# Geo3DSmart/PDANet

Measured on AMD Instinct MI355X. Metric: scenes/sec (16384-pt ONCE, PDA-SSD forward+backward), higher is better.
Workload: dtype f32; 1 GPU; once16k_b2_detector_fwd_bwd_adam; scenes_per_gpu=2, global_batch=2, parallelism=dp1, world_size_seen=1, cpu_affinity=GPU-local NUMA node of 0000:26:00.0: 128 CPUs, full=False, graph_tail=False, graph_head=True

## Files before the change

include/pda_pointnet2.h:

```cpp
#ifndef PDA_POINTNET2_H
#define PDA_POINTNET2_H

#include <stdint.h>

#ifdef __cplusplus
extern "C" {
#endif

#define PDA_OK 0
#define PDA_ERR_INVALID_ARGUMENT 1
#define PDA_ERR_LAUNCH 2
#define PDA_ERR_UNSUPPORTED 3

typedef void *pda_stream_t;

#define PDA_POINTNET2_ABI_VERSION 20
int pda_abi_version(void);
const char *pda_last_error(void);
int pda_fp_contract_mode(void);
int pda_opt_n_threads(int work_size);
int pda_fps_coop_timeouts(unsigned long long *total, int reset);
int pda_debug_fps_spin_limit(int polls);
long long pda_debug_fps_exchange_nonzero(void);

int pda_furthest_point_sampling(const float *xyz, float *temp, int32_t *idx, int b, int n, int m,
                                pda_stream_t stream);
int pda_furthest_point_sampling_with_dist(const float *dist, float *temp, int32_t *idx, int b,
                                          int n, int m, pda_stream_t stream);

int pda_gather_points(const float *points, const int32_t *idx, float *out, int b, int c, int n,
                      int m, pda_stream_t stream);
int pda_gather_points_grad(const float *grad_out, const int32_t *idx, float *grad_points, int b,
                           int c, int n, int m, pda_stream_t stream);

int pda_ball_query(const float *new_xyz, const float *xyz, int32_t *idx, int b, int n, int m,
                   float radius, int nsample, pda_stream_t stream);
int pda_ball_query_dilated(const float *new_xyz, const float *xyz, int32_t *idx, int b, int n,
                           int m, float max_radius, float min_radius, int nsample,
                           pda_stream_t stream);
int pda_ellipsoid_query(const float *new_xyz, const float *xyz, int32_t *idx, int b, int n, int m,
                        float e1, float e2, float e3, int nsample, pda_stream_t stream);
int64_t pda_ball_query_cells_scratch_bytes(int b, int n);
int pda_ball_query_cells(const float *new_xyz, const float *xyz, int32_t *const *idx, int b, int n, int m, int nr,
                         const float *radii, const int32_t *nsamples, void *scratch, int64_t scratch_bytes,
                         pda_stream_t stream);
int pda_ball_query_multi(const float *new_xyz, const float *xyz, int32_t *const *idx, int b, int n,
                         int m, int nr, const float *radii, const int32_t *nsamples,
                         pda_stream_t stream);

int pda_group_points(const float *points, const int32_t *idx, float *out, int b, int c, int n,
                     int npoints, int nsample, pda_stream_t stream);
int pda_group_points_grad(const float *grad_out, const int32_t *idx, float *grad_points, int b,
                          int c, int n, int npoints, int nsample, pda_stream_t stream);

int pda_group_rows(const float *rows, const int32_t *idx, float *out, int b, int n, int c,
                   int64_t num_idx, pda_stream_t stream);
int pda_group_rows_grad(const float *grad_out, const int32_t *idx, float *grad_rows, int b, int n,
                        int c, int64_t num_idx, pda_stream_t stream);

int pda_three_nn(const float *unknown, const float *known, float *dist2, int32_t *idx, int b,
                 int n, int m, pda_stream_t stream);
int pda_three_interpolate(const float *points, const int32_t *idx, const float *weight,
                          float *out, int b, int c, int m, int n, pda_stream_t stream);
int pda_three_interpolate_grad(const float *grad_out, const int32_t *idx, const float *weight,
                               float *grad_points, int b, int c, int n, int m,
                               pda_stream_t stream);

int pda_chamfer_forward(const float *xyz1, const float *xyz2, float *dist1, float *dist2,
                        int32_t *idx1, int32_t *idx2, int b, int n, int m, pda_stream_t stream);
int pda_chamfer_backward(const float *xyz1, const float *xyz2, float *gradxyz1, float *gradxyz2,
                         const float *graddist1, const float *graddist2, const int32_t *idx1,
                         const int32_t *idx2, int b, int n, int m, pda_stream_t stream);

int pda_group_attention_fwd(const float *qkv, float *out, float *lse, int64_t num_groups, int seq,
                            int heads, int head_dim, pda_stream_t stream);
int pda_group_attention_bwd(const float *qkv, const float *grad_out, const float *lse,
                            float *grad_qkv, int64_t num_groups, int seq, int heads, int head_dim,
                            pda_stream_t stream);
int pda_group_attention_fwd_bf16(const uint16_t *qkv, uint16_t *out, float *lse, int64_t num_groups, int seq,
                                 int heads, int head_dim, pda_stream_t stream);
int pda_group_attention_bwd_bf16(const uint16_t *qkv, const uint16_t *grad_out, const float *lse,
                                 uint16_t *grad_qkv, int64_t num_groups, int seq, int heads, int head_dim,
                                 pda_stream_t stream);

int pda_sa_mlp_maxpool(const float *xyz, const float *new_xyz, const float *features,
                       const int32_t *idx, float *out, int b, int n, int m, int c, int nsample,
                       const int32_t *dims, const float *const *wf, const float *const *scale,
                       const float *const *shift, pda_stream_t stream);
int pda_linear_cols_packed_size(int n_out, int k);
int pda_linear_cols_pack(const float *w, float *wf, int n_out, int k, int transposed_source, int gather_order,
                         pda_stream_t stream);
int pda_linear_cols(const float *x, const float *wf, float *y, int64_t tokens, int k, int n_out, pda_stream_t stream);
int pda_sa_gather_linear(const float *xyz, const float *new_xyz, const float *feats_pm, const int32_t *idx,
                         const float *wf, float *y, int b, int n, int m, int c, int nsample, int n_out,
                         pda_stream_t stream);
int64_t pda_linear_split_packed_bytes(int n_out, int k);
int pda_linear_split_pack(const float *w, void *wf, int n_out, int k, int transposed_source, pda_stream_t stream);
int pda_linear_split_pack_both(const float *w, void *wf, void *wft, int n_out, int k, pda_stream_t stream);
int pda_linear_split(const float *x, const void *wf, const float *bias, float *y, int64_t tokens, int k, int n_out,
                     int relu, pda_stream_t stream);
int pda_gemm_split(const float *x, const void *wf, const float *bias, float *y, int64_t tokens, int k, int n_out,
                   int relu, int accumulate, pda_stream_t stream);
int pda_sa_mlp_packed_size(int rows, int cols, int first_layer);
int pda_sa_mlp_pack_weights(const float *w, float *wf, int rows, int cols, int first_layer,
                            pda_stream_t stream);

#ifdef __cplusplus
}
#endif
#endif
```

include/pda_train.h:

```cpp
#ifndef PDA_TRAIN_H
#define PDA_TRAIN_H
#include "pda_pointnet2.h"

#ifdef __cplusplus
extern "C" {
#endif

int pda_grad_norm(const float *g, int64_t n, float *norm_out, float *scratch1024, pda_stream_t stream);
int pda_adam_onecycle_step(float *p, const float *g, float *m, float *v, int64_t n, float lr,
                           float beta1, float beta2, float eps, float wd, int step,
                           const float *total_norm, float max_norm, pda_stream_t stream);

int64_t pda_bn_relu_scratch_bytes(int c);
int pda_bn_relu_fwd(const float *x, const float *gamma, const float *beta, float *running_mean,
                    float *running_var, float *y, float *mean_invstd, void *scratch, int64_t rows, int c,
                    float eps, float momentum, pda_stream_t stream);
int pda_bn_relu_bwd(const float *x, const float *grad_y, const float *gamma, const float *beta,
                    const float *mean_invstd, float *grad_x, float *grad_gamma, float *grad_beta,
                    void *scratch, int64_t rows, int c, pda_stream_t stream);
int pda_bn_relu_fwd_counted(const float *x, const float *gamma, const float *beta, float *running_mean, float *running_var,
                            float *y, float *mean_invstd, void *scratch, int64_t rows, int c, float eps, float momentum,
                            const int32_t *count, int32_t *status, int relu, int training, pda_stream_t stream);
int pda_bn_relu_bwd_counted(const float *x, const float *grad_y, const float *gamma, const float *beta,
                            const float *mean_invstd, float *grad_x, float *grad_gamma, float *grad_beta, void *scratch,
// ... 112 lines not shown
int pda_assemble_tokens_ragged(const float *rppe, const float *dscale, const float *feats, const int32_t *idx,
                               const float *glob, const int32_t *rowmap, const int32_t *off, float *out,
                               int64_t max_tokens, int b, int n, int m, int nsample, int c, int rppe_compact,
                               pda_stream_t stream);
int pda_assemble_tokens_ragged_grad(const float *grad_out, const float *dscale, const float *feats,
                                    const int32_t *idx, const int32_t *cnt, const int32_t *off, const int32_t *rowmap,
                                    float *grad_rppe, float *grad_dscale, float *grad_feats, float *grad_glob,
                                    int64_t max_tokens, int b, int n, int m, int nsample, int c, int rppe_compact,
                                    pda_stream_t stream);
int pda_add_max_pool_ragged(const float *a, const float *b, const int32_t *cnt, const int32_t *off, float *out,
                            uint8_t *arg, int64_t groups, int d, pda_stream_t stream);
int pda_max_pool_scatter_ragged(const float *grad_out, const uint8_t *arg, const int32_t *rowmap,
                                const int32_t *off, float *grad_x, int64_t max_tokens, int64_t groups, int nsample,
                                int d, pda_stream_t stream);
int pda_group_attention_ragged_fwd(const float *qkv, const int32_t *cnt, const int32_t *off, float *out, float *lse,
                                   int64_t tokens, int64_t num_groups, int seq, int heads, int head_dim,
                                   pda_stream_t stream);
int pda_group_attention_ragged_bwd(const float *qkv, const float *grad_out, const float *lse, const int32_t *cnt,
                                   const int32_t *off, float *grad_qkv, int64_t tokens, int64_t num_groups, int seq,
                                   int heads, int head_dim, pda_stream_t stream);

int pda_densitynet_param_count(void);
int64_t pda_densitynet_scratch_bytes(void);
int pda_densitynet_fwd(const float *x, const float *params, float *y, float *stats, void *scratch,
                       float *running_mean1, float *running_var1, float *running_mean2, float *running_var2,
                       float *running_mean3, float *running_var3, int64_t n, float eps, float momentum,
                       pda_stream_t stream);
int pda_densitynet_bwd(const float *x, const float *grad_y, const float *params, const float *stats,
                       float *grad_params, void *scratch, int64_t n, float eps, pda_stream_t stream);
int pda_densitynet_fwd_unique(const float *x, const float *params, float *y, float *stats, void *scratch,
                              float *running_mean1, float *running_var1, float *running_mean2, float *running_var2,
                              float *running_mean3, float *running_var3, int64_t n, const int32_t *rowmap,
                              const float *row_weight, const int32_t *n_unique, int nsample, float eps, float momentum,
                              pda_stream_t stream);
int pda_densitynet_bwd_unique(const float *x, const float *grad_y, const float *params, const float *stats,
                              float *grad_params, void *scratch, int64_t n, const int32_t *rowmap,
                              const float *row_weight, const int32_t *n_unique, int nsample, float eps,
                              pda_stream_t stream);
#define PDA_DENSITYNET_MAX_SCALES 4
typedef struct pda_densitynet_scale {
    const float *x, *grad_y, *params;
    float *y, *stats;
    void *scratch;
    float *running[6];
    float *grad_params;
    int64_t n;
    const int32_t *rowmap;
    const float *row_weight;
    const int32_t *n_unique;
    int nsample;
    float eps, momentum;
} pda_densitynet_scale_t;
int pda_densitynet_fwd_multi(const pda_densitynet_scale_t *scales, int nscales, pda_stream_t stream);
int pda_densitynet_bwd_multi(const pda_densitynet_scale_t *scales, int nscales, pda_stream_t stream);

int pda_densitynet_eval_param_count(void);
int pda_densitynet_eval(const float *x, const float *folded, float *y, int64_t n, pda_stream_t stream);

int pda_pda_geometry(const float *xyz, const float *new_xyz, const int32_t *idx, float *rppe, float *dscale,
                     int b, int n, int m, int nsample, float radius, pda_stream_t stream);

int pda_points_in_boxes(const float *boxes, const float *pts, int32_t *box_idx_of_points, int b, int t,
                        int m, pda_stream_t stream);
int pda_roiaware_pool3d_fwd(const float *rois, const float *pts, const float *pts_feature, int32_t *argmax,
                            int32_t *pts_idx_of_voxels, float *pooled_features, int boxes_num, int pts_num,
                            int channels, int max_pts_each_voxel, int out_x, int out_y, int out_z, int pool_method,
                            pda_stream_t stream);
int pda_roiaware_pool3d_bwd(const int32_t *pts_idx_of_voxels, const int32_t *argmax, const float *grad_out,
                            float *grad_in, int boxes_num, int pts_num, int channels, int max_pts_each_voxel,
                            int out_x, int out_y, int out_z, int pool_method, pda_stream_t stream);
int pda_roipoint_pool3d_fwd(const float *xyz, const float *boxes3d, const float *pts_feature, float *pooled_features,
                            int32_t *pooled_empty_flag, int batch_size, int pts_num, int boxes_num, int channels,
                            int sampled_pts_num, pda_stream_t stream);
int pda_points_in_boxes_mask(const float *boxes, const float *pts, int32_t *mask, int boxes_num, int pts_num,
                             pda_stream_t stream);
int pda_points_in_boxes_count(const float *points, int stride, const float *boxes, int32_t *counts, int pts_num,
                              int batch_size, int boxes_num, pda_stream_t stream);
int pda_assign_point_targets(const float *gt_boxes, const int32_t *in_box, const int32_t *in_ext, int64_t *labels,
                             int64_t *box_idx, float *gt_of_points, int b, int n, int t, int mode, int single_class,
                             pda_stream_t stream);
int pda_head_assign_targets(const float *points, int point_stride, int point_offset, const float *gt_boxes, const float *extra_width,
                            int64_t *labels, int64_t *box_idx, float *gt_of_points, float *box_labels, const float *mean_size,
                            int bins, int b, int n, int t, int mode, int single_class, pda_stream_t stream);
int pda_sa_gaussian_mask(const float *coords, int stride, int offset, const float *gt_of_points, const int64_t *labels,
                         float *out, int64_t points, pda_stream_t stream);

int pda_boxes_overlap_bev(const float *boxes_a, const float *boxes_b, float *ans_overlap, int num_a,
                          int num_b, pda_stream_t stream);
int pda_boxes_iou_bev(const float *boxes_a, const float *boxes_b, float *ans_iou, int num_a, int num_b,
                      pda_stream_t stream);
int64_t pda_nms_mask_words(int n);
int pda_nms_bev(const float *boxes, const int32_t *num_valid, int64_t *keep, int32_t *num_keep,
                uint64_t *mask_scratch, int b, int n, float thresh, int normal, pda_stream_t stream);
int pda_multi_nms_compact(const float *boxes, const float *scores, const int64_t *keep, const int32_t *num_keep,
                          const int32_t *label_map, int b, int c, int k, int post_max, float *pred_boxes, float *pred_scores,
                          int64_t *pred_labels, int32_t *num_pred, pda_stream_t stream);
int pda_multi_nms_compact_wide(int box_cols, const float *boxes, const float *scores, const int64_t *keep,
                               const int32_t *num_keep, const int32_t *label_map, int b, int c, int k, int post_max,
                               float *pred_boxes, float *pred_scores, int64_t *pred_labels, int32_t *num_pred,
                               pda_stream_t stream);

int pda_head_cls_loss(const float *preds, int row_stride, int col0, int num_class, const int64_t *labels, const float *soft,
                      int64_t n, float scale, float *out2, float *grad, pda_stream_t stream);
int pda_head_centerness(const float *centers, const float *gt, const int64_t *labels, float *out, int64_t n, pda_stream_t stream);
int pda_head_box_loss(const float *preds, const float *labels, const int64_t *cls_labels, const float *code_weights, float beta,
                      int bins, float dir_weight, float box_weight, int64_t n, float *out4, float *grad, pda_stream_t stream);
int pda_head_vote_loss(int mode, const float *origin, const float *offsets, const int64_t *key, const float *gt, int b, int boxes,
                       int num_class, float weight, int64_t n, float *out1, float *grad, pda_stream_t stream);
int pda_head_corner_loss(const float *box_preds, const float *centers, const float *cls_preds, int num_class, const float *gt,
                         const int64_t *cls_labels, const float *mean_size, int bins, float weight, int64_t n, float *out1,
                         float *grad_box, float *grad_centers, pda_stream_t stream);

int64_t pda_sa_small_train_workspace_bytes(void);
int pda_sa_small_train_supported(int c, int nsample, int c1, int c2, int c3, int64_t tokens);
int pda_sa_small_train_fwd(const float *xyz, const float *new_xyz, const float *feat_pm, const int32_t *idx,
                           const float *w1, const float *w2, const float *w3, const float *const *gamma,
                           const float *const *beta, float *const *running_mean, float *const *running_var,
                           const float *eps, const float *momentum, void *workspace, float *out, float *zmax,
                           uint8_t *arg, int b, int n, int m, int c, int nsample, int c1, int c2, int c3,
                           pda_stream_t stream);
int pda_sa_small_train_bwd(const float *xyz, const float *new_xyz, const float *feat_pm, const int32_t *idx,
                           const float *grad_out, const float *zmax, const uint8_t *arg, void *workspace, float *dz2,
                           float *dz1, float *dw1, float *dw2, float *dw3, float *const *dgamma, float *const *dbeta,
                           int b, int n, int m, int c, int nsample, int c1, int c2, int c3, pda_stream_t stream);

int64_t pda_sa_xyz_grad_scratch_bytes(int c1);
int pda_sa_point_gather(const float *point_rows, const float *xyz, const float *new_xyz, const int32_t *idx, const float *w,
                        int ldw, const float *bias, int relu, float *z, int b, int n, int m, int nsample, int c1,
                        pda_stream_t stream);
int pda_sa_xyz_grad(const float *grad_z1, const float *xyz, const float *new_xyz, const int32_t *idx, const float *w, int ldw,
                    float *dw, int lddw, float *grad_new_xyz, void *scratch, int b, int n, int m, int nsample, int c1,
                    pda_stream_t stream);
int64_t pda_sa_point_gather_stats_blocks(int64_t tokens, int c1);
int pda_sa_point_gather_stats(const float *point_rows, const float *xyz, const float *new_xyz, const int32_t *idx,
                              const float *w, int ldw, float *z, double *partial, int b, int n, int m, int nsample, int c1,
                              pda_stream_t stream);
int pda_sa_point_grad_bn(const float *grad_a1, const float *z1, const float *mean_invstd, const float *gamma,
                         const float *beta, const float *bwd_sums, const float *xyz, const float *new_xyz, const int32_t *idx,
                         const float *w, int ldw, float *dw, int lddw, float *grad_new_xyz, float *grad_points, void *scratch,
                         int b, int n, int m, int nsample, int c1, pda_stream_t stream);

int64_t pda_input_stage_workspace_bytes(int batch, int64_t n_cap);
int pda_input_stage(const float *points, const int64_t *offsets, int64_t n_total, int batch, int c, int64_t n_cap,
                    const float *range6, int num_points, const int32_t *pick, const int32_t *perm1, const int32_t *perm2,
                    uint64_t seed, int shuffle, float *out_points, int32_t *info, void *workspace, pda_stream_t stream);
int pda_input_boxes(const float *boxes, const int64_t *box_offsets, int64_t m_total, int batch, int box_dim, int max_gt,
                    const float *range6, int min_num_corners, float *gt_boxes, int32_t *info, pda_stream_t stream);

int64_t pda_augment_workspace_bytes(int batch, int64_t n_cap, int k);
int pda_augment(const float *points, const int64_t *offsets, int64_t n_total, int batch, int c, int64_t n_cap,
                const float *boxes, const int64_t *box_offsets, int64_t m_total, const float *db_points,
                const int64_t *db_offsets, int64_t db_n_points, const float *db_boxes, const double *db_centre,
                const int32_t *db_class, int n_obj, const int32_t *cand, const int32_t *cand_group, const double *cand_dz,
                int k, const int32_t *flip, const double *angle, const float *scale, const float *remove_extra_width,
                int64_t paste_cap, float *out_points, int64_t out_cap, int64_t *out_offsets, float *out_boxes,
                int64_t out_box_cap, int64_t *out_box_offsets, int32_t *info, void *workspace, pda_stream_t stream);

int pda_augment_paste(const float *points, const int64_t *offsets, int64_t n_total, int batch, int c, int64_t n_cap,
                      const float *boxes, const int64_t *box_offsets, int64_t m_total, const float *db_points,
                      const int64_t *db_offsets, int64_t db_n_points, const float *db_boxes, const double *db_centre,
                      const int32_t *db_class, int n_obj, const int32_t *cand, const int32_t *cand_group,
                      const double *cand_dz, int k, const float *remove_extra_width, int64_t paste_cap, float *out_points,
                      int64_t out_cap, int64_t *out_offsets, float *out_boxes, int64_t out_box_cap,
                      int64_t *out_box_offsets, int32_t *info, void *workspace, pda_stream_t stream);

int64_t pda_augment_steps_workspace_bytes(int batch, int64_t n_cap, int box_slots, int n_ops);
int pda_augment_steps(const float *points, const int64_t *offsets, int64_t n_total, int batch, int c, int64_t n_cap,
                      const float *boxes, const int64_t *box_offsets, int64_t m_total, const int32_t *ops, int n_ops,
                      const double *scene_draws, const double *box_draws, int draw_cap, int box_slots,
                      const int32_t *info_in, float *out_points, int64_t out_cap, int64_t *out_offsets, float *out_boxes,
                      int64_t out_box_cap, int64_t *out_box_offsets, int32_t *info, void *workspace, pda_stream_t stream);

int64_t pda_pyramid_aug_workspace_bytes(int batch, int64_t n_cap, int box_slots);
int pda_pyramid_aug(const float *points, const int64_t *offsets, int64_t n_total, int batch, int c, int64_t n_cap,
                    const float *boxes, const int64_t *box_offsets, int64_t m_total, const double *draws_f64,
                    const int32_t *draws_i32, const uint64_t *sparsify_key, const int32_t *sparsify_keep,
                    const int32_t *n_draws, int draw_cap, const double *probs, int sparsify_max, int swap_max,
                    int box_slots, const int32_t *info_in, float *out_points, int64_t out_cap, int64_t *out_offsets,
                    float *out_boxes, int64_t out_box_cap, int64_t *out_box_offsets, int32_t *info, void *workspace,
                    pda_stream_t stream);

typedef struct pda_once_frames {
    const double *gt_boxes;
    const int32_t *gt_name;
    const int64_t *gt_offsets;
    const float *pred_boxes, *pred_score;
    const int32_t *pred_name;
    const int64_t *pred_start;
    const int32_t *pred_count;
    const int64_t *iou_start;
    int64_t n_gt_total, pred_cap, iou_cap;
    int n_frames, max_gt, max_pred;
} pda_once_frames_t;

// ... 265 lines not shown
```

pdanet_amd/_lib.py:

```python
import ctypes
import os

_HERE = os.path.dirname(os.path.abspath(__file__))
LIB_PATH = os.environ.get("PDA_LIB_PATH") or os.path.join(_HERE, "libpda_pointnet2.so")
ABI_VERSION = 20


class DensityNetScale(ctypes.Structure):
    _fields_ = [("x", ctypes.c_void_p), ("grad_y", ctypes.c_void_p), ("params", ctypes.c_void_p), ("y", ctypes.c_void_p),
                ("stats", ctypes.c_void_p), ("scratch", ctypes.c_void_p), ("running", ctypes.c_void_p * 6),
                ("grad_params", ctypes.c_void_p), ("n", ctypes.c_int64), ("rowmap", ctypes.c_void_p),
                ("row_weight", ctypes.c_void_p), ("n_unique", ctypes.c_void_p), ("nsample", ctypes.c_int),
                ("eps", ctypes.c_float), ("momentum", ctypes.c_float)]


class OnceFrames(ctypes.Structure):
    _fields_ = [("gt_boxes", ctypes.c_void_p), ("gt_name", ctypes.c_void_p), ("gt_offsets", ctypes.c_void_p),
                ("pred_boxes", ctypes.c_void_p), ("pred_score", ctypes.c_void_p), ("pred_name", ctypes.c_void_p),
                ("pred_start", ctypes.c_void_p), ("pred_count", ctypes.c_void_p), ("iou_start", ctypes.c_void_p),
                ("n_gt_total", ctypes.c_int64), ("pred_cap", ctypes.c_int64), ("iou_cap", ctypes.c_int64),
                ("n_frames", ctypes.c_int), ("max_gt", ctypes.c_int), ("max_pred", ctypes.c_int)]


class KittiFrames(ctypes.Structure):
    _fields_ = [(n, ctypes.c_void_p) for n in ("gt_bbox", "gt_loc", "gt_dims", "gt_ry", "gt_alpha", "gt_trunc", "gt_occ",
                                               "gt_name", "gt_offsets", "dt_bbox", "dt_box", "dt_alpha", "dt_score",
                                               "dt_name", "dt_start", "dt_count", "ov_start", "frame_mode")] + \
               [("n_gt_total", ctypes.c_int64), ("det_cap", ctypes.c_int64), ("ov_cap", ctypes.c_int64),
                ("n_frames", ctypes.c_int), ("max_gt", ctypes.c_int), ("max_det", ctypes.c_int)]


class ParamGradEntry(ctypes.Structure):
    _fields_ = [("kind", ctypes.c_int32), ("count", ctypes.c_int32), ("part", ctypes.c_void_p), ("part_bias", ctypes.c_void_p),
                ("dst", ctypes.c_void_p), ("dst_bias", ctypes.c_void_p), ("nm", ctypes.c_int64), ("n", ctypes.c_int32),
                ("cols", ctypes.c_int32), ("ld", ctypes.c_int64)]


PARAM_EPOCH = [0]
WEIGHT_EPOCH = [0]

_vp = ctypes.c_void_p
_i = ctypes.c_int
_f = ctypes.c_float

SIGNATURES = {
    "pda_furthest_point_sampling": [_vp, _vp, _vp, _i, _i, _i, _vp],
    "pda_furthest_point_sampling_with_dist": [_vp, _vp, _vp, _i, _i, _i, _vp],
    "pda_gather_points": [_vp, _vp, _vp, _i, _i, _i, _i, _vp],
    "pda_gather_points_grad": [_vp, _vp, _vp, _i, _i, _i, _i, _vp],
    "pda_ball_query": [_vp, _vp, _vp, _i, _i, _i, _f, _i, _vp],
    "pda_ball_query_dilated": [_vp, _vp, _vp, _i, _i, _i, _f, _f, _i, _vp],
    "pda_ellipsoid_query": [_vp, _vp, _vp, _i, _i, _i, _f, _f, _f, _i, _vp],
    "pda_ball_query_cells_scratch_bytes": [_i, _i],
    "pda_ball_query_cells": [_vp, _vp, ctypes.POINTER(_vp), _i, _i, _i, _i, ctypes.POINTER(_f), ctypes.POINTER(ctypes.c_int32),
                             _vp, ctypes.c_int64, _vp],
    "pda_ball_query_multi": [_vp, _vp, ctypes.POINTER(_vp), _i, _i, _i, _i,
                             ctypes.POINTER(_f), ctypes.POINTER(ctypes.c_int32), _vp],
    "pda_group_points": [_vp, _vp, _vp, _i, _i, _i, _i, _i, _vp],
    "pda_group_points_grad": [_vp, _vp, _vp, _i, _i, _i, _i, _i, _vp],
    "pda_group_rows": [_vp, _vp, _vp, _i, _i, _i, ctypes.c_int64, _vp],
    "pda_group_rows_grad": [_vp, _vp, _vp, _i, _i, _i, ctypes.c_int64, _vp],
    "pda_three_nn": [_vp, _vp, _vp, _vp, _i, _i, _i, _vp],
    "pda_three_interpolate": [_vp, _vp, _vp, _vp, _i, _i, _i, _i, _vp],
    "pda_three_interpolate_grad": [_vp, _vp, _vp, _vp, _i, _i, _i, _i, _vp],
    "pda_chamfer_forward": [_vp, _vp, _vp, _vp, _vp, _vp, _i, _i, _i, _vp],
    "pda_chamfer_backward": [_vp, _vp, _vp, _vp, _vp, _vp, _vp, _vp, _i, _i, _i, _vp],
    "pda_group_attention_fwd": [_vp, _vp, _vp, ctypes.c_int64, _i, _i, _i, _vp],
    "pda_group_attention_bwd": [_vp, _vp, _vp, _vp, ctypes.c_int64, _i, _i, _i, _vp],
    "pda_group_attention_fwd_bf16": [_vp, _vp, _vp, ctypes.c_int64, _i, _i, _i, _vp],
    "pda_group_attention_bwd_bf16": [_vp, _vp, _vp, _vp, ctypes.c_int64, _i, _i, _i, _vp],
    "pda_sa_mlp_maxpool": [_vp, _vp, _vp, _vp, _vp, _i, _i, _i, _i, _i, ctypes.POINTER(ctypes.c_int32),
                           ctypes.POINTER(_vp), ctypes.POINTER(_vp), ctypes.POINTER(_vp), _vp],
    "pda_linear_cols_packed_size": [_i, _i],
    "pda_linear_cols_pack": [_vp, _vp, _i, _i, _i, _i, _vp],
    "pda_linear_cols": [_vp, _vp, _vp, ctypes.c_int64, _i, _i, _vp],
    "pda_sa_gather_linear": [_vp, _vp, _vp, _vp, _vp, _vp, _i, _i, _i, _i, _i, _i, _vp],
    "pda_linear_split_packed_bytes": [_i, _i],
    "pda_linear_split_pack": [_vp, _vp, _i, _i, _i, _vp],
    "pda_linear_split_pack_both": [_vp, _vp, _vp, _i, _i, _vp],
    "pda_linear_split": [_vp, _vp, _vp, _vp, ctypes.c_int64, _i, _i, _i, _vp],
    "pda_gemm_split": [_vp, _vp, _vp, _vp, ctypes.c_int64, _i, _i, _i, _i, _vp],
    "pda_sa_mlp_packed_size": [_i, _i, _i],
    "pda_sa_mlp_pack_weights": [_vp, _vp, _i, _i, _i, _vp],
    "pda_grad_norm": [_vp, ctypes.c_int64, _vp, _vp, _vp],
    "pda_bn_relu_scratch_bytes": [_i],
    "pda_bn_relu_fwd": [_vp, _vp, _vp, _vp, _vp, _vp, _vp, _vp, ctypes.c_int64, _i, _f, _f, _vp],
    "pda_bn_relu_bwd": [_vp, _vp, _vp, _vp, _vp, _vp, _vp, _vp, _vp, ctypes.c_int64, _i, _vp],    "pda_bn_relu_fwd_mixed": [_vp, _i, _vp, _vp, _vp, _vp, _vp, _i, _vp, _vp, ctypes.c_int64, _i, _f, _f, _vp],
    "pda_bn_relu_bwd_mixed": [_vp, _i, _vp, _i, _vp, _vp, _vp, _vp, _vp, _vp, _vp, ctypes.c_int64, _i, _vp],
    "pda_bn_relu_max_pool_fwd": [_vp, _i, _vp, _vp, _vp, _vp, _vp, _vp, _vp, _vp, ctypes.c_int64, _i, _i, _f, _f, _vp],
    "pda_bn_relu_max_pool_bwd": [_vp, _i, _vp, _vp, _vp, _vp, _vp, _vp, _vp, _vp, _vp, ctypes.c_int64, _i, _i, _vp],

    "pda_layer_norm_scratch_bytes": [_i],
    "pda_layer_norm_fwd": [_vp, _vp, _vp, _vp, _vp, _vp, _vp, ctypes.c_int64, _i, _f, _vp],
    "pda_layer_norm_bwd": [_vp, _vp, _vp, _vp, _vp, _vp, _vp, _vp, _vp, ctypes.c_int64, _i, _vp],
    "pda_layer_norm_fwd_mixed": [_vp, _i, _vp, _vp, _vp, _vp, _vp, _vp, _vp, ctypes.c_int64, _i, _f, _vp],
    "pda_layer_norm_bwd_mixed": [_vp, _vp, _vp, _i, _vp, _vp, _vp, _vp, _vp, _vp, _vp, ctypes.c_int64, _i, _vp],
    "pda_linear_wgrad_scratch_bytes": [ctypes.c_int64, _i, _i],
    "pda_linear_wgrad_form": [ctypes.c_int64, _i, _i],
    "pda_linear_wgrad": [_vp, _vp, _vp, _vp, _vp, ctypes.c_int64, _i, _i, _vp],
    "pda_linear_wgrad_bn": [_vp, _vp, _vp, _vp, _vp, ctypes.c_int64, _i, _i, _vp, _vp, _vp, _vp],
    "pda_linear_wgrad_partials": [_vp, _vp, _vp, _i, ctypes.c_int64, _i, _i, ctypes.POINTER(_i), _vp],
    "pda_linear_wgrad_bn_partials": [_vp, _vp, _vp, ctypes.c_int64, _i, _i, _vp, _vp, _vp, ctypes.POINTER(_i), _vp],
    "pda_layer_norm_bwd_partials": [_vp, _vp, _vp, _i, _vp, _vp, _vp, _vp, _vp, ctypes.c_int64, _i, ctypes.POINTER(_i), _vp],
    "pda_param_grad_reduce_grouped": [ctypes.POINTER(ParamGradEntry), _i, _vp],
    "pda_gemm_split_bn_tiles": [ctypes.c_int64],
    "pda_gemm_split_bn": [_vp, _vp, _vp, ctypes.c_int64, _i, _i, _vp, _vp, _vp, _i, _vp, _vp],
    "pda_gemm_split_maxpool": [_vp, _vp, _vp, _vp, ctypes.c_int64, _i, _i, _i, _i, _vp],
    "pda_gemm_split_gather": [_vp, _vp, _vp, _vp, _vp, _i, _vp, _vp, _vp, _vp, _i, _i, _i, _i, _i, _i, _i, _vp],
    "pda_bn_stats_fwd": [_vp, _vp, _vp, _vp, _vp, ctypes.c_int64, _i, _f, _f, _vp],
    "pda_bn_finalize_fwd": [_vp, _i, _i, ctypes.c_int64, _f, _f, _vp, _vp, _vp, _vp],
    "pda_bn_relu_max_pool_apply": [_vp, _vp, _vp, _vp, _vp, _vp, ctypes.c_int64, _i, _i, _vp],
    "pda_bn_relu_bwd_reduce": [_vp, _vp, _vp, _vp, _vp, _vp, _vp, _vp, _vp, ctypes.c_int64, _i, _vp],
    "pda_colsum_scratch_bytes": [_i],
    "pda_colsum_bf16": [_vp, _vp, _vp, ctypes.c_int64, _i, _vp],
    "pda_assemble_tokens": [_vp, _vp, _vp, _vp, _vp, _vp, _i, _i, _i, _i, _i, _vp],
    "pda_assemble_tokens_grad": [_vp, _vp, _vp, _vp, _vp, _vp, _vp, _vp, _i, _i, _i, _i, _i, _vp],
    "pda_add_max_pool": [_vp, _vp, _vp, _vp, ctypes.c_int64, _i, _i, _vp],
    "pda_max_pool_scatter": [_vp, _vp, _vp, ctypes.c_int64, _i, _i, _vp],
    "pda_add_max_pool_bf16": [_vp, _vp, _vp, _vp, ctypes.c_int64, _i, _i, _vp],
    "pda_max_pool_scatter_bf16": [_vp, _vp, _vp, _vp, ctypes.c_int64, _i, _i, _vp],
    "pda_ragged_plan": [_vp, _vp, _vp, _vp, _vp, ctypes.c_int64, _i, _vp],
    "pda_assemble_tokens_ragged": [_vp, _vp, _vp, _vp, _vp, _vp, _vp, _vp, ctypes.c_int64, _i, _i, _i, _i, _i, _i, _vp],
    "pda_assemble_tokens_ragged_grad": [_vp, _vp, _vp, _vp, _vp, _vp, _vp, _vp, _vp, _vp, _vp, ctypes.c_int64, _i, _i, _i, _i, _i, _i, _vp],
    "pda_bn_relu_fwd_weighted": [_vp, _vp, _vp, _vp, _vp, _vp, _vp, _vp, ctypes.c_int64, _i, _f, _f, _vp, ctypes.c_int64, _vp],
    "pda_bn_relu_bwd_weighted": [_vp, _vp, _vp, _vp, _vp, _vp, _vp, _vp, _vp, ctypes.c_int64, _i, _vp, ctypes.c_int64, _vp],
    "pda_add_max_pool_ragged": [_vp, _vp, _vp, _vp, _vp, _vp, ctypes.c_int64, _i, _vp],
    "pda_max_pool_scatter_ragged": [_vp, _vp, _vp, _vp, _vp, ctypes.c_int64, ctypes.c_int64, _i, _i, _vp],
    "pda_group_attention_ragged_fwd": [_vp, _vp, _vp, _vp, _vp, ctypes.c_int64, ctypes.c_int64, _i, _i, _i, _vp],
    "pda_group_attention_ragged_bwd": [_vp, _vp, _vp, _vp, _vp, _vp, ctypes.c_int64, ctypes.c_int64, _i, _i, _i, _vp],
    "pda_densitynet_param_count": [],
    "pda_densitynet_eval_param_count": [],
    "pda_densitynet_scratch_bytes": [],
    "pda_densitynet_fwd": [_vp, _vp, _vp, _vp, _vp, _vp, _vp, _vp, _vp, _vp, _vp, ctypes.c_int64, _f, _f, _vp],
    "pda_densitynet_bwd": [_vp, _vp, _vp, _vp, _vp, _vp, ctypes.c_int64, _f, _vp],
    "pda_densitynet_eval": [_vp, _vp, _vp, ctypes.c_int64, _vp],
    "pda_densitynet_fwd_multi": [_vp, _i, _vp],
    "pda_densitynet_bwd_multi": [_vp, _i, _vp],
    "pda_densitynet_fwd_unique": [_vp, _vp, _vp, _vp, _vp, _vp, _vp, _vp, _vp, _vp, _vp, ctypes.c_int64, _vp, _vp, _vp, _i, _f, _f, _vp],
    "pda_densitynet_bwd_unique": [_vp, _vp, _vp, _vp, _vp, _vp, ctypes.c_int64, _vp, _vp, _vp, _i, _f, _vp],
    "pda_pda_geometry": [_vp, _vp, _vp, _vp, _vp, _i, _i, _i, _i, _f, _vp],
    "pda_points_in_boxes": [_vp, _vp, _vp, _i, _i, _i, _vp],
    "pda_roiaware_pool3d_fwd": [_vp, _vp, _vp, _vp, _vp, _vp, _i, _i, _i, _i, _i, _i, _i, _i, _vp],
    "pda_roiaware_pool3d_bwd": [_vp, _vp, _vp, _vp, _i, _i, _i, _i, _i, _i, _i, _i, _vp],
    "pda_roipoint_pool3d_fwd": [_vp, _vp, _vp, _vp, _vp, _i, _i, _i, _i, _i, _vp],
    "pda_points_in_boxes_mask": [_vp, _vp, _vp, _i, _i, _vp],
    "pda_points_in_boxes_count": [_vp, _i, _vp, _vp, _i, _i, _i, _vp],
    "pda_assign_point_targets": [_vp, _vp, _vp, _vp, _vp, _vp, _i, _i, _i, _i, _i, _vp],
    "pda_sa_gaussian_mask": [_vp, _i, _i, _vp, _vp, _vp, ctypes.c_int64, _vp],
    "pda_head_assign_targets": [_vp, _i, _i, _vp, ctypes.POINTER(ctypes.c_float), _vp, _vp, _vp, _vp, _vp, _i, _i, _i, _i, _i, _i, _vp],
    "pda_head_cls_loss": [_vp, _i, _i, _i, _vp, _vp, ctypes.c_int64, _f, _vp, _vp, _vp],
    "pda_head_centerness": [_vp, _vp, _vp, _vp, ctypes.c_int64, _vp],
    "pda_head_box_loss": [_vp, _vp, _vp, _vp, _f, _i, _f, _f, ctypes.c_int64, _vp, _vp, _vp],
    "pda_head_vote_loss": [_i, _vp, _vp, _vp, _vp, _i, _i, _i, _f, ctypes.c_int64, _vp, _vp, _vp],
    "pda_head_corner_loss": [_vp, _vp, _vp, _i, _vp, _vp, _vp, _i, _f, ctypes.c_int64, _vp, _vp, _vp, _vp],
    "pda_boxes_overlap_bev": [_vp, _vp, _vp, _i, _i, _vp],
    "pda_boxes_iou_bev": [_vp, _vp, _vp, _i, _i, _vp],
    "pda_nms_mask_words": [_i],
    "pda_nms_bev": [_vp, _vp, _vp, _vp, _vp, _i, _i, _f, _i, _vp],
    "pda_sa_small_train_workspace_bytes": [],
    "pda_sa_small_train_supported": [_i, _i, _i, _i, _i, ctypes.c_int64],
    "pda_sa_small_train_fwd": [_vp] * 7 + [ctypes.POINTER(_vp)] * 4 + [ctypes.POINTER(_f)] * 2 + [_vp] * 4 + [_i] * 8 + [_vp],
    "pda_sa_small_train_bwd": [_vp] * 13 + [ctypes.POINTER(_vp)] * 2 + [_i] * 8 + [_vp],
    "pda_sa_xyz_grad_scratch_bytes": [_i],
    "pda_sa_point_gather": [_vp, _vp, _vp, _vp, _vp, _i, _vp, _i, _vp, _i, _i, _i, _i, _i, _vp],
    "pda_sa_xyz_grad": [_vp, _vp, _vp, _vp, _vp, _i, _vp, _i, _vp, _vp, _i, _i, _i, _i, _i, _vp],
    "pda_sa_point_gather_stats_blocks": [ctypes.c_int64, _i],
    "pda_sa_point_gather_stats": [_vp, _vp, _vp, _vp, _vp, _i, _vp, _vp, _i, _i, _i, _i, _i, _vp],
    "pda_sa_point_grad_bn": [_vp] * 10 + [_i, _vp, _i, _vp, _vp, _vp, _i, _i, _i, _i, _i, _vp],
    "pda_adam_onecycle_step": [_vp, _vp, _vp, _vp, ctypes.c_int64, _f, _f, _f, _f, _f, _i, _vp, _f, _vp],
    "pda_input_stage_workspace_bytes": [_i, ctypes.c_int64],
    "pda_input_stage": [_vp, _vp, ctypes.c_int64, _i, _i, ctypes.c_int64, ctypes.POINTER(_f), _i, _vp, _vp, _vp,
                        ctypes.c_uint64, _i, _vp, _vp, _vp, _vp],
    "pda_input_boxes": [_vp, _vp, ctypes.c_int64, _i, _i, _i, ctypes.POINTER(_f), _i, _vp, _vp, _vp],
    "pda_augment_workspace_bytes": [_i, ctypes.c_int64, _i],
    "pda_augment": [_vp, _vp, ctypes.c_int64, _i, _i, ctypes.c_int64, _vp, _vp, ctypes.c_int64, _vp, _vp, ctypes.c_int64, _vp,
                    _vp, _vp, _i, _vp, _vp, _vp, _i, _vp, _vp, _vp, ctypes.POINTER(_f), ctypes.c_int64, _vp, ctypes.c_int64,
                    _vp, _vp, ctypes.c_int64, _vp, _vp, _vp, _vp],
    "pda_augment_paste": [_vp, _vp, ctypes.c_int64, _i, _i, ctypes.c_int64, _vp, _vp, ctypes.c_int64, _vp, _vp, ctypes.c_int64, _vp,
                          _vp, _vp, _i, _vp, _vp, _vp, _i, ctypes.POINTER(_f), ctypes.c_int64, _vp, ctypes.c_int64, _vp, _vp,
                          ctypes.c_int64, _vp, _vp, _vp, _vp],
    "pda_augment_steps_workspace_bytes": [_i, ctypes.c_int64, _i, _i],
    "pda_augment_steps": [_vp, _vp, ctypes.c_int64, _i, _i, ctypes.c_int64, _vp, _vp, ctypes.c_int64,
                          ctypes.POINTER(ctypes.c_int32), _i, _vp, _vp, _i, _i, _vp, _vp, ctypes.c_int64, _vp, _vp,
                          ctypes.c_int64, _vp, _vp, _vp, _vp],
    "pda_pyramid_aug_workspace_bytes": [_i, ctypes.c_int64, _i],
    "pda_pyramid_aug": [_vp, _vp, ctypes.c_int64, _i, _i, ctypes.c_int64, _vp, _vp, ctypes.c_int64, _vp, _vp, _vp, _vp, _vp, _i,
                        ctypes.POINTER(ctypes.c_double), _i, _i, _i, _vp, _vp, ctypes.c_int64, _vp, _vp, ctypes.c_int64, _vp,
                        _vp, _vp, _vp],
    "pda_once_eval_workspace_bytes": [_i, ctypes.c_int64, _i],
    "pda_once_eval_iou": [ctypes.POINTER(OnceFrames), _i, _vp, _vp, _vp],
    "pda_once_eval_accumulate": [ctypes.POINTER(OnceFrames), _vp, _vp, _i, _i, ctypes.POINTER(ctypes.c_double), _i, _vp, _vp,
                                 _vp, _vp],
    "pda_once_eval_match": [ctypes.POINTER(OnceFrames), _vp, _vp, _i, _i, ctypes.POINTER(ctypes.c_double), _i, _i, _vp, _vp,
                            _vp, _vp, _vp, _vp, _vp, _vp],
    "pda_kitti_eval_workspace_bytes": [_i, ctypes.c_int64, ctypes.c_int64, _i],
    "pda_kitti_eval_overlaps": [ctypes.POINTER(KittiFrames), _vp, _vp, _vp],
    "pda_kitti_eval_first_pass": [ctypes.POINTER(KittiFrames), _vp, _i, _i, _vp, _vp, _vp, ctypes.POINTER(ctypes.c_double),
                                  _vp, _vp, _vp, _vp, _vp, _vp],
    "pda_kitti_eval_match": [ctypes.POINTER(KittiFrames), _vp, _i, _i, _vp, _vp, _vp, ctypes.POINTER(ctypes.c_double), _i,
                             _vp, _vp, _vp, _vp, _vp, _vp, _vp, _vp, _vp, _vp, _vp],
    "pda_kitti_eval_predictions": [_vp, ctypes.c_int64, _i, _i, _vp, _vp, _vp, _i, _vp, _vp, _vp, _vp, _vp],
    "pda_recall_record": [_vp, _vp, _vp, _i, ctypes.POINTER(_f), _i, _vp, _vp, _i, _i, _i, _vp],
    "pda_roi_max_iou": [_vp, _vp, _vp, _i, _i, _vp, _vp, _i, _i, _i, _vp],
    "pda_roi_sample_targets": [_vp, _vp, _vp, _vp, _i, _vp, _vp, _i, _i] + [ctypes.c_double] * 5 + [_i, _vp, _vp, _vp, _vp,
                               ctypes.c_uint64] + [_vp] * 10 + [_i, _i, _i, _vp],
    "pda_kitti_fov_filter_workspace_bytes": [_i, ctypes.c_int64],
    "pda_kitti_fov_filter": [_vp, _vp, ctypes.c_int64, _i, _i, ctypes.c_int64, _vp, _vp, _vp, ctypes.c_int64, _vp, _vp, _vp, _vp],
    "pda_gt_extract_workspace_bytes": [_i, ctypes.c_int64, ctypes.c_int64],
    "pda_gt_extract_count": [_vp, _vp, ctypes.c_int64, _i, _i, ctypes.c_int64, _vp, _vp, ctypes.c_int64, _vp, _vp, _vp, _vp],
    "pda_gt_extract_write": [_vp, _vp, ctypes.c_int64, _i, _i, ctypes.c_int64, _vp, _vp, ctypes.c_int64, _vp, _vp, _vp,
                             ctypes.c_int64, _vp, _vp, _vp],
    "pda_voxel_workspace_bytes": [_i, ctypes.c_int64, _i, _i],
    "pda_voxelize": [_vp, _vp, ctypes.c_int64, _i, _i, ctypes.c_int64, ctypes.POINTER(_f), ctypes.POINTER(_f),
                     ctypes.POINTER(ctypes.c_int32), _i, _i, _vp, _vp, _vp, _vp, _vp, _vp],
    "pda_voxel_sample": [_vp, _vp, ctypes.c_int64, _i, _i, ctypes.c_int64, ctypes.POINTER(_f), ctypes.POINTER(_f),
                         ctypes.POINTER(ctypes.c_int32), _i, _i, _i, _i, _i, _vp, _vp, ctypes.c_int64, ctypes.c_uint64, _vp,
                         ctypes.c_int64, _vp, _vp, _vp, _vp],
    "pda_dyn_voxel_workspace_bytes": [ctypes.c_int64, _i],
    "pda_dyn_voxel_index": [_vp, ctypes.c_int64, _i, ctypes.POINTER(_f), ctypes.POINTER(_f), ctypes.POINTER(ctypes.c_int32),
                            _i, _i, _vp, _vp, _vp, _vp, _vp, _vp, _vp, _vp, _vp],
    "pda_dyn_scatter_mean": [_vp, _i, _vp, _vp, _vp, ctypes.c_int64, _vp, _vp],
    "pda_dyn_scatter_max_fwd": [_vp, _i, _vp, _vp, _vp, ctypes.c_int64, _vp, _vp, _vp],
    "pda_dyn_scatter_max_bwd": [_vp, _vp, _vp, _vp, ctypes.c_int64, ctypes.c_int64, _i, _vp, _vp],
    "pda_dyn_pillar_features": [_vp, ctypes.c_int64, _i, _vp, _vp, _vp, _vp, _vp, ctypes.POINTER(_f), ctypes.POINTER(_f), _i,
                                _i, _vp, _vp],
    "pda_pillar_scatter_fwd": [_vp, _vp, _vp, ctypes.c_int64, _i, _i, _i, _i, _vp, _vp],
    "pda_pillar_scatter_bwd": [_vp, _vp, _vp, ctypes.c_int64, _i, _i, _i, _i, _vp, _vp],
    "pda_center_assign_targets": [_vp, _i, _i, _i, _i, _i] + [ctypes.POINTER(ctypes.c_int32)] * 3 + [_i, _i, _i]
                                 + [ctypes.c_double] * 6 + [_i] + [ctypes.POINTER(_vp)] * 4 + [_vp],
    "pda_center_focal_blocks": [ctypes.c_int64],
    "pda_center_focal_loss": [_vp, _vp, ctypes.c_int64, _vp, _vp, _vp, _vp],
    "pda_center_scale": [_vp, _vp, _vp, _f, ctypes.c_int64, _vp, _vp],
# ... 139 lines not shown
```

pdanet_amd/csrc/gemm_split.hip:

```cpp
#include "pda_common.h"
#include "split_bf16.h"

#include <stdlib.h>

namespace pda {

constexpr int GS_MAX_N = 2048;
constexpr int GS_KSTEP = 12 * 64;

__device__ __forceinline__ void split_pack_one(const float* __restrict__ w, uint32_t* __restrict__ wf, int64_t o, int rows, int cols,
                                               int KS, int trans) {
    const int pr = (int)(o & 3), lane = (int)((o >> 2) & 63);
    int64_t rest = o >> 8;
    const int rb = (int)(rest & 3); rest >>= 2;
    const int s = (int)(rest % KS), c = (int)(rest / KS);
    const int row = c * 128 + rb * 32 + (lane & 31);
    const int k = 16 * s + 8 * (lane >> 5) + 2 * pr;
    float v[2];
    for (int e = 0; e < 2; ++e)
        v[e] = (row < rows && k + e < cols) ? (trans ? w[(size_t)(k + e) * rows + row] : w[(size_t)row * cols + k + e]) : 0.f;
    uint32_t h, m, l;
    split2(v[0], v[1], h, m, l);
    const size_t base = ((((size_t)c * KS + s) * 4 + rb) * 3) * 256 + (size_t)lane * 4 + pr;
    wf[base] = h; wf[base + 256] = m; wf[base + 512] = l;
}

__global__ void split_pack_kernel(const float* __restrict__ w, uint32_t* __restrict__ wf, int rows, int cols, int KS,
                                  int chunks, int trans) {
    const int64_t total = (int64_t)chunks * KS * 4 * 64 * 4;
    for (int64_t o = blockIdx.x * (int64_t)blockDim.x + threadIdx.x; o < total; o += (int64_t)gridDim.x * blockDim.x)
        split_pack_one(w, wf, o, rows, cols, KS, trans);
}

__global__ void split_pack_both_kernel(const float* __restrict__ w, uint32_t* __restrict__ wf, uint32_t* __restrict__ wft, int n_out,
                                       int k, int KS, int chunks, int KSt, int chunks_t) {
    const int64_t total = (int64_t)chunks * KS * 4 * 64 * 4, total_t = (int64_t)chunks_t * KSt * 4 * 64 * 4;
    for (int64_t o = blockIdx.x * (int64_t)blockDim.x + threadIdx.x; o < total + total_t; o += (int64_t)gridDim.x * blockDim.x) {
        if (o < total) split_pack_one(w, wf, o, n_out, k, KS, 0);
        else split_pack_one(w, wft, o - total, k, n_out, KSt, 1);
    }
}

struct LinSplitParams {
    const float* x;
    const uint4* wf;
    const float* bias;
    float* y;
    int64_t tokens;
    int k, n_out, chunks, relu;
    int cpb;
    unsigned long long* dbg;
};
#ifdef GS_PROFILE
#define GS_MARK(i) do { if (tid == 0) p.dbg[(size_t)blockIdx.x * 16 + (i)] = __builtin_readcyclecounter(); } while (0)
#else
#define GS_MARK(i) do {} while (0)
#endif

template <int KS>
__global__ __launch_bounds__(256) __attribute__((amdgpu_waves_per_eu(1, 1)))
void lin_split_kernel(const LinSplitParams p) {
    constexpr int G = KS % 4 == 0 ? 4 : 2;
    constexpr int TILE = G * GS_KSTEP;
    constexpr int NG = KS / G;
    constexpr int NLD = TILE / 256;
    __shared__ uint4 ring[3 * TILE];
    __shared__ float bias_s[GS_MAX_N];
    const int tid = threadIdx.x, lane = tid & 63, w = __builtin_amdgcn_readfirstlane(tid >> 6);
    const int h = lane >> 5, j = lane & 31;
    const int64_t tok0 = ((int64_t)blockIdx.x * 4 + w) * 32;
    const int64_t tk = tok0 + j < p.tokens ? tok0 + j : p.tokens - 1;
    const uint4* src = p.wf + tid;
    const int ntiles = p.chunks * NG;
    const int c0 = (int)blockIdx.y * p.cpb, c1 = min(p.chunks, c0 + p.cpb);
    const uint32_t ring_base = (uint32_t)(uintptr_t)(__attribute__((address_space(3))) void*)ring + w * 1024;
    auto issue = [&](int t, int slot) {
        const uint4* g = src + (size_t)(t < ntiles ? t : ntiles - 1) * TILE;
        const uint32_t l = ring_base + slot * (TILE * 16);
#pragma unroll
        for (int i = 0; i < NLD; ++i) glds16(g + 256 * i, l + 4096 * i);
    };
    static_assert(NLD <= G * 4, "one DMA instruction per MFMA group at most");
    GS_MARK(0);
    float x[KS * 8];
    {
        const float* row = p.x + tk * p.k + 8 * h;
#pragma unroll
        for (int s = 0; s < KS; ++s) {
            const float4 a = *reinterpret_cast<const float4*>(row + 16 * s), b = *reinterpret_cast<const float4*>(row + 16 * s + 4);
            x[8 * s] = a.x; x[8 * s + 1] = a.y; x[8 * s + 2] = a.z; x[8 * s + 3] = a.w;
            x[8 * s + 4] = b.x; x[8 * s + 5] = b.y; x[8 * s + 6] = b.z; x[8 * s + 7] = b.w;
        }
    }
    for (int i = tid; i < p.n_out; i += 256) bias_s[i] = p.bias ? p.bias[i] : 0.f;
    asm volatile("s_waitcnt vmcnt(0)" ::: "memory");
    GS_MARK(1);
    issue(c0 * NG, 0);
    issue(c0 * NG + 1, 1);
    asm volatile("s_waitcnt vmcnt(%0)" ::"n"(NLD) : "memory");
    __builtin_amdgcn_s_barrier();
    GS_MARK(2);
    const uint32_t lane_off = (uint32_t)(4 * h * p.n_out + j);
    const int64_t left = p.tokens - tok0 - 4 * h;
    const bool whole = tok0 + 32 <= p.tokens;
    auto store_one = [&](const gs_f32x16 (&res)[4], int chunk, int n) {
        const int r = n >> 4, i = n & 15, t = (i & 3) + 8 * (i >> 2);
        float v = res[r][i] + bias_s[chunk * 128 + r * 32 + j];
        if (p.relu) v = fmaxf(v, 0.f);
        float* row = p.y + (tok0 + t) * p.n_out + chunk * 128 + r * 32;
        if (whole) row[lane_off] = v;
        else if (t < left) row[lane_off] = v;
    };
    int ti = c0 * NG, slot = 0;
    gs_f32x16 done[4];
    for (int c = c0; c < c1; ++c) {
        gs_f32x16 acc[4];
#pragma unroll
        for (int r = 0; r < 4; ++r)
#pragma unroll
            for (int i = 0; i < 16; ++i) acc[r][i] = 0.f;
#pragma unroll
        for (int g = 0; g < NG; ++g, ++ti, slot = slot == 2 ? 0 : slot + 1) {
            if (c == 1 && g == 0) GS_MARK(4);
// ... 411 lines not shown
        }
        return;
    }
    double cs1[4], cs2[4];
#pragma unroll
    for (int ot = 0; ot < 4; ++ot) {
        cs1[ot] = 0; cs2[ot] = 0;
        const int col = (2 * ncb + wo) * 128 + ot * 32 + r;
        if (col >= p.n_out) continue;
        const float bias = p.bias ? p.bias[col] : 0.f;
#pragma unroll
        for (int tt = 0; tt < 2; ++tt) {
            const int64_t trow = tok0 + wt * 64 + tt * 32 + 4 * h;
#pragma unroll
            for (int i = 0; i < 16; ++i) {
                const int64_t tok = trow + (i & 3) + 8 * (i >> 2);
                if (tok < p.tokens) {
                    float* dst = p.y + tok * p.n_out + col;
                    float v = acc[tt][ot][i] + bias;
                    if (p.accum) v += *dst;
                    if (p.relu) v = fmaxf(v, 0.f);
#ifdef GS_NOSTORE
                    if (v == 12345.678f)
#endif
                    *dst = v;
                    if constexpr (EPI == 1) { cs1[ot] += v; cs2[ot] += (double)v * v; }
                }
            }
        }
    }
    if constexpr (EPI == 1) {
        double* red = reinterpret_cast<double*>(gp_planes);
        __syncthreads();
#pragma unroll
        for (int ot = 0; ot < 4; ++ot) {
            const double a = cs1[ot] + __shfl_xor(cs1[ot], 32), b = cs2[ot] + __shfl_xor(cs2[ot], 32);
            if (h == 0) {
                const int cl = wo * 128 + ot * 32 + r;
                red[(wt * 256 + cl) * 2] = a; red[(wt * 256 + cl) * 2 + 1] = b;
            }
        }
        __syncthreads();
        if (tid < 256) {
            const int col = 2 * ncb * 128 + tid;
            if (col < p.n_out) {
                double a = 0, b = 0;
#pragma unroll
                for (int q = 0; q < TW; ++q) { a += red[(q * 256 + tid) * 2]; b += red[(q * 256 + tid) * 2 + 1]; }
                double* pp = p.partial + (size_t)(blockIdx.x / (unsigned)wide_chunks) * 2 * p.n_out;
                pp[col] = a; pp[p.n_out + col] = b;
            }
        }
    }
}

}

PDA_API int64_t pda_linear_split_packed_bytes(int n_out, int k) {
    if (n_out <= 0 || k <= 0) return 0;
    return (int64_t)pda::divup(n_out, 128) * pda::divup(k, 32) * 2 * 12 * 64 * 16;
}

PDA_API int pda_linear_split_pack(const float* w, void* wf, int n_out, int k, int transposed_source, pda_stream_t stream) {
    PDA_REQUIRE(w && wf && n_out > 0 && k > 0, "pda_linear_split_pack: bad argument");
    const int chunks = pda::divup(n_out, 128), KS = pda::divup(k, 32) * 2;
    const int64_t total = (int64_t)chunks * KS * 4 * 64 * 4;
    const int blocks = (int)(pda::divup64(total, 256) < 2048 ? pda::divup64(total, 256) : 2048);
    hipLaunchKernelGGL(pda::split_pack_kernel, dim3(blocks), dim3(256), 0, (hipStream_t)stream, w, (uint32_t*)wf, n_out, k, KS,
                       chunks, transposed_source);
    return pda::check_launch("pda_linear_split_pack");
}

PDA_API int pda_linear_split_pack_both(const float* w, void* wf, void* wft, int n_out, int k, pda_stream_t stream) {
    PDA_REQUIRE(w && wf && wft && n_out > 0 && k > 0, "pda_linear_split_pack_both: bad argument");
    const int chunks = pda::divup(n_out, 128), KS = pda::divup(k, 32) * 2;
    const int chunks_t = pda::divup(k, 128), KSt = pda::divup(n_out, 32) * 2;
    const int64_t total = ((int64_t)chunks * KS + (int64_t)chunks_t * KSt) * 4 * 64 * 4;
    const int blocks = (int)(pda::divup64(total, 256) < 2048 ? pda::divup64(total, 256) : 2048);
    hipLaunchKernelGGL(pda::split_pack_both_kernel, dim3(blocks), dim3(256), 0, (hipStream_t)stream, w, (uint32_t*)wf, (uint32_t*)wft,
                       n_out, k, KS, chunks, KSt, chunks_t);
    return pda::check_launch("pda_linear_split_pack_both");
}

PDA_API int pda_linear_split(const float* x, const void* wf, const float* bias, float* y, int64_t tokens, int k, int n_out,
                             int relu, pda_stream_t stream) {
    PDA_REQUIRE(tokens >= 0 && k > 0 && n_out > 0, "pda_linear_split: bad size");
    if (tokens == 0) return PDA_OK;
    PDA_REQUIRE(x && wf && y && (((uintptr_t)x | (uintptr_t)wf | (uintptr_t)y | (uintptr_t)bias) & 15) == 0,
                "pda_linear_split: null or misaligned pointer");
    if (k % 32 != 0 || k > 512 || n_out % 128 != 0 || n_out > pda::GS_MAX_N) {
        pda::set_error("pda_linear_split: no kernel built for K=%d, N=%d (K a multiple of 32 <= 512, N a multiple of 128 <= 2048)", k, n_out);
        return PDA_ERR_UNSUPPORTED;
    }
    pda::LinSplitParams p{};
    p.x = x; p.wf = (const uint4*)wf; p.bias = bias; p.y = y; p.tokens = tokens; p.k = k; p.n_out = n_out; p.chunks = n_out / 128;
    p.relu = relu;
#ifdef GS_PROFILE
    p.dbg = (unsigned long long*)bias; p.bias = nullptr;
#endif
    const int64_t tiles = pda::divup64(tokens, 128);
    const int want = tiles >= 192 ? 1 : (int)pda::divup64(256, tiles);
    p.cpb = pda::divup(p.chunks, want < p.chunks ? want : p.chunks);
    const dim3 grid((unsigned)tiles, (unsigned)pda::divup(p.chunks, p.cpb)), block(256);
    const hipStream_t s = (hipStream_t)stream;
    switch (k / 16) {
#define PDA_GS_CASE(KS) case KS: hipLaunchKernelGGL((pda::lin_split_kernel<KS>), grid, block, 0, s, p); break
        PDA_GS_CASE(2); PDA_GS_CASE(4); PDA_GS_CASE(6); PDA_GS_CASE(8); PDA_GS_CASE(12); PDA_GS_CASE(16); PDA_GS_CASE(24); PDA_GS_CASE(32);
#undef PDA_GS_CASE
        default:
            pda::set_error("pda_linear_split: no kernel built for K=%d", k);
            return PDA_ERR_UNSUPPORTED;
    }
    return pda::check_launch("pda_linear_split");
}

PDA_API int pda_gemm_split(const float* x, const void* wf, const float* bias, float* y, int64_t tokens, int k, int n_out,
                           int relu, int accumulate, pda_stream_t stream) {
    PDA_REQUIRE(tokens >= 0 && k > 0 && n_out > 0, "pda_gemm_split: bad size");
    if (tokens == 0) return PDA_OK;
    PDA_REQUIRE(x && wf && y && (((uintptr_t)x | (uintptr_t)wf) & 15) == 0, "pda_gemm_split: null or misaligned pointer");
    if (k % 16 != 0) {
        pda::set_error("pda_gemm_split: K=%d must be a multiple of 16", k);
        return PDA_ERR_UNSUPPORTED;
    }
    pda::GemmSplitParams p{};
    p.x = x; p.wf = (const uint4*)wf; p.bias = bias; p.y = y; p.tokens = tokens; p.k = k; p.n_out = n_out;
    p.chunks = pda::divup(n_out, 128); p.ksteps = pda::divup(k, 32) * 2; p.relu = relu; p.accum = accumulate;
    const int64_t blocks = pda::divup64(tokens, 128) * p.chunks;
    PDA_REQUIRE(blocks < (1ll << 31), "pda_gemm_split: too many tiles");
    const int packed_steps = p.ksteps;
    p.ksteps = k / 16;
    if (packed_steps != p.ksteps) {
        pda::set_error("pda_gemm_split: K=%d must be a multiple of 32 (packed planes come in pairs of K steps)", k);
        return PDA_ERR_UNSUPPORTED;
    }
    static const int force = getenv("PDA_GEMM_SPLIT_TILE") ? atoi(getenv("PDA_GEMM_SPLIT_TILE")) : 0;
    const int64_t wide_blocks = pda::divup64(tokens, 256) * ((p.chunks + 1) / 2);
    if (force == 256 || (force != 128 && wide_blocks >= 200 && (p.chunks % 2 == 0 || p.chunks >= 5))) {
        static pda::PerDevice<bool> lds_ok;
        const bool ok = lds_ok.get([] { return hipFuncSetAttribute((const void*)pda::gemm_split_wide_kernel<0, 0>, hipFuncAttributeMaxDynamicSharedMemorySize,
                                                                   2 * pda::GW_TILE_U4 * 16) == hipSuccess; });
        if (ok) {
            hipLaunchKernelGGL((pda::gemm_split_wide_kernel<0, 0>), dim3((unsigned)wide_blocks), dim3(512), 2 * pda::GW_TILE_U4 * 16,
                               (hipStream_t)stream, p);
            return pda::check_launch("pda_gemm_split");
        }
    }
    hipLaunchKernelGGL(pda::gemm_split_kernel, dim3((unsigned)blocks), dim3(256), 0, (hipStream_t)stream, p);
    return pda::check_launch("pda_gemm_split");
}

PDA_API int64_t pda_gemm_split_bn_tiles(int64_t tokens) { return tokens > 0 ? pda::divup64(tokens, 256) : 0; }

PDA_API int pda_gemm_split_bn(const float* x, const void* wf, float* y, int64_t tokens, int k, int n_out, const float* in_mean_invstd,
                              const float* in_gamma, const float* in_beta, int stats_mode, double* partial, pda_stream_t stream) {
    PDA_REQUIRE(tokens >= 1 && k > 0 && n_out > 0, "pda_gemm_split_bn: bad size");
    PDA_REQUIRE(x && wf && y && (((uintptr_t)x | (uintptr_t)wf) & 15) == 0, "pda_gemm_split_bn: null or misaligned pointer");
    const bool pro = in_mean_invstd != nullptr;
    PDA_REQUIRE(pro == (in_gamma != nullptr) && pro == (in_beta != nullptr), "pda_gemm_split_bn: the input BatchNorm needs mean_invstd, gamma and beta");
    PDA_REQUIRE(stats_mode >= 0 && stats_mode <= 1 && (stats_mode == 0 || partial), "pda_gemm_split_bn: stats_mode=%d (0 or 1; 1 needs `partial`)", stats_mode);
    if (k % 32 != 0 || k > 1024) {
        pda::set_error("pda_gemm_split_bn: no kernel built for K=%d (a multiple of 32, <= 1024)", k);
        return PDA_ERR_UNSUPPORTED;
    }
    pda::GemmSplitParams p{};
    p.x = x; p.wf = (const uint4*)wf; p.y = y; p.tokens = tokens; p.k = k; p.n_out = n_out;
// ... 69 lines not shown
```

pdanet_amd/csrc/head_loss.hip:

```cpp
#include "pda_common.h"

namespace pda {

constexpr int HL_THREADS = 1024;

__device__ __forceinline__ double hl_block_sum(double v, double* red) {
    const int lane = threadIdx.x & 63, w = threadIdx.x >> 6;
#pragma unroll
    for (int o = 32; o > 0; o >>= 1) v += __shfl_down(v, o);
    __syncthreads();
    if (lane == 0) red[w] = v;
    __syncthreads();
    if (threadIdx.x == 0) {
        double s = 0;
        for (int i = 0; i < HL_THREADS / 64; ++i) s += red[i];
        red[16] = s;
    }
    __syncthreads();
    return red[16];
}

__device__ __forceinline__ float hl_smooth_l1(float d, float beta, float& dd) {
    const float n = fabsf(d);
    if (beta < 1e-5f) { dd = d > 0.f ? 1.f : (d < 0.f ? -1.f : 0.f); return n; }
    if (n < beta) { dd = d / beta; return 0.5f * n * n / beta; }
    dd = d > 0.f ? 1.f : -1.f;
    return n - 0.5f * beta;
}

__global__ __launch_bounds__(HL_THREADS) void head_cls_loss_kernel(const float* __restrict__ preds, int row_stride, int col0, int C,
                                                                   const int64_t* __restrict__ labels, const float* __restrict__ soft,
                                                                   int64_t n, float scale, float* __restrict__ out,
                                                                   float* __restrict__ grad) {
    __shared__ double red[17];
    double cnt = 0;
    for (int64_t r = threadIdx.x; r < n; r += HL_THREADS) cnt += labels[r] > 0 ? 1.0 : 0.0;
    const double npos = hl_block_sum(cnt, red);
    const float wnorm = 1.f / (float)(npos > 1.0 ? npos : 1.0);
    double acc = 0;
    for (int64_t r = threadIdx.x; r < n; r += HL_THREADS) {
        const int64_t lab = labels[r];
        const float w = lab >= 0 ? wnorm : 0.f;
        const float s = soft ? soft[r] : 1.f;
        const float* x = preds + r * row_stride;
        float* g = grad + r * row_stride;
        for (int c = 0; c < col0; ++c) g[c] = 0.f;
        for (int c = col0 + C; c < row_stride; ++c) g[c] = 0.f;
        float rowloss = 0.f;
        for (int c = 0; c < C; ++c) {
            const float v = x[col0 + c];
            const float t = lab == c + 1 ? s : 0.f;
            const float e = expf(-fabsf(v));
            rowloss += fmaxf(v, 0.f) - v * t + log1pf(e);
            const float sig = v >= 0.f ? 1.f / (1.f + e) : e / (1.f + e);
            g[col0 + c] = scale * w * (sig - t) / (float)C;
        }
        acc += (double)(w * rowloss) / C;
    }
    const double total = hl_block_sum(acc, red);
    if (threadIdx.x == 0) { out[0] = scale * (float)total; out[1] = (float)npos; }
}

__global__ __launch_bounds__(256) void head_centerness_kernel(const float* __restrict__ centers, const float* __restrict__ gt,
                                                              const int64_t* __restrict__ labels, float* __restrict__ out, int64_t n) {
    const int64_t p = (int64_t)blockIdx.x * 256 + threadIdx.x;
    if (p >= n) return;
    const float* c = centers + p * 4 + 1;
    const float* g = gt + p * 8;
    const float dx = c[0] - g[0], dy = c[1] - g[1], dz = c[2] - g[2];
    const float a = -g[6], ca = cosf(a), sa = sinf(a);
    const float o[3] = {dx * ca + dy * (-sa), dx * sa + dy * ca, dz};
    float prod = 1.f;
#pragma unroll
    for (int k = 0; k < 3; ++k) {
        const float m = g[3 + k] * 0.5f;
        const float d0 = m - o[k], d1 = m + o[k];
        prod *= fminf(d0, d1) / fmaxf(d0, d1);
    }
    out[p] = labels[p] > 0 ? powf(fmaxf(prod, 1e-6f), 1.f / 3.f) : 0.f;
}

__global__ __launch_bounds__(HL_THREADS) void head_box_loss_kernel(const float* __restrict__ preds, const float* __restrict__ labels,
                                                                   const int64_t* __restrict__ cls_labels, const float* __restrict__ code_w,
                                                                   float beta, int nb, float dir_w, float box_w, int64_t n,
                                                                   float* __restrict__ out, float* __restrict__ grad) {
    __shared__ double red[17];
    const int W = 6 + 2 * nb;
    double cnt = 0, sres = 0;
    for (int64_t r = threadIdx.x; r < n; r += HL_THREADS) {
        cnt += cls_labels[r] > 0 ? 1.0 : 0.0;
        const int id = (int)labels[r * 8 + 6];
        float dd;
        sres += hl_smooth_l1(preds[r * W + 6 + nb + id] - labels[r * 8 + 7], 1.f, dd);
    }
    const double npos = hl_block_sum(cnt, red);
    const double res_mean = hl_block_sum(sres, red) / (double)(n > 0 ? n : 1);
    const float wpos = 1.f / (float)(npos > 1.0 ? npos : 1.0);
    const float sumw = npos > 0.0 ? 1.f : 0.f;
    double a_xyz = 0, a_cls = 0;
    for (int64_t r = threadIdx.x; r < n; r += HL_THREADS) {
        const float w = cls_labels[r] > 0 ? wpos : 0.f;
        const float* x = preds + r * W;
        const float* l = labels + r * 8;
        float* g = grad + r * W;
        float rl = 0.f;
#pragma unroll
        for (int k = 0; k < 6; ++k) {
            const float cw = code_w ? code_w[k] : 1.f;
            const float t = (__float_as_uint(l[k]) & 0x7fffffffu) > 0x7f800000u ? x[k] : l[k];
            float dd;
            rl += hl_smooth_l1((x[k] - t) * cw, beta, dd);
            g[k] = box_w * w * dd * cw;
        }
        a_xyz += (double)(w * rl);
        const int id = (int)l[6];
        float mx = x[6];
        for (int k = 1; k < nb; ++k) mx = fmaxf(mx, x[6 + k]);
        float se = 0.f;
        for (int k = 0; k < nb; ++k) se += expf(x[6 + k] - mx);
        const float lse = mx + logf(se);
        a_cls += (double)(w * (lse - x[6 + id]));
        for (int k = 0; k < nb; ++k) g[6 + k] = box_w * dir_w * w * (expf(x[6 + k] - lse) - (k == id ? 1.f : 0.f));
        float dd;
        hl_smooth_l1(x[6 + nb + id] - l[7], 1.f, dd);
        for (int k = 0; k < nb; ++k) g[6 + nb + k] = k == id ? box_w * sumw * dd / (float)n : 0.f;
    }
    const double xyz = hl_block_sum(a_xyz, red);
    const double cls = hl_block_sum(a_cls, red) * dir_w;
    if (threadIdx.x == 0) {
        const double res = res_mean * sumw;
        out[0] = (float)((xyz + res + cls) * box_w); out[1] = (float)xyz; out[2] = (float)cls; out[3] = (float)res;
    }
}

constexpr int HL_MAX_SEG = 2048;
__global__ __launch_bounds__(HL_THREADS) void head_vote_loss_kernel(int mode, const float* __restrict__ origin, const float* __restrict__ offsets,
                                                                    const int64_t* __restrict__ key, const float* __restrict__ gt, int B,
                                                                    int S, int num_class, float weight, int64_t n, float* __restrict__ out,
                                                                    float* __restrict__ grad) {
    __shared__ double red[17];
    __shared__ float cnt[HL_MAX_SEG], m3[HL_MAX_SEG][3], a3[HL_MAX_SEG][3], lsum[HL_MAX_SEG];
    const int nseg = mode == 0 ? num_class + 1 : B * S;
    for (int s = threadIdx.x; s < nseg; s += HL_THREADS) {
        cnt[s] = 0.f; lsum[s] = 0.f;
        for (int k = 0; k < 3; ++k) { m3[s][k] = 0.f; a3[s][k] = 0.f; }
    }
    __syncthreads();
    const int64_t per_scene = n / (B > 0 ? B : 1);
    auto seg_of = [&](int64_t r) -> int {
        const int64_t k = key[r];
        if (mode == 0) return (k >= 1 && k <= num_class) ? (int)k : -1;
        return k >= 0 ? (int)(r / per_scene) * S + (int)k : -1;
    };
    for (int64_t r = threadIdx.x; r < n; r += HL_THREADS) {
        const int s = seg_of(r);
        if (s < 0) continue;
        atomicAdd(&cnt[s], 1.f);
        if (mode == 1)
            for (int k = 0; k < 3; ++k) atomicAdd(&m3[s][k], origin[r * 4 + 1 + k] + offsets[r * 4 + 1 + k]);
    }
    __syncthreads();
    if (mode == 1)
        for (int s = threadIdx.x; s < nseg; s += HL_THREADS)
            for (int k = 0; k < 3; ++k) m3[s][k] = m3[s][k] / fmaxf(cnt[s], 1.f);
    __syncthreads();
    double present = 0;
    for (int s = threadIdx.x; s < nseg; s += HL_THREADS) present += cnt[s] > 0.f ? 1.0 : 0.0;
    const double npresent = hl_block_sum(present, red);
    const float inv_present = 1.f / (float)(npresent > 1.0 ? npresent : 1.0);
    for (int64_t r = threadIdx.x; r < n; r += HL_THREADS) {
        const int s = seg_of(r);
        if (s < 0) continue;
        float l = 0.f;
        for (int k = 0; k < 3; ++k) {
            const float p = origin[r * 4 + 1 + k] + offsets[r * 4 + 1 + k];
            float dd;
            l += hl_smooth_l1(p - gt[r * 8 + k], 1.f, dd);
            if (mode == 1) {
                float dm;
                l += 0.5f * hl_smooth_l1(p - m3[s][k], 1.f, dm);
                atomicAdd(&a3[s][k], dm);
            }
        }
        atomicAdd(&lsum[s], l);
    }
    __syncthreads();
    double acc = 0;
    for (int s = threadIdx.x; s < nseg; s += HL_THREADS)
        if (cnt[s] > 0.f) acc += (double)lsum[s] / (double)(cnt[s] * (mode == 0 ? 3.f : 1.f));
    const double total = hl_block_sum(acc, red);
    if (threadIdx.x == 0) out[0] = mode == 0 ? (float)(total / npresent * weight) : (float)(total * inv_present * weight);
    for (int64_t r = threadIdx.x; r < n; r += HL_THREADS) {
        const int s = seg_of(r);
        float* g = grad + r * 4;
        g[0] = 0.f;
        if (s < 0) { g[1] = g[2] = g[3] = 0.f; continue; }
        const float base = weight / (mode == 0 ? (float)npresent * 3.f * cnt[s] : cnt[s]) * (mode == 0 ? 1.f : inv_present);
        for (int k = 0; k < 3; ++k) {
            const float p = origin[r * 4 + 1 + k] + offsets[r * 4 + 1 + k];
            float dd, dm = 0.f;
            hl_smooth_l1(p - gt[r * 8 + k], 1.f, dd);
            float d = dd;
            if (mode == 1) {
                hl_smooth_l1(p - m3[s][k], 1.f, dm);
                d += 0.5f * (dm - a3[s][k] / cnt[s]);
            }
            g[1 + k] = base * d;
        }
    }
}

__global__ __launch_bounds__(HL_THREADS) void head_corner_loss_kernel(const float* __restrict__ box_preds, const float* __restrict__ centers,
                                                                      const float* __restrict__ cls_preds, int C, const float* __restrict__ gt,
                                                                      const int64_t* __restrict__ cls_labels, const float* __restrict__ mean_size,
                                                                      int nb, float weight, int64_t n, float* __restrict__ out,
                                                                      float* __restrict__ grad_box, float* __restrict__ grad_ctr) {
    __shared__ double red[17];
    const int W = 6 + 2 * nb;
    const float PI = 3.14159265358979323846f;
    const float inter = 2.f * PI / (float)nb;
    double cnt = 0;
    for (int64_t r = threadIdx.x; r < n; r += HL_THREADS) cnt += cls_labels[r] > 0 ? 1.0 : 0.0;
    const double npos = hl_block_sum(cnt, red);
    const float wpos = weight / (float)npos;
    double acc = 0;
    const float tmpl[8][3] = {{1, 1, -1}, {1, -1, -1}, {-1, -1, -1}, {-1, 1, -1}, {1, 1, 1}, {1, -1, 1}, {-1, -1, 1}, {-1, 1, 1}};
    for (int64_t r = threadIdx.x; r < n; r += HL_THREADS) {
        float* gb = grad_box + r * W;
        float* gc = grad_ctr + r * 4;
        for (int k = 0; k < W; ++k) gb[k] = 0.f;
        gc[0] = gc[1] = gc[2] = gc[3] = 0.f;
        if (!(cls_labels[r] > 0)) continue;
        const float* e = box_preds + r * W;
        int pc = 0;
        for (int c = 1; c < C; ++c) pc = cls_preds[r * C + c] > cls_preds[r * C + pc] ? c : pc;
        float dxa = 1.f, dya = 1.f, dza = 1.f, diag = 1.f;
        if (mean_size) { dxa = mean_size[pc * 3]; dya = mean_size[pc * 3 + 1]; dza = mean_size[pc * 3 + 2]; diag = sqrtf(dxa * dxa + dya * dya); }
        const float xa = centers[r * 4 + 1], ya = centers[r * 4 + 2], za = centers[r * 4 + 3];
        const float xg = mean_size ? e[0] * diag + xa : e[0] + xa, yg = mean_size ? e[1] * diag + ya : e[1] + ya,
                    zg = mean_size ? e[2] * dza + za : e[2] + za;
        const float dxg = expf(e[3]) * dxa, dyg = expf(e[4]) * dya, dzg = expf(e[5]) * dza;
        int bin = 0;
        for (int k = 1; k < nb; ++k) bin = e[6 + k] > e[6 + bin] ? k : bin;
        const float ry = ((float)bin * inter - PI + inter * 0.5f) + e[6 + nb + bin] * (inter * 0.5f);
        const float* g = gt + r * 8;
        const float cp = cosf(ry), sp = sinf(ry), cg = cosf(g[6]), sg = sinf(g[6]), cf = cosf(g[6] + PI), sf = sinf(g[6] + PI);
        float d_x = 0.f, d_y = 0.f, d_z = 0.f, d_dx = 0.f, d_dy = 0.f, d_dz = 0.f, d_ry = 0.f, lsum = 0.f;
#pragma unroll
        for (int k = 0; k < 8; ++k) {
            const float tx = tmpl[k][0] * 0.5f, ty = tmpl[k][1] * 0.5f, tz = tmpl[k][2] * 0.5f;
            const float px = tx * dxg, py = ty * dyg;
            const float rx = px * cp - py * sp, rry = px * sp + py * cp;
            const float pcx = rx + xg, pcy = rry + yg, pcz = tz * dzg + zg;
            const float qx = tx * g[3], qy = ty * g[4];
            const float gx = qx * cg - qy * sg + g[0], gy = qx * sg + qy * cg + g[1], gz = tz * g[5] + g[2];
            const float fx = qx * cf - qy * sf + g[0], fy = qx * sf + qy * cf + g[1];
            const float ax = pcx - gx, ay = pcy - gy, az = pcz - gz;
            const float bx = pcx - fx, by = pcy - fy;
            const float d0 = sqrtf(ax * ax + ay * ay + az * az), d1 = sqrtf(bx * bx + by * by + az * az);
            const bool first = d0 <= d1;
            const float d = first ? d0 : d1;
            float dd;
            lsum += hl_smooth_l1(d, 1.f, dd);
            const float inv = d > 0.f ? dd / d : 0.f;
            const float ux = (first ? ax : bx) * inv, uy = (first ? ay : by) * inv, uz = az * inv;
            d_x += ux; d_y += uy; d_z += uz;
            d_dx += ux * tx * cp + uy * tx * sp;
            d_dy += -ux * ty * sp + uy * ty * cp;
            d_dz += uz * tz;
            d_ry += -ux * rry + uy * rx;
        }
        acc += (double)(lsum * 0.125f);
        const float s = wpos * 0.125f;
        gc[1] = s * d_x; gc[2] = s * d_y; gc[3] = s * d_z;
        gb[0] = s * d_x * (mean_size ? diag : 1.f); gb[1] = s * d_y * (mean_size ? diag : 1.f); gb[2] = s * d_z * (mean_size ? dza : 1.f);
        gb[3] = s * d_dx * dxg; gb[4] = s * d_dy * dyg; gb[5] = s * d_dz * dzg;
        gb[6 + nb + bin] = s * d_ry * (inter * 0.5f);
    }
    const double total = hl_block_sum(acc, red);
    if (threadIdx.x == 0) out[0] = (float)(total / npos) * weight;
}

}

PDA_API int pda_head_cls_loss(const float* preds, int row_stride, int col0, int num_class, const int64_t* labels, const float* soft,
                              int64_t n, float scale, float* out2, float* grad, pda_stream_t stream) {
    PDA_REQUIRE(n >= 0 && num_class >= 1 && col0 >= 0 && col0 + num_class <= row_stride, "pda_head_cls_loss: bad shape");
    PDA_REQUIRE(preds && labels && out2 && grad, "pda_head_cls_loss: null pointer");
    hipLaunchKernelGGL(pda::head_cls_loss_kernel, dim3(1), dim3(pda::HL_THREADS), 0, (hipStream_t)stream, preds, row_stride, col0, num_class,
                       labels, soft, n, scale, out2, grad);
    return pda::check_launch("pda_head_cls_loss");
}

PDA_API int pda_head_centerness(const float* centers, const float* gt, const int64_t* labels, float* out, int64_t n, pda_stream_t stream) {
    PDA_REQUIRE(n >= 0, "pda_head_centerness: n=%lld", (long long)n);
    if (n == 0) return PDA_OK;
    PDA_REQUIRE(centers && gt && labels && out, "pda_head_centerness: null pointer");
    hipLaunchKernelGGL(pda::head_centerness_kernel, dim3((unsigned)pda::divup64(n, 256)), dim3(256), 0, (hipStream_t)stream, centers, gt, labels,
                       out, n);
    return pda::check_launch("pda_head_centerness");
}

PDA_API int pda_head_box_loss(const float* preds, const float* labels, const int64_t* cls_labels, const float* code_weights, float beta,
                              int bins, float dir_weight, float box_weight, int64_t n, float* out4, float* grad, pda_stream_t stream) {
    PDA_REQUIRE(n >= 1 && bins >= 1 && bins <= 64, "pda_head_box_loss: n=%lld bins=%d", (long long)n, bins);
    PDA_REQUIRE(preds && labels && cls_labels && out4 && grad, "pda_head_box_loss: null pointer");
    hipLaunchKernelGGL(pda::head_box_loss_kernel, dim3(1), dim3(pda::HL_THREADS), 0, (hipStream_t)stream, preds, labels, cls_labels,
                       code_weights, beta, bins, dir_weight, box_weight, n, out4, grad);
    return pda::check_launch("pda_head_box_loss");
}

PDA_API int pda_head_vote_loss(int mode, const float* origin, const float* offsets, const int64_t* key, const float* gt, int b, int boxes,
                               int num_class, float weight, int64_t n, float* out1, float* grad, pda_stream_t stream) {
    PDA_REQUIRE(n >= 1 && b >= 1 && n % b == 0 && (mode == 0 || mode == 1), "pda_head_vote_loss: n=%lld b=%d mode=%d", (long long)n, b, mode);
    if ((mode == 0 ? num_class + 1 : b * boxes) > pda::HL_MAX_SEG) {
        pda::set_error("pda_head_vote_loss: %d segments exceed %d", mode == 0 ? num_class + 1 : b * boxes, pda::HL_MAX_SEG);
        return PDA_ERR_UNSUPPORTED;
    }
    PDA_REQUIRE(origin && offsets && key && gt && out1 && grad, "pda_head_vote_loss: null pointer");
    hipLaunchKernelGGL(pda::head_vote_loss_kernel, dim3(1), dim3(pda::HL_THREADS), 0, (hipStream_t)stream, mode, origin, offsets, key, gt, b,
                       boxes, num_class, weight, n, out1, grad);
    return pda::check_launch("pda_head_vote_loss");
}

PDA_API int pda_head_corner_loss(const float* box_preds, const float* centers, const float* cls_preds, int num_class, const float* gt,
                                 const int64_t* cls_labels, const float* mean_size, int bins, float weight, int64_t n, float* out1,
                                 float* grad_box, float* grad_centers, pda_stream_t stream) {
    PDA_REQUIRE(n >= 1 && bins >= 1 && bins <= 64 && num_class >= 1, "pda_head_corner_loss: n=%lld bins=%d", (long long)n, bins);
    PDA_REQUIRE(box_preds && centers && cls_preds && gt && cls_labels && out1 && grad_box && grad_centers, "pda_head_corner_loss: null pointer");
    hipLaunchKernelGGL(pda::head_corner_loss_kernel, dim3(1), dim3(pda::HL_THREADS), 0, (hipStream_t)stream, box_preds, centers, cls_preds,
                       num_class, gt, cls_labels, mean_size, bins, weight, n, out1, grad_box, grad_centers);
    return pda::check_launch("pda_head_corner_loss");
}
```

pdanet_amd/csrc/head_targets.hip:

```cpp
#include "pda_common.h"

namespace pda {

__global__ __launch_bounds__(256) void assign_point_targets_kernel(const float* __restrict__ gt_boxes, const int* __restrict__ in_box,
                                                                   const int* __restrict__ in_ext, int64_t* __restrict__ labels,
                                                                   int64_t* __restrict__ box_idx, float* __restrict__ gt_of_points,
                                                                   int n, int t, int mode, int single_class, int64_t total) {
    const int64_t p = (int64_t)blockIdx.x * 256 + threadIdx.x;
    if (p >= total) return;
    const int64_t b = p / n;
    const int ib = in_box[p], ie = in_ext[p];
    const bool box_fg = ib >= 0, ext_fg = ie >= 0;
    bool fg;
    int idx;
    int64_t lab = 0;
    if (mode == 0) {
        fg = box_fg; idx = ib;
        if (fg != ext_fg) lab = -1;
    } else {
        idx = box_fg ? ib : ie;
        if (mode == 2) { fg = ext_fg != box_fg; if (ib != -1) idx = -1; }
        else fg = ext_fg;
    }
    const float4* row = reinterpret_cast<const float4*>(gt_boxes + ((size_t)b * t + (idx < 0 ? idx + t : idx)) * 8);
    const float4 r0 = row[0], r1 = row[1];
    const int64_t cls = single_class ? 1 : (int64_t)r1.w;
    if (fg) lab = cls;
    labels[p] = lab;
    box_idx[p] = idx;
    float4* out = reinterpret_cast<float4*>(gt_of_points + (size_t)p * 8);
    out[0] = r0; out[1] = r1;
}

__global__ __launch_bounds__(256) void sa_gaussian_mask_kernel(const float* __restrict__ coords, int stride, int offset,
                                                               const float* __restrict__ gt, const int64_t* __restrict__ labels,
                                                               float* __restrict__ out, int64_t total) {
    const int64_t p = (int64_t)blockIdx.x * 256 + threadIdx.x;
    if (p >= total) return;
    const float* c = coords + (size_t)p * stride + offset;
    const float4 g0 = reinterpret_cast<const float4*>(gt + (size_t)p * 8)[0], g1 = reinterpret_cast<const float4*>(gt + (size_t)p * 8)[1];
    const float dx = c[0] - g0.x, dy = c[1] - g0.y, dz = c[2] - g0.z;
    const float w = g0.w, l = g1.x, h = g1.y, a = -g1.z, cls = g1.w;
    const float ca = cosf(a), sa = sinf(a);
    const float ox = dx * ca + dy * (-sa), oy = dx * sa + dy * ca, oz = dz;
    const float k = cls == 1.f ? 4.f : (cls == 2.f ? 6.f : (cls == 3.f ? 5.f : 1.f));
    const float vx = ox * (4.f / (w * w + l * l) * k), vy = oy * (4.f / (w * w + h * h) * k), vz = oz * (4.f / (h * h + l * l) * k);
    const float hm = expf(-0.5f * (vx * vx + vy * vy + vz * vz));
    out[p] = labels[p] > 0 ? hm : 0.f;
}

struct HtBoxRec {
    float cx, cy, cz, cosa, sina, hz, hz_e;
    double lim_x, lim_y, lim_xe, lim_ye;
};

__global__ __launch_bounds__(256) void head_assign_targets_kernel(const float* __restrict__ pts, int pstride, int poff,
                                                                  const float* __restrict__ gt_boxes, float ex, float ey, float ez,
                                                                  int64_t* __restrict__ labels, int64_t* __restrict__ box_idx,
                                                                  float* __restrict__ gt_of_points, float* __restrict__ box_labels,
                                                                  const float* __restrict__ mean_size, int bins, int n, int t, int mode,
                                                                  int single_class) {
    __shared__ HtBoxRec rec[256];
    const int bs = blockIdx.y;
    const int pt = blockIdx.x * 256 + threadIdx.x;
    const bool live = pt < n;
    float x = 0.f, y = 0.f, z = 0.f;
    if (live) {
        const float* p = pts + ((size_t)bs * n + pt) * pstride + poff;
        x = p[0]; y = p[1]; z = p[2];
    }
    int ib = -1, ie = -1;
    for (int k0 = 0; k0 < t; k0 += 256) {
        const int nk = min(256, t - k0);
        __syncthreads();
        if ((int)threadIdx.x < nk) {
            const float* b = gt_boxes + ((size_t)bs * t + k0 + threadIdx.x) * 8;
            HtBoxRec r;
            r.cx = b[0]; r.cy = b[1]; r.cz = b[2];
            const double a = (double)(-b[6]);
            r.cosa = (float)cos(a);
            r.sina = (float)sin(a);
            r.hz = b[5] * 0.5f;
            r.lim_x = (double)b[3] / 2.0 + (double)1e-5f;
            r.lim_y = (double)b[4] / 2.0 + (double)1e-5f;
            const float dxe = b[3] + ex, dye = b[4] + ey, dze = b[5] + ez;
            r.hz_e = dze * 0.5f;
            r.lim_xe = (double)dxe / 2.0 + (double)1e-5f;
            r.lim_ye = (double)dye / 2.0 + (double)1e-5f;
            rec[threadIdx.x] = r;
        }
        __syncthreads();
        if (live && (ib < 0 || ie < 0)) {
            for (int k = 0; k < nk; ++k) {
                const HtBoxRec& r = rec[k];
                const float az = fabsf(z - r.cz);
                if (az > r.hz_e && az > r.hz) continue;
                const float sx = x - r.cx, sy = y - r.cy;
#if PDA_FP_CONTRACT
                const float lx = __builtin_fmaf(sx, r.cosa, sy * (-r.sina));
                const float ly = __builtin_fmaf(sx, r.sina, sy * r.cosa);
#else
                const float lx = sx * r.cosa + sy * (-r.sina);
                const float ly = sx * r.sina + sy * r.cosa;
#endif
                const double alx = (double)fabsf(lx), aly = (double)fabsf(ly);
                if (ib < 0 && !(az > r.hz) && alx < r.lim_x && aly < r.lim_y) ib = k0 + k;
                if (ie < 0 && !(az > r.hz_e) && alx < r.lim_xe && aly < r.lim_ye) ie = k0 + k;
                if (ib >= 0 && ie >= 0) break;
            }
        }
    }
    if (!live) return;
    const size_t p = (size_t)bs * n + pt;
    const bool box_fg = ib >= 0, ext_fg = ie >= 0;
    bool fg;
    int idx;
    int64_t lab = 0;
    if (mode == 0) {
        fg = box_fg; idx = ib;
        if (fg != ext_fg) lab = -1;
    } else {
        idx = box_fg ? ib : ie;
        if (mode == 2) { fg = ext_fg != box_fg; if (ib != -1) idx = -1; }
        else fg = ext_fg;
    }
    const float4* row = reinterpret_cast<const float4*>(gt_boxes + ((size_t)bs * t + (idx < 0 ? idx + t : idx)) * 8);
    const float4 r0 = row[0], r1 = row[1];
    const int64_t cls = single_class ? 1 : (int64_t)r1.w;
    if (fg) lab = cls;
    labels[p] = lab;
    box_idx[p] = idx;
    float4* out = reinterpret_cast<float4*>(gt_of_points + p * 8);
    out[0] = r0; out[1] = r1;
    if (box_labels) {
        float4 e0 = make_float4(0.f, 0.f, 0.f, 0.f), e1 = e0;
        if (lab > 0) {
            const float PI = 3.14159265358979323846f;
            const float dxg = fmaxf(r0.w, 1e-5f), dyg = fmaxf(r1.x, 1e-5f), dzg = fmaxf(r1.y, 1e-5f);
            if (mean_size) {
                int gc = (int)r1.w; gc = gc < 1 ? 1 : gc;
                const float dxa = mean_size[(gc - 1) * 3], dya = mean_size[(gc - 1) * 3 + 1], dza = mean_size[(gc - 1) * 3 + 2];
                const float diag = sqrtf(dxa * dxa + dya * dya);
                e0 = make_float4((r0.x - x) / diag, (r0.y - y) / diag, (r0.z - z) / dza, logf(dxg / dxa));
                e1.x = logf(dyg / dya); e1.y = logf(dzg / dza);
            } else {
                e0 = make_float4(r0.x - x, r0.y - y, r0.z - z, logf(dxg));
                e1.x = logf(dyg); e1.y = logf(dzg);
            }
            const float inter = (float)(2.0 * 3.14159265358979323846 / (double)bins), half = (float)(3.14159265358979323846 / (double)bins);
            const float rg = fminf(fmaxf(r1.z, -PI + 1e-5f), PI - 1e-5f);
            const float sh = rg + PI;
            const float bin = floorf(sh / inter);
            e1.z = bin;
            e1.w = (sh - (bin * inter + half)) / half;
        }
        float4* bl = reinterpret_cast<float4*>(box_labels + p * 8);
        bl[0] = e0; bl[1] = e1;
    }
}

}

PDA_API int pda_assign_point_targets(const float* gt_boxes, const int32_t* in_box, const int32_t* in_ext, int64_t* labels,
                                     int64_t* box_idx, float* gt_of_points, int b, int n, int t, int mode, int single_class,
                                     pda_stream_t stream) {
    PDA_REQUIRE(b >= 0 && n >= 0 && t >= 1 && mode >= 0 && mode <= 2, "pda_assign_point_targets: b=%d n=%d boxes=%d mode=%d", b, n, t, mode);
    const int64_t total = (int64_t)b * n;
    if (total == 0) return PDA_OK;
    PDA_REQUIRE(gt_boxes && in_box && in_ext && labels && box_idx && gt_of_points, "pda_assign_point_targets: null pointer");
    PDA_REQUIRE((((uintptr_t)gt_boxes | (uintptr_t)gt_of_points) & 15) == 0, "pda_assign_point_targets: gt_boxes / gt_of_points must be 16-byte aligned");
    hipLaunchKernelGGL(pda::assign_point_targets_kernel, dim3((unsigned)pda::divup64(total, 256)), dim3(256), 0, (hipStream_t)stream, gt_boxes,
                       in_box, in_ext, labels, box_idx, gt_of_points, n, t, mode, single_class, total);
    return pda::check_launch("pda_assign_point_targets");
}

PDA_API int pda_sa_gaussian_mask(const float* coords, int stride, int offset, const float* gt_of_points, const int64_t* labels,
                                 float* out, int64_t points, pda_stream_t stream) {
    PDA_REQUIRE(points >= 0 && stride >= 3 && offset >= 0 && offset + 3 <= stride, "pda_sa_gaussian_mask: points=%lld stride=%d offset=%d",
                (long long)points, stride, offset);
    if (points == 0) return PDA_OK;
    PDA_REQUIRE(coords && gt_of_points && labels && out, "pda_sa_gaussian_mask: null pointer");
    PDA_REQUIRE(((uintptr_t)gt_of_points & 15) == 0, "pda_sa_gaussian_mask: gt_of_points must be 16-byte aligned");
    hipLaunchKernelGGL(pda::sa_gaussian_mask_kernel, dim3((unsigned)pda::divup64(points, 256)), dim3(256), 0, (hipStream_t)stream, coords,
                       stride, offset, gt_of_points, labels, out, points);
    return pda::check_launch("pda_sa_gaussian_mask");
}

PDA_API int pda_head_assign_targets(const float* points, int point_stride, int point_offset, const float* gt_boxes, const float* extra_width,
                                    int64_t* labels, int64_t* box_idx, float* gt_of_points, float* box_labels, const float* mean_size,
                                    int bins, int b, int n, int t, int mode, int single_class, pda_stream_t stream) {
    PDA_REQUIRE(b >= 0 && n >= 0 && t >= 1 && mode >= 0 && mode <= 2 && point_stride >= 3 && point_offset >= 0 && point_offset + 3 <= point_stride,
                "pda_head_assign_targets: b=%d n=%d boxes=%d mode=%d stride=%d", b, n, t, mode, point_stride);
    if (b == 0 || n == 0) return PDA_OK;
    PDA_REQUIRE(points && gt_boxes && extra_width && labels && box_idx && gt_of_points, "pda_head_assign_targets: null pointer");
    PDA_REQUIRE((((uintptr_t)gt_boxes | (uintptr_t)gt_of_points | (uintptr_t)box_labels) & 15) == 0 && b <= 65535,
                "pda_head_assign_targets: gt_boxes / gt_of_points / box_labels must be 16-byte aligned, b <= 65535");
    PDA_REQUIRE(!box_labels || (bins >= 1 && bins <= 64), "pda_head_assign_targets: bins=%d", bins);
    hipLaunchKernelGGL(pda::head_assign_targets_kernel, dim3(pda::divup(n, 256), b), dim3(256), 0, (hipStream_t)stream, points, point_stride,
                       point_offset, gt_boxes, extra_width[0], extra_width[1], extra_width[2], labels, box_idx, gt_of_points, box_labels,
                       mean_size, bins, n, t, mode, single_class);
    return pda::check_launch("pda_head_assign_targets");
}
```

pdanet_amd/iassd_head.py:

```python
import numpy as np
import os

import torch
import torch.nn as nn
import torch.nn.functional as F

from . import box_coder_utils, box_utils, loss_utils, roiaware_pool3d_utils


def _get(cfg, key, default=None):
    return cfg.get(key, default) if hasattr(cfg, "get") else getattr(cfg, key, default)


FUSED_HEAD_TARGETS = True

FUSED_HEAD_LOSS = os.environ.get("PDA_FUSED_HEAD_LOSS", "1") != "0"


class IASSD_Head(nn.Module):
    def __init__(self, num_class, input_channels, model_cfg, predict_boxes_when_training=False, **kwargs):
        super().__init__()
        self.model_cfg, self.num_class = model_cfg, num_class
        self.predict_boxes_when_training = predict_boxes_when_training
        target_cfg = model_cfg["TARGET_CONFIG"]
        if target_cfg["BOX_CODER"] != "PointResidual_BinOri_Coder":
            raise NotImplementedError(target_cfg["BOX_CODER"])
        self.box_coder = box_coder_utils.PointResidual_BinOri_Coder(**target_cfg["BOX_CODER_CONFIG"])
        detector_dim = _get(model_cfg, "INPUT_DIM", input_channels)
        self.cls_center_layers = self.make_fc_layers(model_cfg["CLS_FC"], detector_dim, num_class)
        self.box_center_layers = self.make_fc_layers(model_cfg["REG_FC"], detector_dim, self.box_coder.code_size)
        if _get(model_cfg, "IOU_FC") is not None:
            raise NotImplementedError("IOU_FC head (not used by PDA-SSD.yaml)")
        self.build_losses(model_cfg["LOSS_CONFIG"])
        self.forward_ret_dict = None

    @staticmethod
    def make_fc_layers(fc_cfg, input_channels, output_channels):
        layers, c_in = [], input_channels
        for c in fc_cfg:
            layers.extend([nn.Linear(c_in, c, bias=False), nn.BatchNorm1d(c), nn.ReLU()])
            c_in = c
        layers.append(nn.Linear(c_in, output_channels, bias=True))
        return nn.Sequential(*layers)

    def build_losses(self, losses_cfg):
        for key in ("LOSS_CLS", "LOSS_INS"):
            if not str(_get(losses_cfg, key, "WeightedCrossEntropy")).startswith("WeightedCrossEntropy"):
                raise NotImplementedError("%s = %s" % (key, losses_cfg[key]))
        if losses_cfg["LOSS_REG"] != "WeightedSmoothL1Loss":
            raise NotImplementedError(losses_cfg["LOSS_REG"])
        self.decode_in_training = True
        self.cls_loss_func = loss_utils.WeightedClassificationLoss()
        self.ins_loss_func = loss_utils.WeightedClassificationLoss()
        self.reg_loss_func = loss_utils.WeightedSmoothL1Loss(
            code_weights=_get(losses_cfg["LOSS_WEIGHTS"], "code_weights"), **_get(losses_cfg, "LOSS_REG_CONFIG", {}))

    def assign_stack_targets_IASSD(self, points, gt_boxes, extend_gt_boxes=None, ret_box_labels=False,
                                   set_ignore_flag=True, use_ex_gt_assign=False, fg_pc_ignore=False,
                                   binary_label=False, extra_width=None):
        assert points.dim() == 2 and points.shape[1] == 4 and gt_boxes.dim() == 3 and gt_boxes.shape[2] == 8
        B, T = gt_boxes.shape[0], gt_boxes.shape[1]
        assert points.shape[0] % B == 0, "scenes must contribute equally many points"
        if FUSED_HEAD_TARGETS and points.is_cuda and extra_width is not None and (use_ex_gt_assign or set_ignore_flag):
            mode = (2 if fg_pc_ignore else 1) if use_ex_gt_assign else 0
            coder = self.box_coder
            mean = coder._mean(gt_boxes).contiguous() if (ret_box_labels and coder.use_mean_size) else None
            labels, idx, gt_of_pts, box_labels = roiaware_pool3d_utils.head_assign_targets(
                points.contiguous(), gt_boxes.contiguous(), extra_width, mode, self.num_class == 1 or binary_label, mean_size=mean,
                bins=coder.bin_size, ret_box_labels=ret_box_labels)
            return {'point_cls_labels': labels, 'point_box_labels': box_labels, 'box_idxs_labels': idx,
                    'gt_box_of_points': gt_of_pts}
        xyz = points[:, 1:4].reshape(B, -1, 3).contiguous()
        N = xyz.shape[1]
        if FUSED_HEAD_TARGETS and xyz.is_cuda and (use_ex_gt_assign or set_ignore_flag):
            in_box = roiaware_pool3d_utils.points_in_boxes_gpu(xyz, gt_boxes[:, :, 0:7].contiguous())
            in_ext = roiaware_pool3d_utils.points_in_boxes_gpu(xyz, extend_gt_boxes[:, :, 0:7].contiguous())
            mode = (2 if fg_pc_ignore else 1) if use_ex_gt_assign else 0
            labels, idx, gt_of_pts = roiaware_pool3d_utils.assign_point_targets(
                gt_boxes.contiguous(), in_box, in_ext, mode, self.num_class == 1 or binary_label)
            box_labels = None
            if ret_box_labels:
                enc = self.box_coder.encode_torch(gt_of_pts[:, :-1], xyz.reshape(B * N, 3),
                                                  gt_classes=gt_of_pts[:, -1].long().clamp(min=1))
                box_labels = torch.where((labels > 0).reshape(-1, 1), enc, torch.zeros_like(enc))
            return {'point_cls_labels': labels, 'point_box_labels': box_labels, 'box_idxs_labels': idx,
                    'gt_box_of_points': gt_of_pts}
        in_box = roiaware_pool3d_utils.points_in_boxes_gpu(xyz, gt_boxes[:, :, 0:7].contiguous()).long()
        box_fg = in_box >= 0
        labels = torch.zeros_like(in_box)
        if use_ex_gt_assign:
            in_ext = roiaware_pool3d_utils.points_in_boxes_gpu(xyz, extend_gt_boxes[:, :, 0:7].contiguous()).long()
            ext_fg = in_ext >= 0
            idx = torch.where(box_fg, in_box, in_ext)
            if fg_pc_ignore:
                fg = ext_fg ^ box_fg
                idx = torch.where(in_box != -1, torch.full_like(idx, -1), idx)
            else:
                fg = ext_fg
        elif set_ignore_flag:
            in_ext = roiaware_pool3d_utils.points_in_boxes_gpu(xyz, extend_gt_boxes[:, :, 0:7].contiguous()).long()
            fg, idx = box_fg, in_box
            labels = torch.where(fg ^ (in_ext >= 0), torch.full_like(labels, -1), labels)
        else:
            raise NotImplementedError
        gt_of_pts = torch.gather(gt_boxes, 1, torch.where(idx < 0, idx + T, idx).unsqueeze(-1).expand(B, N, 8))
        cls_of_box = torch.ones_like(labels) if (self.num_class == 1 or binary_label) else gt_of_pts[..., -1].long()
        labels = torch.where(fg, cls_of_box, labels)
        fg = fg & (labels != 0)
        box_labels = None
        if ret_box_labels:
            enc = self.box_coder.encode_torch(gt_of_pts.reshape(B * N, 8)[:, :-1], xyz.reshape(B * N, 3),
                                              gt_classes=gt_of_pts.reshape(B * N, 8)[:, -1].long().clamp(min=1))
            box_labels = torch.where(fg.reshape(-1, 1), enc, torch.zeros_like(enc))
        return {'point_cls_labels': labels.reshape(-1), 'point_box_labels': box_labels,
                'box_idxs_labels': idx.reshape(-1), 'gt_box_of_points': gt_of_pts.reshape(B * N, 8)}

    def assign_targets(self, input_dict):
        target_cfg = self.model_cfg["TARGET_CONFIG"]
        gt_boxes = input_dict['gt_boxes']
        if gt_boxes.shape[-1] == 10:
            gt_boxes = torch.cat((gt_boxes[..., 0:7], gt_boxes[..., -1:]), dim=-1)
        B = input_dict['batch_size']
        self._bs, self._num_boxes = B, gt_boxes.shape[1]
        if _get(target_cfg, 'EXTRA_WIDTH', False):
            raise NotImplementedError("TARGET_CONFIG.EXTRA_WIDTH (enlarge_box3d_for_class)")

        fused = FUSED_HEAD_TARGETS and gt_boxes.is_cuda

        def enlarge(width):
            if fused:
                return None
            return box_utils.enlarge_box3d(gt_boxes.view(-1, gt_boxes.shape[-1]), extra_width=width).view(B, -1, gt_boxes.shape[-1])

        out = {}
        t = self.assign_stack_targets_IASSD(input_dict['centers'].detach(), gt_boxes, enlarge(target_cfg["GT_EXTRA_WIDTH"]),
                                            set_ignore_flag=True, ret_box_labels=True, extra_width=target_cfg["GT_EXTRA_WIDTH"])
        out['center_cls_labels'], out['center_box_labels'] = t['point_cls_labels'], t['point_box_labels']
        out['center_gt_box_of_points'] = t['gt_box_of_points']
        if _get(target_cfg, 'INS_AWARE_ASSIGN', False):
            preds = input_dict['sa_ins_preds']
            ext = enlarge([0.5, 0.5, 0.5])
            first = self.assign_stack_targets_IASSD(input_dict['encoder_coords'][0].reshape(-1, 4).detach(), gt_boxes, ext,
                                                    set_ignore_flag=True, extra_width=[0.5, 0.5, 0.5])
            out['get_origin_class_label'] = [first['point_cls_labels']]
            labels, boxes, coords, idxs = [], [], [], []
            for i in range(1, len(preds)):
                sa_xyz = input_dict['encoder_coords'][i]
                t = self.assign_stack_targets_IASSD(sa_xyz.reshape(-1, sa_xyz.shape[-1]).detach(), gt_boxes, ext,
                                                    set_ignore_flag=(i == 1), use_ex_gt_assign=(i >= 2), extra_width=[0.5, 0.5, 0.5])
                coords.append(sa_xyz); labels.append(t['point_cls_labels'])
                boxes.append(t['gt_box_of_points']); idxs.append(t['box_idxs_labels'])
            out.update(sa_ins_labels=labels, sa_xyz_coords=coords, sa_gt_box_of_points=boxes, sa_box_idxs_labels=idxs)
        extra = _get(target_cfg, 'ASSIGN_METHOD')
        if extra is not None:
            if extra["NAME"] != 'extend_gt':
                raise NotImplementedError(extra["NAME"])
            pts = input_dict['centers_origin' if _get(extra, 'ASSIGN_TYPE', 'centers') == 'centers_origin' else 'centers'].detach()
            t = self.assign_stack_targets_IASSD(pts, gt_boxes, enlarge(extra["EXTRA_WIDTH"]), set_ignore_flag=True,
                                                ret_box_labels=True, use_ex_gt_assign=True, extra_width=extra["EXTRA_WIDTH"],
                                                fg_pc_ignore=extra["FG_PC_IGNORE"])
            out['center_origin_cls_labels'] = t['point_cls_labels']
            out['center_origin_box_idxs_of_pts'] = t['box_idxs_labels']
            out['gt_box_of_center_origin'] = t['gt_box_of_points']
        return out

    def generate_predicted_boxes(self, points, point_cls_preds, point_box_preds):
        _, pred_classes = point_cls_preds.max(dim=-1)
        return point_cls_preds, self.box_coder.decode_torch(point_box_preds, points, pred_classes + 1)

    def forward(self, batch_dict):
        feats, centers = batch_dict['centers_features'], batch_dict['centers']
        cls_preds = self.cls_center_layers(feats)
        box_preds = self.box_center_layers(feats)
        ret = {'center_cls_preds': cls_preds, 'center_box_preds': box_preds, 'ctr_offsets': batch_dict['ctr_offsets'],
               'centers': centers, 'centers_origin': batch_dict['centers_origin'],
               'sa_ins_preds': batch_dict['sa_ins_preds'], 'sample_list_id': batch_dict.get('sample_list_id'),
               'box_iou3d_preds': None}
        if self.training:
            ret.update(self.assign_targets(batch_dict))
        loss_cfg = self.model_cfg["LOSS_CONFIG"]
        regularised = (_get(loss_cfg, "CORNER_LOSS_REGULARIZATION", False) or _get(loss_cfg, "CENTERNESS_REGULARIZATION", False)
                       or _get(loss_cfg, "IOU3D_REGULARIZATION", False))
        skip = (self.training and not self.predict_boxes_when_training and not self.decode_in_training and FUSED_HEAD_LOSS
                and feats.is_cuda and not _get(loss_cfg, "IOU3D_REGULARIZATION", False))
        if (not self.training or self.predict_boxes_when_training or regularised) and not skip:
            point_cls_preds, point_box_preds = self.generate_predicted_boxes(centers[:, 1:4], cls_preds, box_preds)
            batch_dict['batch_cls_preds'], batch_dict['batch_box_preds'] = point_cls_preds, point_box_preds
            batch_dict['box_iou3d_preds'] = None
            batch_dict['batch_index'] = centers[:, 0]
            batch_dict['cls_preds_normalized'] = False
            ret['point_box_preds'] = point_box_preds
        self.forward_ret_dict = ret
        return batch_dict

    def get_loss(self, tb_dict=None):
        tb_dict = {} if tb_dict is None else tb_dict
        cfg, tcfg = self.model_cfg["LOSS_CONFIG"], self.model_cfg["TARGET_CONFIG"]
        am = _get(tcfg, 'ASSIGN_METHOD')
        if am is not None and _get(am, 'ASSIGN_TYPE') == 'centers_origin':
            kind = _get(cfg, 'LOSS_VOTE_TYPE', 'none')
            if kind == 'ver2':
                vote = self.get_contextual_vote_loss_ver2(tb_dict)
            elif kind == 'none':
                vote = self.get_contextual_vote_loss(tb_dict)
            else:
                raise NotImplementedError("LOSS_VOTE_TYPE %s" % kind)
        else:
            raise NotImplementedError("vote loss on 'centers' assignment (get_vote_loss_loss)")
        sa = self.get_sa_ins_layer_loss(tb_dict) if _get(cfg, 'LOSS_INS') is not None else 0
        cls = self.get_center_cls_layer_loss(tb_dict)
        box = self.get_center_box_binori_layer_loss(tb_dict)
        corner = self.get_corner_layer_loss(tb_dict) if _get(cfg, 'CORNER_LOSS_REGULARIZATION', False) else 0
        return vote + cls + box + corner + sa, tb_dict

    def _weights(self):
        return self.model_cfg["LOSS_CONFIG"]["LOSS_WEIGHTS"]

    def get_contextual_vote_loss_ver2(self, tb_dict):
        r = self.forward_ret_dict
        idx, gt = r['center_origin_box_idxs_of_pts'], r['gt_box_of_center_origin']
        if FUSED_HEAD_LOSS and gt.is_cuda and self._bs * self._num_boxes <= 2048:
            loss = roiaware_pool3d_utils.head_vote_loss(1, r['centers_origin'].detach().contiguous(), r['ctr_offsets'], idx.contiguous(),
                                                        gt.contiguous(), self._bs, self._num_boxes, self.num_class,
                                                        self._weights()['vote_weight'])
            tb_dict['vote_loss_ver2'] = loss.detach()
            return loss
        pred = r['centers_origin'][:, 1:4] + r['ctr_offsets'][:, 1:4]
        B, S = self._bs, self._num_boxes
        scene = torch.arange(B, device=idx.device).repeat_interleave(idx.shape[0] // B)
        valid = idx >= 0
        seg = torch.where(valid, scene * S + idx, torch.full_like(idx, B * S))
        ones = valid.to(pred.dtype)
        cnt = torch.zeros(B * S + 1, device=pred.device, dtype=pred.dtype).index_add_(0, seg, ones)
        mean = torch.zeros(B * S + 1, 3, device=pred.device, dtype=pred.dtype).index_add_(0, seg, pred * ones[:, None])
        mean = mean / cnt.clamp(min=1.0)[:, None]
        l_gt = F.smooth_l1_loss(pred, gt[:, 0:3], reduction='none').sum(-1)
        l_mean = F.smooth_l1_loss(pred, mean.index_select(0, seg), reduction='none').sum(-1)
        per_pt = torch.where(valid, l_gt + 0.5 * l_mean, torch.zeros_like(l_gt))
        per_ins = torch.zeros(B * S + 1, device=pred.device, dtype=pred.dtype).index_add_(0, seg, per_pt) / cnt.clamp(min=1.0)
        present = (cnt[:-1] > 0).to(pred.dtype)
        loss = (per_ins[:-1] * present).sum() / present.sum().clamp(min=1.0)
        loss = loss * self._weights()['vote_weight']
        tb_dict['vote_loss_ver2'] = loss.detach()
        return loss

    def get_contextual_vote_loss(self, tb_dict):
        r = self.forward_ret_dict
        labels, gt = r['center_origin_cls_labels'], r['gt_box_of_center_origin']
        if FUSED_HEAD_LOSS and gt.is_cuda:
            loss = roiaware_pool3d_utils.head_vote_loss(0, r['centers_origin'].detach().contiguous(), r['ctr_offsets'], labels.contiguous(),
                                                        gt.contiguous(), self._bs, self._num_boxes, self.num_class,
                                                        self._weights()['vote_weight'])
            tb_dict['center_origin_loss_reg'] = loss.detach()
            return loss
        pred = r['centers_origin'][:, 1:4] + r['ctr_offsets'][:, 1:4]
        l = F.smooth_l1_loss(pred, gt[:, 0:3], reduction='none').sum(-1)
        total, present = 0, 0
        for c in range(1, self.num_class + 1):
            m = labels == c
            n = m.sum()
            total = total + torch.where(m, l, torch.zeros_like(l)).sum() / (3.0 * n.clamp(min=1))
            present = present + (n > 0).to(l.dtype)
        loss = total / present * self._weights()['vote_weight']
        tb_dict['center_origin_loss_reg'] = loss.detach()
        return loss

    @staticmethod
    def _one_hot_targets(preds, labels, num_class):
        one_hot = preds.new_zeros(*labels.shape, num_class + 1)
        one_hot.scatter_(-1, (labels * (labels >= 0).long()).unsqueeze(-1).long(), 1.0)
        return one_hot[..., 1:]

    @staticmethod
    def _cls_weights(labels):
        positives = labels > 0
        w = ((labels == 0) * 1.0 + 1.0 * positives).float()
        n = positives.sum(dim=0).float()
        return w / torch.clamp(n, min=1.0), n

    def get_center_cls_layer_loss(self, tb_dict):
        r = self.forward_ret_dict
        labels = r['center_cls_labels'].view(-1)
        preds = r['center_cls_preds'].view(-1, self.num_class)
        if FUSED_HEAD_LOSS and preds.is_cuda:
            soft = None
            if self.model_cfg["LOSS_CONFIG"]["CENTERNESS_REGULARIZATION"]:
                soft = roiaware_pool3d_utils.head_centerness(r['centers'].detach().contiguous(), r['center_gt_box_of_points'].contiguous(), labels)
            loss, n = roiaware_pool3d_utils.head_cls_loss(preds, 0, self.num_class, labels, soft, self._weights()['point_cls_weight'])
            tb_dict.update(center_loss_cls=loss.detach(), center_pos_num=n)
            return loss
        w, n = self._cls_weights(labels)
        targets = self._one_hot_targets(preds, labels, self.num_class)
        if self.model_cfg["LOSS_CONFIG"]["CENTERNESS_REGULARIZATION"]:
            targets = targets * self.generate_center_ness_mask().unsqueeze(-1)
        loss = self.cls_loss_func(preds, targets, weights=w).mean(dim=-1).sum() * self._weights()['point_cls_weight']
        tb_dict.update(center_loss_cls=loss.detach(), center_pos_num=n)
        return loss

    def generate_center_ness_mask(self):
        r = self.forward_ret_dict
        pos = r['center_cls_labels'] > 0
        gt = r['center_gt_box_of_points']
        off = r['centers'][:, 1:4].detach() - gt[:, 0:3]
        off = box_utils.rotate_points_along_z(off.unsqueeze(1), -gt[:, 6]).squeeze(1)
        template = box_utils.const_tensor(gt, 'centerness', ([1, 1, 1], [-1, -1, -1])) / 2
        margin = gt[:, None, 3:6].repeat(1, 2, 1) * template[None, :, :]
        dist = margin - off[:, None, :].repeat(1, 2, 1)
        d0, d1 = dist[:, 0, :], -dist[:, 1, :]
        c = torch.min(d0, d1) / torch.max(d0, d1)
        c = torch.pow(torch.clamp(c[:, 0] * c[:, 1] * c[:, 2], min=1e-6), 1 / 3)
        return torch.where(pos, c, torch.zeros_like(c))

    def sa_gaussian_masks(self):
        r = self.forward_ret_dict
        masks = []
        for labels, gt, coords in zip(r['sa_ins_labels'], r['sa_gt_box_of_points'], r['sa_xyz_coords']):
            if FUSED_HEAD_TARGETS and gt.is_cuda and gt.shape[-1] == 8:
                c2 = coords.detach().reshape(-1, coords.shape[-1]).contiguous()
                masks.append(roiaware_pool3d_utils.sa_gaussian_mask(c2, gt.contiguous(), labels.reshape(-1).contiguous()))
                continue
            pos = labels > 0
            xyz = coords.reshape(-1, coords.shape[-1])[:, 1:4].detach()
            off = box_utils.rotate_points_along_z((xyz - gt[:, 0:3]).unsqueeze(1), -gt[:, 6]).squeeze(1)
            w, l, h, cls = gt[:, 3], gt[:, 4], gt[:, 5], gt[:, -1]
            covs = []
            for c in (4 / (w ** 2 + l ** 2), 4 / (w ** 2 + h ** 2), 4 / (h ** 2 + l ** 2)):
                c = torch.where(cls == 1, c * 4, c)
                c = torch.where(cls == 2, c * 6, c)
                c = torch.where(cls == 3, c * 5, c)
                covs.append(c)
            v = off * torch.stack(covs, dim=-1)
            hm = torch.exp(-0.5 * (v * v).sum(-1))
            masks.append(torch.where(pos, hm, torch.zeros_like(hm)))
        return masks

    def get_sa_ins_layer_loss(self, tb_dict):
        r = self.forward_ret_dict
        labels_l, preds_l = r['sa_ins_labels'], r['sa_ins_preds']
        masks = self.sa_gaussian_masks()
        methods = self.model_cfg["LOSS_CONFIG"]["SAMPLE_METHOD_LIST"]
        ws = _get(self._weights(), 'ins_aware_weight', [1] * len(labels_l))
        total, ignore = 0, 0
        for i in range(len(labels_l)):
            if len(preds_l[i]) == 0:
                ignore += 1
                continue
            labels = labels_l[i].view(-1)
            if FUSED_HEAD_LOSS and preds_l[i].is_cuda:
                soft = masks[i] if 'ctr' in methods[i + 1][0] else None
                li, n = roiaware_pool3d_utils.head_cls_loss(preds_l[i], 1, self.num_class, labels, soft, ws[i])
                total = total + li
                tb_dict['sa%d_loss_ins' % i], tb_dict['sa%d_pos_num' % i] = li.detach(), n
                continue
            preds = preds_l[i][..., 1:].reshape(-1, self.num_class)
            w, n = self._cls_weights(labels)
            targets = self._one_hot_targets(preds, labels, self.num_class)
            if 'ctr' in methods[i + 1][0]:
                targets = targets * masks[i].unsqueeze(-1)
            li = self.ins_loss_func(preds, targets, weights=w).mean(dim=-1).sum() * ws[i]
            total = total + li
            tb_dict['sa%d_loss_ins' % i], tb_dict['sa%d_pos_num' % i] = li.detach(), n
        total = total / (len(labels_l) - ignore)
        tb_dict['sa_loss_ins'] = tb_dict['sa_loss_ins_all'] = total.detach()
        return total

    def get_center_box_binori_layer_loss(self, tb_dict):
        r = self.forward_ret_dict
        pos = r['center_cls_labels'] > 0
        labels, preds = r['center_box_labels'], r['center_box_preds']
        if FUSED_HEAD_LOSS and preds.is_cuda:
            lw = self._weights()
            loss, l_xyz, l_bin, l_res = roiaware_pool3d_utils.head_box_loss(
                preds, labels.contiguous(), r['center_cls_labels'].view(-1), self.reg_loss_func.code_weights, self.reg_loss_func.beta,
                self.box_coder.bin_size, _get(lw, 'dir_weight', 1.0), lw['point_box_weight'])
            tb_dict.update(center_loss_box=loss.detach(), center_loss_box_xyzwhl=l_xyz, center_loss_box_ori_bin=l_bin, center_loss_box_ori_res=l_res)
            return loss
        w = pos.float()
        w = w / torch.clamp(pos.sum().float(), min=1.0)
        loss_xyzwhl = self.reg_loss_func(preds[None, :, :6], labels[None, :, :6], weights=w[None]).sum()
        nb = self.box_coder.bin_size
        bin_id, bin_res = preds[:, 6:6 + nb], preds[:, 6 + nb:]
        lab_id, lab_res = labels[:, 6].long(), labels[:, 7]
        loss_cls = (F.cross_entropy(bin_id.contiguous(), lab_id.contiguous(), reduction='none') * w).sum()
        res = torch.sum(bin_res * F.one_hot(lab_id, nb).float(), dim=-1)
        loss_res = torch.sum(F.smooth_l1_loss(res, lab_res) * w)
        lw = self._weights()
        loss_cls = loss_cls * _get(lw, 'dir_weight', 1.0)
        loss = (loss_xyzwhl + loss_res + loss_cls) * lw['point_box_weight']
        tb_dict.update(center_loss_box=loss.detach(), center_loss_box_xyzwhl=loss_xyzwhl.detach(),
                       center_loss_box_ori_bin=loss_cls.detach(), center_loss_box_ori_res=loss_res.detach())
        return loss

    def get_corner_layer_loss(self, tb_dict):
        r = self.forward_ret_dict
        pos = r['center_cls_labels'] > 0
        if FUSED_HEAD_LOSS and r['center_box_preds'].is_cuda and isinstance(self.box_coder, box_coder_utils.PointResidual_BinOri_Coder):
            mean = self.box_coder._mean(r['center_box_preds']) if self.box_coder.use_mean_size else None
            loss = roiaware_pool3d_utils.head_corner_loss(r['center_box_preds'], r['centers'], r['center_cls_preds'],
                                                          r['center_gt_box_of_points'].contiguous(), r['center_cls_labels'].view(-1),
                                                          None if mean is None else mean.contiguous(), self.box_coder.bin_size,
                                                          self._weights()['corner_weight'])
            tb_dict['corner_loss_reg'] = loss.detach()
            return loss
        per_pt = loss_utils.get_corner_loss_lidar(r['point_box_preds'][:, 0:7], r['center_gt_box_of_points'][:, 0:7])
        loss = torch.where(pos, per_pt, torch.zeros_like(per_pt)).sum() / pos.sum()
        loss = loss * self._weights()['corner_weight']
        tb_dict['corner_loss_reg'] = loss.detach()
        return loss

    def compact_targets(self):
        r = self.forward_ret_dict
        out = {'center_gt_box_of_fg_points': r['center_gt_box_of_points'][r['center_cls_labels'] > 0]}
        if 'sa_ins_labels' in r:
            out['sa_gt_box_of_fg_points'] = [g[l > 0] for g, l in zip(r['sa_gt_box_of_points'], r['sa_ins_labels'])]
        if 'center_origin_cls_labels' in r:
            out['center_origin_gt_box_of_fg_points'] = r['gt_box_of_center_origin'][r['center_origin_cls_labels'] > 0]
        return out
```

pdanet_amd/param_cache.py:

```python
import weakref

import torch
import torch.nn as nn

from . import _lib


def parameters_written():
    _lib.PARAM_EPOCH[0] += 1
    _lib.WEIGHT_EPOCH[0] += 1


def buffers_written():
    _lib.PARAM_EPOCH[0] += 1


def stamp(tensors, weights_only=False):
    key = [_lib.WEIGHT_EPOCH[0] if weights_only else _lib.PARAM_EPOCH[0]]
    for t in tensors:
        key.append(None if t is None else (t.data_ptr(), t._version))
    return tuple(key)


def owning_parameter(t):
    if isinstance(t, nn.Parameter):
        return t
    base = t._base
    return base if isinstance(base, nn.Parameter) else None


class Store:

    def __init__(self, under_capture, weights_only=False):
        self.under_capture, self.weights_only = under_capture, weights_only
        self._entries = {}

    def __len__(self):
        return len(self._entries)

    def _collected(self, key, ref):
        ent = self._entries.get(key)
        if ent is not None and ent[1] is ref:
            del self._entries[key]

    def _fill(self, key, st, owner, offset, make):
        value = make()
        self._entries[key] = (st, weakref.ref(owner, lambda r: self._collected(key, r)), offset, value)
        return value

    def get(self, owner, sources, make):
        if not self.under_capture and sources[0].is_cuda and torch.cuda.is_current_stream_capturing():
            return None
        st, key = stamp(sources, self.weights_only), id(owner)
        ent = self._entries.get(key)
        if ent is not None and ent[0] == st and ent[1]() is owner:
            return ent[3]
        return self._fill(key, st, owner, 0, make)

    def get_at(self, t, make, extra=()):
        if not self.under_capture and t.is_cuda and torch.cuda.is_current_stream_capturing():
            return None
        st = stamp((t,), self.weights_only) + extra
        key = st[1][0]
        ent = self._entries.get(key)
        if ent is not None:
            held = ent[1]()
            if held is None or held.data_ptr() + ent[2] != key:
                del self._entries[key]
            elif ent[0] == st:
                return ent[3]
        owner = owning_parameter(t)
        return None if owner is None else self._fill(key, st, owner, key - owner.data_ptr(), make)
```

pdanet_amd/pointnet2_batch_cuda.py:

```python
import ctypes

import functools
import os
import threading

import torch

from . import _lib
from . import param_cache


def _chk(t, name, dtype):
    if not isinstance(t, torch.Tensor):
        raise TypeError("%s must be a torch.Tensor" % name)
    if not t.is_cuda:
        raise RuntimeError("%s must be a CUDA(HIP) tensor -- there is no CPU path" % name)
    if not t.is_contiguous():
        raise RuntimeError("%s must be contiguous" % name)
    if t.dtype != dtype:
        raise RuntimeError("%s must be %s, got %s" % (name, dtype, t.dtype))
    return t.data_ptr()


def _numel_ok(t, n, name):
# ... 726 lines not shown
          _chk(idx, "idx", I32), _chk(glob, "glob", F32), _chk(rowmap, "rowmap", I32), _chk(off, "off", I32), _chk(out, "out", F32),
          tokens, b, n, m, nsample, c, 1 if rppe_compact else 0)
    return 1


def assemble_tokens_ragged_grad(grad_out, dscale, feats, idx, cnt, off, grad_rppe, grad_dscale, grad_feats, grad_glob, tokens, b, n, m, nsample, c,
                                rppe_compact=False, rowmap=None):
    t = b * m * nsample
    if rowmap is not None:
        _numel_ok(rowmap, tokens, "rowmap")
    _numel_ok(grad_out, tokens * 4 * c, "grad_out"); _numel_ok(grad_rppe, (tokens if rppe_compact else t) * c, "grad_rppe"); _numel_ok(grad_dscale, t, "grad_dscale")
    _numel_ok(grad_feats, b * n * c, "grad_feats"); _numel_ok(grad_glob, b * m * c, "grad_glob"); _numel_ok(cnt, b * m, "cnt"); _numel_ok(off, b * m + 1, "off")
    _call("pda_assemble_tokens_ragged_grad", grad_out, _chk(grad_out, "grad_out", F32), _chk(dscale, "dscale", F32), _chk(feats, "feats", F32),
          _chk(idx, "idx", I32), _chk(cnt, "cnt", I32), _chk(off, "off", I32), None if rowmap is None else _chk(rowmap, "rowmap", I32),
          _chk(grad_rppe, "grad_rppe", F32), _chk(grad_dscale, "grad_dscale", F32), _chk(grad_feats, "grad_feats", F32),
          _chk(grad_glob, "grad_glob", F32), tokens, b, n, m, nsample, c, 1 if rppe_compact else 0)
    return 1


def add_max_pool_ragged(a, b, cnt, off, out, arg, tokens, groups, d):
    _numel_ok(a, tokens * d, "a"); _numel_ok(b, tokens * d, "b"); _numel_ok(out, groups * d, "out"); _numel_ok(arg, groups * d, "arg")
    _numel_ok(cnt, groups, "cnt"); _numel_ok(off, groups + 1, "off")
    _call("pda_add_max_pool_ragged", a, _chk(a, "a", F32), _chk(b, "b", F32), _chk(cnt, "cnt", I32), _chk(off, "off", I32),
          _chk(out, "out", F32), _chk(arg, "arg", torch.uint8), groups, d)
    return 1


def max_pool_scatter_ragged(grad_out, arg, rowmap, off, grad_x, tokens, groups, nsample, d):
    _numel_ok(grad_out, groups * d, "grad_out"); _numel_ok(arg, groups * d, "arg"); _numel_ok(grad_x, tokens * d, "grad_x")
    _numel_ok(rowmap, tokens, "rowmap"); _numel_ok(off, groups + 1, "off")
    _call("pda_max_pool_scatter_ragged", grad_out, _chk(grad_out, "grad_out", F32), _chk(arg, "arg", torch.uint8),
          _chk(rowmap, "rowmap", I32), _chk(off, "off", I32), _chk(grad_x, "grad_x", F32), tokens, groups, nsample, d)
    return 1


def group_attention_ragged_fwd(qkv, cnt, off, out, lse, tokens, num_groups, seq, heads, head_dim):
    _numel_ok(qkv, tokens * 3 * heads * head_dim, "qkv"); _numel_ok(out, tokens * heads * head_dim, "out")
    _numel_ok(lse, num_groups * heads * seq, "lse"); _numel_ok(cnt, num_groups, "cnt"); _numel_ok(off, num_groups + 1, "off")
    _call("pda_group_attention_ragged_fwd", qkv, _chk(qkv, "qkv", F32), _chk(cnt, "cnt", I32), _chk(off, "off", I32),
          _chk(out, "out", F32), _chk(lse, "lse", F32), tokens, num_groups, seq, heads, head_dim)
    return 1


def group_attention_ragged_bwd(qkv, grad_out, lse, cnt, off, grad_qkv, tokens, num_groups, seq, heads, head_dim):
    _numel_ok(qkv, tokens * 3 * heads * head_dim, "qkv"); _numel_ok(grad_qkv, tokens * 3 * heads * head_dim, "grad_qkv")
    _numel_ok(grad_out, tokens * heads * head_dim, "grad_out"); _numel_ok(lse, num_groups * heads * seq, "lse")
    _call("pda_group_attention_ragged_bwd", qkv, _chk(qkv, "qkv", F32), _chk(grad_out, "grad_out", F32), _chk(lse, "lse", F32),
          _chk(cnt, "cnt", I32), _chk(off, "off", I32), _chk(grad_qkv, "grad_qkv", F32), tokens, num_groups, seq, heads, head_dim)
    return 1


def linear_cols_pack(w, n_out, k, transposed_source=False, gather_order=False):
    lib = _lib.load()
    wf = torch.empty((_cols_packed_size(int(n_out), int(k)),), dtype=F32, device=w.device)
    _numel_ok(w, n_out * k, "w")
    _call("pda_linear_cols_pack", w, _chk(w, "w", F32), _chk(wf, "wf", F32), n_out, k, 1 if transposed_source else 0,
          1 if gather_order else 0)
    return wf


def linear_cols(x, wf, y, tokens, k, n_out):
    _numel_ok(x, tokens * k, "x"); _numel_ok(y, tokens * n_out, "y")
    _numel_ok(wf, _cols_packed_size(int(n_out), int(k)), "wf")
    _call("pda_linear_cols", x, _chk(x, "x", F32), _chk(wf, "wf", F32), _chk(y, "y", F32), tokens, k, n_out)
    return 1


def linear_split_pack(w, n_out, k, transposed_source=False):
    lib = _lib.load()
    wf = torch.empty((_split_packed_bytes(int(n_out), int(k)),), dtype=torch.uint8, device=w.device)
    _numel_ok(w, n_out * k, "w")
    _call("pda_linear_split_pack", w, _chk(w, "w", F32), _chk(wf, "wf", torch.uint8), n_out, k, 1 if transposed_source else 0)
    return wf


def linear_split_pack_both(w, n_out, k):
    wf = torch.empty((_split_packed_bytes(int(n_out), int(k)),), dtype=torch.uint8, device=w.device)
    wft = torch.empty((_split_packed_bytes(int(k), int(n_out)),), dtype=torch.uint8, device=w.device)
    _numel_ok(w, n_out * k, "w")
    _call("pda_linear_split_pack_both", w, _chk(w, "w", F32), _chk(wf, "wf", torch.uint8), _chk(wft, "wft", torch.uint8), n_out, k)
    return wf, wft


def linear_split(x, wf, bias, y, tokens, k, n_out, relu=False):
    _numel_ok(x, tokens * k, "x"); _numel_ok(y, tokens * n_out, "y")
    _numel_ok(wf, _split_packed_bytes(int(n_out), int(k)), "wf")
    if bias is not None:
        _numel_ok(bias, n_out, "bias")
    _call("pda_linear_split", x, _chk(x, "x", F32), _chk(wf, "wf", torch.uint8), None if bias is None else _chk(bias, "bias", F32),
          _chk(y, "y", F32), tokens, k, n_out, 1 if relu else 0)
    return 1


def gemm_split(x, wf, bias, y, tokens, k, n_out, relu=False, accumulate=False):
    _numel_ok(x, tokens * k, "x"); _numel_ok(y, tokens * n_out, "y")
    _numel_ok(wf, _split_packed_bytes(int(n_out), int(k)), "wf")
    if bias is not None:
        _numel_ok(bias, n_out, "bias")
    _call("pda_gemm_split", x, _chk(x, "x", F32), _chk(wf, "wf", torch.uint8), None if bias is None else _chk(bias, "bias", F32),
          _chk(y, "y", F32), tokens, k, n_out, 1 if relu else 0, 1 if accumulate else 0)
    return 1


def sa_gather_linear(xyz, new_xyz, feats_pm, idx, wf, y, b, n, m, c, nsample, n_out):
    _numel_ok(xyz, b * n * 3, "xyz"); _numel_ok(new_xyz, b * m * 3, "new_xyz"); _numel_ok(feats_pm, b * n * c, "feats_pm")
    _numel_ok(idx, b * m * nsample, "idx"); _numel_ok(y, b * m * nsample * n_out, "y")
    _numel_ok(wf, _cols_packed_size(int(n_out), 3 + int(c)), "wf")
    _call("pda_sa_gather_linear", xyz, _chk(xyz, "xyz", F32), _chk(new_xyz, "new_xyz", F32), _chk(feats_pm, "feats_pm", F32),
          _chk(idx, "idx", I32), _chk(wf, "wf", F32), _chk(y, "y", F32), b, n, m, c, nsample, n_out)
    return 1


@functools.lru_cache(maxsize=None)
def sa_small_train_workspace_bytes():
    return int(_lib.load().pda_sa_small_train_workspace_bytes())


@functools.lru_cache(maxsize=None)
def sa_small_train_supported(c, ns, c1, c2, c3, tokens):
    return bool(_lib.load().pda_sa_small_train_supported(int(c), int(ns), int(c1), int(c2), int(c3), int(tokens)))


def sa_small_train_fwd(xyz, new_xyz, feat_pm, idx, weights, gammas, betas, running_means, running_vars, eps, momentum,
                       workspace, out, zmax, arg, b, n, m, c, ns):
    c1, c2, c3 = (int(w.shape[0]) for w in weights)
    tokens = b * m * ns
    _numel_ok(xyz, b * n * 3, "xyz"); _numel_ok(new_xyz, b * m * 3, "new_xyz"); _numel_ok(idx, tokens, "idx")
    _numel_ok(out, b * m * c3, "out"); _numel_ok(zmax, b * m * c3, "zmax"); _numel_ok(arg, b * m * c3, "arg")
    _numel_ok(workspace, sa_small_train_workspace_bytes(), "workspace")
    assert weights[0].shape[1] == 3 + c and weights[1].shape[1] == c1 and weights[2].shape[1] == c2
    if feat_pm is not None:
        _numel_ok(feat_pm, b * n * c, "feat_pm")
    rm = [None if t is None else _chk(t, "running_mean", F32) for t in running_means]
    rv = [None if t is None else _chk(t, "running_var", F32) for t in running_vars]
    _buffers_written(rm[0] or rm[1] or rm[2])
    _call("pda_sa_small_train_fwd", xyz, _chk(xyz, "xyz", F32), _chk(new_xyz, "new_xyz", F32),
          None if feat_pm is None else _chk(feat_pm, "feat_pm", F32), _chk(idx, "idx", I32),
          _chk(weights[0], "w1", F32), _chk(weights[1], "w2", F32), _chk(weights[2], "w3", F32),
          _ptr_array([_chk(t, "gamma", F32) for t in gammas]), _ptr_array([_chk(t, "beta", F32) for t in betas]),
          _ptr_array(rm), _ptr_array(rv), (ctypes.c_float * 3)(*[float(e) for e in eps]),
          (ctypes.c_float * 3)(*[float(x) for x in momentum]), _chk(workspace, "workspace", torch.uint8),
          _chk(out, "out", F32), _chk(zmax, "zmax", F32), _chk(arg, "arg", torch.uint8), b, n, m, c, ns, c1, c2, c3)
    return 1


def sa_small_train_bwd(xyz, new_xyz, feat_pm, idx, grad_out, zmax, arg, workspace, dz2, dz1, dws, dgammas, dbetas, b, n, m, c, ns):
    c1, c2, c3 = (int(w.shape[0]) for w in dws)
    tokens = b * m * ns
    _numel_ok(grad_out, b * m * c3, "grad_out"); _numel_ok(dz2, tokens * c2, "dz2"); _numel_ok(dz1, tokens * c1, "dz1")
    _numel_ok(workspace, sa_small_train_workspace_bytes(), "workspace")
    _call("pda_sa_small_train_bwd", xyz, _chk(xyz, "xyz", F32), _chk(new_xyz, "new_xyz", F32),
          None if feat_pm is None else _chk(feat_pm, "feat_pm", F32), _chk(idx, "idx", I32), _chk(grad_out, "grad_out", F32),
          _chk(zmax, "zmax", F32), _chk(arg, "arg", torch.uint8), _chk(workspace, "workspace", torch.uint8),
          _chk(dz2, "dz2", F32), _chk(dz1, "dz1", F32), _chk(dws[0], "dw1", F32), _chk(dws[1], "dw2", F32), _chk(dws[2], "dw3", F32),
          _ptr_array([_chk(t, "dgamma", F32) for t in dgammas]), _ptr_array([_chk(t, "dbeta", F32) for t in dbetas]),
          b, n, m, c, ns, c1, c2, c3)
    return 1


@functools.lru_cache(maxsize=None)
def sa_xyz_grad_scratch_bytes(c1):
    return int(_lib.load().pda_sa_xyz_grad_scratch_bytes(int(c1)))


def sa_xyz_grad(grad_z1, xyz, new_xyz, idx, w, dw, grad_new_xyz, b, n, m, ns, c1):
    _numel_ok(grad_z1, b * m * ns * c1, "grad_z1"); _numel_ok(idx, b * m * ns, "idx")
# ... 52 lines not shown
```

pdanet_amd/pointnet2_utils.py:

```python
from typing import List, Tuple

import functools
import os

import torch
import torch.nn as nn
from torch.autograd import Function

from . import _lib
from . import param_cache
from . import pointnet2_batch_cuda as pointnet2

_fwd = torch.amp.custom_fwd(device_type="cuda", cast_inputs=torch.float32)
_bwd = torch.amp.custom_bwd(device_type="cuda")


class FarthestPointSampling(Function):

    @staticmethod
    @_fwd
    def forward(ctx, xyz: torch.Tensor, npoint: int) -> torch.Tensor:
        assert xyz.is_contiguous()
        B, N, _ = xyz.size()
        output = torch.empty((B, npoint), dtype=torch.int32, device=xyz.device)
# ... 489 lines not shown
        if n_out % 4 or n_in % 4:
            return False
        if max(n_out, n_in) <= 64:
            return tokens >= 4096
        return min(n_out, n_in) >= 64 and tokens >= LinearLongTokens.MIN_TOKENS

    @staticmethod
    def forward(ctx, x, weight, bias):
        ctx.save_for_backward(x, weight)
        ctx.has_bias = bias is not None
        if x.numel() // x.shape[-1] < LinearLongTokens.SPLIT_MIN_TOKENS or min(weight.shape) < 128:
            return torch.nn.functional.linear(x, weight, bias)
        return _gemm_nt(x.reshape(-1, x.shape[-1]), weight, bias).view(*x.shape[:-1], weight.shape[0])

    @staticmethod
    def backward(ctx, grad_out):
        x, weight = ctx.saved_tensors
        grad_out = grad_out.contiguous()
        gx = gw = gb = None
        if ctx.needs_input_grad[0]:
            if grad_out.numel() // grad_out.shape[-1] < LinearLongTokens.SPLIT_MIN_TOKENS or min(weight.shape) < 128:
                gx = grad_out.matmul(weight)
            else:
                gx = _gemm_nn(grad_out.reshape(-1, grad_out.shape[-1]), weight).view(*grad_out.shape[:-1], weight.shape[1])
        if ctx.needs_input_grad[1] or (ctx.has_bias and ctx.needs_input_grad[2]):
            n_out, n_in = weight.shape
            xc = x.contiguous()
            tokens = xc.numel() // n_in
            gw = torch.empty_like(weight)
            gb = torch.empty((n_out,), dtype=torch.float32, device=x.device) if ctx.has_bias else None
            pointnet2.linear_wgrad(xc, grad_out, gw, gb, tokens, n_in, n_out)
        return gx, gw, gb


DENSE_BF16 = False
BF16_MIN_TOKENS = 32768
BF16_MIN_FEATURES = 128


def _dense_bf16(x, weight=None):
    if not (DENSE_BF16 and x.is_cuda and x.dtype in (torch.float32, torch.bfloat16) and not torch.is_autocast_enabled()):
        return False
    if x.numel() // max(1, x.shape[-1]) < BF16_MIN_TOKENS:
        return False
    return weight is None or min(weight.shape[0], weight.shape[1]) >= BF16_MIN_FEATURES


def _b16(t):
    return t if t.dtype == torch.bfloat16 else t.to(torch.bfloat16)


_B16_COPIES = param_cache.Store(under_capture=False)


def _b16p(p):
    if p.dtype == torch.bfloat16:
        return p

    def cast():
        return p.detach().to(torch.bfloat16)
    pb = _B16_COPIES.get(p, (p,), cast)
    return cast() if pb is None else pb


SPLIT_GEMM = os.environ.get("PDA_SPLIT_GEMM", "1") != "0"

SPLIT_GEMM_MIN_TOKENS = 4096


def _split_gemm_ok(x2d, k):
    return (SPLIT_GEMM and x2d.is_cuda and x2d.dtype == torch.float32 and k % 32 == 0 and x2d.shape[0] >= SPLIT_GEMM_MIN_TOKENS
            and not DENSE_BF16 and not torch.is_autocast_enabled())


ROWS_IN_REGISTERS_MAX_TOKENS = int(os.environ.get("PDA_ROWS_MAX_TOKENS", "98304"))


def _rows_in_registers(tokens, k, n_out):
    return k <= 256 and n_out % 128 == 0 and n_out <= 2048 and tokens < ROWS_IN_REGISTERS_MAX_TOKENS


_PLANES = param_cache.Store(under_capture=False, weights_only=True)


def _split_planes(w, transposed=False):
    n_out, k = w.shape
    wd = w.detach()

    def pack(t):
        src = wd if wd.is_contiguous() else wd.contiguous()
        return pointnet2.linear_split_pack(src, k, n_out, transposed_source=True) if t else pointnet2.linear_split_pack(src, n_out, k)
    pair = _PLANES.get_at(w, lambda: [None, None], extra=(n_out, k)) if wd.is_contiguous() else None
    slot = 1 if transposed else 0
    if pair is not None and pair[slot] is not None:
        return pair[slot]
    if pair is None or param_cache.owning_parameter(w) is None:
        return pack(transposed)
    if w.requires_grad and n_out % 32 == 0 and k >= 128:
        pair[:] = pointnet2.linear_split_pack_both(wd, n_out, k)
    else:
        pair[slot] = pack(transposed)
    return pair[slot]


def _gemm_nt(x2d, w, bias=None, relu=False):
    n_out, k = w.shape
    if _split_gemm_ok(x2d, k) and w.dtype == torch.float32 and n_out >= 128:
        x2d = x2d.contiguous()
        T = x2d.shape[0]
        y = torch.empty((T, n_out), dtype=torch.float32, device=x2d.device)
        wf = _split_planes(w)
        bias = None if bias is None else bias.detach().contiguous()
        if _rows_in_registers(T, k, n_out):
            pointnet2.linear_split(x2d, wf, bias, y, T, k, n_out, relu=relu)
        else:
            pointnet2.gemm_split(x2d, wf, bias, y, T, k, n_out, relu=relu)
        return y
    if relu and bias is not None:
        return torch._addmm_activation(bias, x2d, w.t())
    y = torch.nn.functional.linear(x2d, w, bias)
    return torch.relu_(y) if relu else y


def _gemm_nn(g2d, w, acc=None):
    n, k_out = w.shape
    if _split_gemm_ok(g2d, n) and w.dtype == torch.float32 and k_out >= 128:
        g2d = g2d.contiguous()
        T = g2d.shape[0]
        y = acc if acc is not None else torch.empty((T, k_out), dtype=torch.float32, device=g2d.device)
        wf = _split_planes(w, transposed=True)
        if acc is None and _rows_in_registers(T, n, k_out):
            pointnet2.linear_split(g2d, wf, None, y, T, n, k_out)
        else:
            pointnet2.gemm_split(g2d, wf, None, y, T, n, k_out, accumulate=acc is not None)
        return y
    if acc is not None:
        return acc.addmm_(g2d, w)
    return g2d.mm(w)


def _mm_nt(x2d, w, bf16):
    if bf16:
        return torch.mm(_b16(x2d), _b16p(w).t(), out_dtype=torch.float32)
    return x2d.mm(w.t())


def _mm_nn(g2d, w, bf16, acc=None):
    if bf16:
        gb, wb = _b16(g2d), _b16p(w)
        if acc is not None:
            return torch.addmm(acc, gb, wb, out_dtype=torch.float32)
        return torch.mm(gb, wb, out_dtype=torch.float32)
    if acc is not None:
        return acc.addmm_(g2d, w)
    return g2d.mm(w)


def _lin(x, w, b, bf16, keep=False):
    if not bf16:
        y = torch.nn.functional.linear(x, w, b)
        return (y, x.reshape(-1, x.shape[-1])) if keep else y
    xb = _b16(x.reshape(-1, x.shape[-1]))
    y = _mm_nt(xb, w, True)
    if b is not None:
        y.add_(b)
    y = y.view(*x.shape[:-1], w.shape[0])
    return (y, xb) if keep else y


class LinearBF16(Function):
# ... 1050 lines not shown
```

pdanet_amd/roiaware_pool3d_utils.py:

```python
import torch

from .pointnet2_batch_cuda import F32, I32, _call, _chk, _numel_ok


class roiaware_pool3d_cuda:
    @staticmethod
    def points_in_boxes_gpu(boxes, pts, box_idx_of_points):
        b, t, m = boxes.shape[0], boxes.shape[1], pts.shape[1]
        _numel_ok(boxes, b * t * 7, "boxes"); _numel_ok(pts, b * m * 3, "pts")
        _numel_ok(box_idx_of_points, b * m, "box_idx_of_points")
        _call("pda_points_in_boxes", pts, _chk(boxes, "boxes", F32), _chk(pts, "pts", F32),
              _chk(box_idx_of_points, "box_idx_of_points", I32), b, t, m)
        return 1

    @staticmethod
    def forward(rois, pts, pts_feature, argmax, pts_idx_of_voxels, pooled_features, pool_method):
        n, p, c = rois.shape[0], pts.shape[0], pts_feature.shape[1]
        ox, oy, oz, k = (int(v) for v in pts_idx_of_voxels.shape[1:5])
        _numel_ok(rois, n * 7, "rois"); _numel_ok(pts, p * 3, "pts"); _numel_ok(pts_feature, p * c, "pts_feature")
        _numel_ok(argmax, n * ox * oy * oz * c, "argmax"); _numel_ok(pooled_features, n * ox * oy * oz * c, "pooled_features")
        _numel_ok(pts_idx_of_voxels, n * ox * oy * oz * k, "pts_idx_of_voxels")
        _call("pda_roiaware_pool3d_fwd", pts_feature, _chk(rois, "rois", F32), _chk(pts, "pts", F32),
              _chk(pts_feature, "pts_feature", F32), _chk(argmax, "argmax", I32), _chk(pts_idx_of_voxels, "pts_idx_of_voxels", I32),
              _chk(pooled_features, "pooled_features", F32), n, p, c, k, ox, oy, oz, int(pool_method))
        if p == 0 and int(pool_method) == 0:
            argmax.fill_(-1)
        return 1

    @staticmethod
    def backward(pts_idx_of_voxels, argmax, grad_out, grad_in, pool_method):
        n, ox, oy, oz, k = (int(v) for v in pts_idx_of_voxels.shape)
        c, p = int(grad_out.shape[4]), int(grad_in.shape[0])
        _numel_ok(argmax, n * ox * oy * oz * c, "argmax"); _numel_ok(grad_out, n * ox * oy * oz * c, "grad_out")
        _numel_ok(pts_idx_of_voxels, n * ox * oy * oz * k, "pts_idx_of_voxels"); _numel_ok(grad_in, p * c, "grad_in")
        _call("pda_roiaware_pool3d_bwd", grad_out, _chk(pts_idx_of_voxels, "pts_idx_of_voxels", I32), _chk(argmax, "argmax", I32),
              _chk(grad_out, "grad_out", F32), _chk(grad_in, "grad_in", F32), n, p, c, k, ox, oy, oz, int(pool_method))
        return 1

    @staticmethod
    def points_in_boxes_cpu(boxes, pts, pts_indices):
        n, p = boxes.shape[0], pts.shape[0]
        _numel_ok(boxes, n * 7, "boxes"); _numel_ok(pts, p * 3, "pts"); _numel_ok(pts_indices, n * p, "pts_indices")
        _call("pda_points_in_boxes_mask", pts, _chk(boxes, "boxes", F32), _chk(pts, "pts", F32),
              _chk(pts_indices, "pts_indices", I32), n, p)
        return 1


def points_in_boxes_count(points, boxes):
    if points.dim() != 2 or points.shape[1] < 4 or boxes.dim() != 3 or boxes.shape[2] < 7:
        raise ValueError("points must be (N, >= 4) and boxes (B, M, >= 7), got %s and %s" % (tuple(points.shape), tuple(boxes.shape)))
    points = points.detach().contiguous()
    boxes = boxes.detach()[..., :7].contiguous()
    B, M = boxes.shape[0], boxes.shape[1]
    counts = torch.zeros((B, M), dtype=I32, device=boxes.device)
    _call("pda_points_in_boxes_count", boxes, _chk(points, "points", F32), int(points.shape[1]), _chk(boxes, "boxes", F32),
          _chk(counts, "counts", I32), int(points.shape[0]), B, M)
    return counts


def points_in_boxes_gpu(points, boxes):
    assert boxes.shape[0] == points.shape[0]
    assert boxes.shape[2] == 7 and points.shape[2] == 3
    batch_size, num_points, _ = points.shape
    box_idxs_of_pts = points.new_zeros((batch_size, num_points), dtype=torch.int).fill_(-1)
    roiaware_pool3d_cuda.points_in_boxes_gpu(boxes.contiguous(), points.contiguous(), box_idxs_of_pts)
    return box_idxs_of_pts


def assign_point_targets(gt_boxes, in_box, in_ext, mode, single_class):
    B, T = gt_boxes.shape[0], gt_boxes.shape[1]
    N = in_box.shape[1]
    _numel_ok(gt_boxes, B * T * 8, "gt_boxes"); _numel_ok(in_ext, B * N, "in_ext")
    labels = torch.empty((B * N,), dtype=torch.int64, device=gt_boxes.device)
    idx = torch.empty((B * N,), dtype=torch.int64, device=gt_boxes.device)
    gt_of = torch.empty((B * N, 8), dtype=torch.float32, device=gt_boxes.device)
    _call("pda_assign_point_targets", gt_boxes, _chk(gt_boxes, "gt_boxes", F32), _chk(in_box, "in_box", I32), _chk(in_ext, "in_ext", I32),
          _chk(labels, "labels", torch.int64), _chk(idx, "box_idx", torch.int64), _chk(gt_of, "gt_of_points", F32), B, N, T, int(mode),
          int(bool(single_class)))
    return labels, idx, gt_of


def head_assign_targets(points, gt_boxes, extra_width, mode, single_class, mean_size=None, bins=0, ret_box_labels=False):
    import ctypes
    B, T = gt_boxes.shape[0], gt_boxes.shape[1]
    P = points.shape[0]
    N = P // B
    dev = gt_boxes.device
    labels = torch.empty((P,), dtype=torch.int64, device=dev)
    idx = torch.empty((P,), dtype=torch.int64, device=dev)
    gt_of = torch.empty((P, 8), dtype=torch.float32, device=dev)
    box_labels = torch.empty((P, 8), dtype=torch.float32, device=dev) if ret_box_labels else None
    ew = (ctypes.c_float * 3)(*[float(w) for w in extra_width])
    _call("pda_head_assign_targets", gt_boxes, _chk(points, "points", F32), int(points.shape[1]), 1, _chk(gt_boxes, "gt_boxes", F32), ew,
          _chk(labels, "labels", torch.int64), _chk(idx, "box_idx", torch.int64), _chk(gt_of, "gt_of_points", F32),
          None if box_labels is None else _chk(box_labels, "box_labels", F32), None if mean_size is None else _chk(mean_size, "mean_size", F32),
          int(bins), B, N, T, int(mode), int(bool(single_class)))
    return labels, idx, gt_of, box_labels


def sa_gaussian_mask(coords, gt_of_points, labels):
    P = gt_of_points.shape[0]
    _numel_ok(coords, P * coords.shape[-1], "coords"); _numel_ok(labels, P, "labels")
    out = torch.empty((P,), dtype=torch.float32, device=gt_of_points.device)
    _call("pda_sa_gaussian_mask", gt_of_points, _chk(coords, "coords", F32), int(coords.shape[-1]), 1, _chk(gt_of_points, "gt_of_points", F32),
          _chk(labels, "labels", torch.int64), _chk(out, "out", F32), P)
    return out


I64 = torch.int64


def head_centerness(centers, gt_of_points, labels):
    n = gt_of_points.shape[0]
    out = torch.empty((n,), dtype=torch.float32, device=gt_of_points.device)
    _call("pda_head_centerness", gt_of_points, _chk(centers, "centers", F32), _chk(gt_of_points, "gt_of_points", F32),
          _chk(labels, "labels", I64), _chk(out, "out", F32), n)
    return out


class _ScaledGrad(torch.autograd.Function):

    @staticmethod
    def forward(ctx, run, *preds):
        outs, grads = run()
        ctx.save_for_backward(*grads)
        ctx.mark_non_differentiable(*outs[1:])
        return tuple(outs)

    @staticmethod
    def backward(ctx, g0, *unused):
        return (None,) + tuple(g * g0 for g in ctx.saved_tensors)


def head_cls_loss(preds, col0, num_class, labels, soft, scale):
    p2 = preds.reshape(-1, preds.shape[-1])
    p2 = p2 if p2.is_contiguous() else p2.contiguous()
    n, cols = p2.shape

    def run():
        out = torch.empty((2,), dtype=torch.float32, device=p2.device)
        grad = torch.empty_like(p2)
        _call("pda_head_cls_loss", p2, _chk(p2.detach(), "preds", F32), cols, int(col0), int(num_class), _chk(labels, "labels", I64),
              None if soft is None else _chk(soft, "soft", F32), n, float(scale), _chk(out, "out", F32), _chk(grad, "grad", F32))
        return (out[0], out[1]), (grad.view(preds.shape),)
    return _ScaledGrad.apply(run, preds)


def head_box_loss(preds, labels, cls_labels, code_weights, beta, bins, dir_weight, box_weight):
    p2 = preds if preds.is_contiguous() else preds.contiguous()
    n = p2.shape[0]

    def run():
        out = torch.empty((4,), dtype=torch.float32, device=p2.device)
        grad = torch.empty_like(p2)
        _call("pda_head_box_loss", p2, _chk(p2.detach(), "preds", F32), _chk(labels, "labels", F32), _chk(cls_labels, "cls_labels", I64),
              None if code_weights is None else _chk(code_weights, "code_weights", F32), float(beta), int(bins), float(dir_weight),
              float(box_weight), n, _chk(out, "out", F32), _chk(grad, "grad", F32))
        return (out[0], out[1], out[2], out[3]), (grad,)
    return _ScaledGrad.apply(run, preds)


def head_vote_loss(mode, origin, offsets, key, gt, batch_size, boxes, num_class, weight):
    o2 = offsets if offsets.is_contiguous() else offsets.contiguous()
    n = o2.shape[0]

    def run():
        out = torch.empty((1,), dtype=torch.float32, device=o2.device)
        grad = torch.empty_like(o2)
        _call("pda_head_vote_loss", o2, int(mode), _chk(origin, "origin", F32), _chk(o2.detach(), "offsets", F32), _chk(key, "key", I64),
              _chk(gt, "gt", F32), int(batch_size), int(boxes), int(num_class), float(weight), n, _chk(out, "out", F32), _chk(grad, "grad", F32))
        return (out[0],), (grad,)
    return _ScaledGrad.apply(run, offsets)[0]


def head_corner_loss(box_preds, centers, cls_preds, gt, cls_labels, mean_size, bins, weight):
    b2 = box_preds if box_preds.is_contiguous() else box_preds.contiguous()
    c2 = centers if centers.is_contiguous() else centers.contiguous()
    k2 = cls_preds.detach().reshape(b2.shape[0], -1).contiguous()
    n = b2.shape[0]

    def run():
        out = torch.empty((1,), dtype=torch.float32, device=b2.device)
        gb, gc = torch.empty_like(b2), torch.empty_like(c2)
        _call("pda_head_corner_loss", b2, _chk(b2.detach(), "box_preds", F32), _chk(c2.detach(), "centers", F32), _chk(k2, "cls_preds", F32),
              int(k2.shape[1]), _chk(gt, "gt", F32), _chk(cls_labels, "cls_labels", I64),
              None if mean_size is None else _chk(mean_size, "mean_size", F32), int(bins), float(weight), n, _chk(out, "out", F32),
              _chk(gb, "grad_box", F32), _chk(gc, "grad_centers", F32))
        return (out[0],), (gb, gc)
    return _ScaledGrad.apply(run, box_preds, centers)[0]


def points_in_boxes_cpu(points, boxes):
    import numpy as np
    assert boxes.shape[1] == 7
    assert points.shape[1] == 3
    is_numpy = isinstance(points, np.ndarray)
    points = torch.from_numpy(points).float() if is_numpy else points
    boxes = torch.from_numpy(boxes).float() if isinstance(boxes, np.ndarray) else boxes
    home = points.device
    dev = home if home.type == "cuda" else (boxes.device if boxes.is_cuda else torch.device("cuda", torch.cuda.current_device()))
    point_indices = torch.zeros((boxes.shape[0], points.shape[0]), dtype=torch.int, device=dev)
    roiaware_pool3d_cuda.points_in_boxes_cpu(boxes.to(dev).float().contiguous(), points.to(dev).float().contiguous(), point_indices)
    return point_indices.cpu().numpy() if is_numpy else point_indices.to(home)


class RoIAwarePool3d(torch.nn.Module):
    def __init__(self, out_size, max_pts_each_voxel=128):
        super().__init__()
        self.out_size = out_size
        self.max_pts_each_voxel = max_pts_each_voxel

    def forward(self, rois, pts, pts_feature, pool_method='max'):
        assert pool_method in ['max', 'avg']
        return RoIAwarePool3dFunction.apply(rois, pts, pts_feature, self.out_size, self.max_pts_each_voxel, pool_method)


class RoIAwarePool3dFunction(torch.autograd.Function):
    @staticmethod
    def forward(ctx, rois, pts, pts_feature, out_size, max_pts_each_voxel, pool_method):
        assert rois.shape[1] == 7 and pts.shape[1] == 3
        if isinstance(out_size, int):
            out_x = out_y = out_z = out_size
        else:
            assert len(out_size) == 3
            for k in range(3):
                assert isinstance(out_size[k], int)
            out_x, out_y, out_z = out_size
        num_rois, num_channels, num_pts = rois.shape[0], pts_feature.shape[-1], pts.shape[0]
        pooled_features = pts_feature.new_zeros((num_rois, out_x, out_y, out_z, num_channels))
        argmax = pts_feature.new_zeros((num_rois, out_x, out_y, out_z, num_channels), dtype=torch.int)
        pts_idx_of_voxels = pts_feature.new_zeros((num_rois, out_x, out_y, out_z, max_pts_each_voxel), dtype=torch.int)
        pool_method = {'max': 0, 'avg': 1}[pool_method]
        roiaware_pool3d_cuda.forward(rois.contiguous(), pts.contiguous(), pts_feature.contiguous(), argmax, pts_idx_of_voxels,
                                     pooled_features, pool_method)
        ctx.roiaware_pool3d_for_backward = (pts_idx_of_voxels, argmax, pool_method, num_pts, num_channels)
        return pooled_features

    @staticmethod
    def backward(ctx, grad_out):
        pts_idx_of_voxels, argmax, pool_method, num_pts, num_channels = ctx.roiaware_pool3d_for_backward
        grad_in = grad_out.new_zeros((num_pts, num_channels))
        roiaware_pool3d_cuda.backward(pts_idx_of_voxels, argmax, grad_out.contiguous(), grad_in, pool_method)
        return None, None, grad_in, None, None, None
```

Before: 124.8 scenes/s.

## Batch head losses, target assignment and weight repacking into grouped launches

Adds grouped kernels that run several head loss terms (cls, box, corner) in one launch with one block per term. It also adds a grouped target-assignment call and a grouped split-weight repack that refreshes all stale packed planes at once after an optimizer step. The aim is to cut kernel launch count and Python/ctypes dispatch overhead in a launch-bound small-batch training step. In exchange the loss computations are deferred until the context exits, and per-call argument structs get larger.

```diff
diff --git a/include/pda_pointnet2.h b/include/pda_pointnet2.h
--- a/include/pda_pointnet2.h
+++ b/include/pda_pointnet2.h
@@ -97,6 +97,12 @@
 int64_t pda_linear_split_packed_bytes(int n_out, int k);
 int pda_linear_split_pack(const float *w, void *wf, int n_out, int k, int transposed_source, pda_stream_t stream);
 int pda_linear_split_pack_both(const float *w, void *wf, void *wft, int n_out, int k, pda_stream_t stream);
+typedef struct pda_split_pack_entry {
+    const float *w;
+    void *wf, *wft;
+    int32_t n_out, k;
+} pda_split_pack_entry_t;
+int pda_linear_split_pack_grouped(const pda_split_pack_entry_t *entries, int count, pda_stream_t stream);
 int pda_linear_split(const float *x, const void *wf, const float *bias, float *y, int64_t tokens, int k, int n_out,
                      int relu, pda_stream_t stream);
 int pda_gemm_split(const float *x, const void *wf, const float *bias, float *y, int64_t tokens, int k, int n_out,
diff --git a/include/pda_train.h b/include/pda_train.h
--- a/include/pda_train.h
+++ b/include/pda_train.h
@@ -218,6 +218,16 @@
 int pda_head_assign_targets(const float *points, int point_stride, int point_offset, const float *gt_boxes, const float *extra_width,
                             int64_t *labels, int64_t *box_idx, float *gt_of_points, float *box_labels, const float *mean_size,
                             int bins, int b, int n, int t, int mode, int single_class, pda_stream_t stream);
+typedef struct pda_head_targets_problem {
+    const float *points;
+    int64_t *labels, *box_idx;
+    float *gt_of_points, *box_labels;
+    const float *mean_size;
+    float extra_width[3];
+    int32_t point_stride, point_offset, n, bins, mode, single_class;
+} pda_head_targets_problem_t;
+int pda_head_assign_targets_grouped(const pda_head_targets_problem_t *problems, int count, const float *gt_boxes, int b, int t,
+                                    pda_stream_t stream);
 int pda_sa_gaussian_mask(const float *coords, int stride, int offset, const float *gt_of_points, const int64_t *labels,
                          float *out, int64_t points, pda_stream_t stream);
 
@@ -246,6 +256,16 @@
 int pda_head_corner_loss(const float *box_preds, const float *centers, const float *cls_preds, int num_class, const float *gt,
                          const int64_t *cls_labels, const float *mean_size, int bins, float weight, int64_t n, float *out1,
                          float *grad_box, float *grad_centers, pda_stream_t stream);
+enum { PDA_HEAD_LOSS_CLS = 0, PDA_HEAD_LOSS_BOX = 1, PDA_HEAD_LOSS_CORNER = 2 };
+typedef struct pda_head_loss_entry {
+    int32_t kind, row_stride, col0, num_class, bins;
+    float weight, beta, dir_weight;
+    int64_t n;
+    const float *preds, *aux, *gt, *cls_preds, *table;
+    const int64_t *labels;
+    float *out, *grad, *grad2;
+} pda_head_loss_entry_t;
+int pda_head_loss_grouped(const pda_head_loss_entry_t *entries, int count, pda_stream_t stream);
 
 int64_t pda_sa_small_train_workspace_bytes(void);
 int pda_sa_small_train_supported(int c, int nsample, int c1, int c2, int c3, int64_t tokens);
diff --git a/pdanet_amd/_lib.py b/pdanet_amd/_lib.py
--- a/pdanet_amd/_lib.py
+++ b/pdanet_amd/_lib.py
@@ -34,6 +34,24 @@
     _fields_ = [("kind", ctypes.c_int32), ("count", ctypes.c_int32), ("part", ctypes.c_void_p), ("part_bias", ctypes.c_void_p),
                 ("dst", ctypes.c_void_p), ("dst_bias", ctypes.c_void_p), ("nm", ctypes.c_int64), ("n", ctypes.c_int32),
                 ("cols", ctypes.c_int32), ("ld", ctypes.c_int64)]
+
+
+class HeadTargetsProblem(ctypes.Structure):
+    _fields_ = [("points", ctypes.c_void_p), ("labels", ctypes.c_void_p), ("box_idx", ctypes.c_void_p),
+                ("gt_of_points", ctypes.c_void_p), ("box_labels", ctypes.c_void_p), ("mean_size", ctypes.c_void_p),
+                ("extra_width", ctypes.c_float * 3), ("point_stride", ctypes.c_int32), ("point_offset", ctypes.c_int32),
+                ("n", ctypes.c_int32), ("bins", ctypes.c_int32), ("mode", ctypes.c_int32), ("single_class", ctypes.c_int32)]
+
+
+class HeadLossEntry(ctypes.Structure):
+    _fields_ = [(n, ctypes.c_int32) for n in ("kind", "row_stride", "col0", "num_class", "bins")] + \
+               [(n, ctypes.c_float) for n in ("weight", "beta", "dir_weight")] + [("n", ctypes.c_int64)] + \
+               [(n, ctypes.c_void_p) for n in ("preds", "aux", "gt", "cls_preds", "table", "labels", "out", "grad", "grad2")]
+
+
+class SplitPackEntry(ctypes.Structure):
+    _fields_ = [("w", ctypes.c_void_p), ("wf", ctypes.c_void_p), ("wft", ctypes.c_void_p), ("n_out", ctypes.c_int32),
+                ("k", ctypes.c_int32)]
 
 
 PARAM_EPOCH = [0]
@@ -78,6 +96,7 @@
     "pda_linear_split_packed_bytes": [_i, _i],
     "pda_linear_split_pack": [_vp, _vp, _i, _i, _i, _vp],
     "pda_linear_split_pack_both": [_vp, _vp, _vp, _i, _i, _vp],
+    "pda_linear_split_pack_grouped": [ctypes.POINTER(SplitPackEntry), _i, _vp],
     "pda_linear_split": [_vp, _vp, _vp, _vp, ctypes.c_int64, _i, _i, _i, _vp],
     "pda_gemm_split": [_vp, _vp, _vp, _vp, ctypes.c_int64, _i, _i, _i, _i, _vp],
     "pda_sa_mlp_packed_size": [_i, _i, _i],
@@ -148,6 +167,8 @@
     "pda_assign_point_targets": [_vp, _vp, _vp, _vp, _vp, _vp, _i, _i, _i, _i, _i, _vp],
     "pda_sa_gaussian_mask": [_vp, _i, _i, _vp, _vp, _vp, ctypes.c_int64, _vp],
     "pda_head_assign_targets": [_vp, _i, _i, _vp, ctypes.POINTER(ctypes.c_float), _vp, _vp, _vp, _vp, _vp, _i, _i, _i, _i, _i, _i, _vp],
+    "pda_head_assign_targets_grouped": [ctypes.POINTER(HeadTargetsProblem), _i, _vp, _i, _i, _vp],
+    "pda_head_loss_grouped": [ctypes.POINTER(HeadLossEntry), _i, _vp],
     "pda_head_cls_loss": [_vp, _i, _i, _i, _vp, _vp, ctypes.c_int64, _f, _vp, _vp, _vp],
     "pda_head_centerness": [_vp, _vp, _vp, _vp, ctypes.c_int64, _vp],
     "pda_head_box_loss": [_vp, _vp, _vp, _vp, _f, _i, _f, _f, ctypes.c_int64, _vp, _vp, _vp],
diff --git a/pdanet_amd/csrc/gemm_split.hip b/pdanet_amd/csrc/gemm_split.hip
--- a/pdanet_amd/csrc/gemm_split.hip
+++ b/pdanet_amd/csrc/gemm_split.hip
@@ -39,6 +39,31 @@
         if (o < total) split_pack_one(w, wf, o, n_out, k, KS, 0);
         else split_pack_one(w, wft, o - total, k, n_out, KSt, 1);
     }
+}
+
+constexpr int SP_MAX_ENTRIES = 48;
+
+struct SplitPackArgs {
+    pda_split_pack_entry_t e[SP_MAX_ENTRIES];
+    int first[SP_MAX_ENTRIES + 1];
+    int count;
+};
+
+static int64_t split_pack_threads(int rows, int cols) { return (int64_t)divup(rows, 128) * (divup(cols, 32) * 2) * 4 * 64 * 4; }
+
+__global__ __launch_bounds__(256) void split_pack_grouped_kernel(const SplitPackArgs a) {
+    const int b = (int)blockIdx.x;
+    int lo = 0, hi = a.count;
+    while (hi - lo > 1) {
+        const int mid = (lo + hi) >> 1;
+        if (a.first[mid] <= b) lo = mid; else hi = mid;
+    }
+    const pda_split_pack_entry_t& e = a.e[lo];
+    const int KS = (e.k + 31) / 32 * 2, KSt = (e.n_out + 31) / 32 * 2;
+    const int64_t total = e.wf ? (int64_t)((e.n_out + 127) / 128) * KS * 4 * 64 * 4 : 0;
+    const int64_t o = (int64_t)(b - a.first[lo]) * 256 + threadIdx.x;
+    if (o < total) split_pack_one(e.w, (uint32_t*)e.wf, o, e.n_out, e.k, KS, 0);
+    else split_pack_one(e.w, (uint32_t*)e.wft, o - total, e.k, e.n_out, KSt, 1);
 }
 
 struct LinSplitParams {
@@ -616,6 +641,35 @@
     return pda::check_launch("pda_linear_split_pack_both");
 }
 
+PDA_API int pda_linear_split_pack_grouped(const pda_split_pack_entry_t* entries, int count, pda_stream_t stream) {
+    PDA_REQUIRE(count >= 1, "pda_linear_split_pack_grouped: bad size: count=%d", count);
+    PDA_REQUIRE(entries, "pda_linear_split_pack_grouped: null pointer");
+    for (int i = 0; i < count; ++i) {
+        const pda_split_pack_entry_t& e = entries[i];
+        PDA_REQUIRE(e.n_out > 0 && e.k > 0, "pda_linear_split_pack_grouped: bad size: entry %d: n_out=%d k=%d", i, e.n_out, e.k);
+        PDA_REQUIRE(e.w && (e.wf || e.wft), "pda_linear_split_pack_grouped: entry %d: null pointer", i);
+        PDA_REQUIRE((pda::split_pack_threads(e.n_out, e.k) + pda::split_pack_threads(e.k, e.n_out)) / 256 < ((int64_t)1 << 30),
+                    "pda_linear_split_pack_grouped: bad size: entry %d: n_out=%d k=%d", i, e.n_out, e.k);
+    }
+    for (int i0 = 0; i0 < count; ) {
+        pda::SplitPackArgs a;
+        a.count = 0;
+        int64_t blocks = 0;
+        for (; i0 < count && a.count < pda::SP_MAX_ENTRIES; ++i0) {
+            const pda_split_pack_entry_t& e = entries[i0];
+            const int64_t nb = ((e.wf ? pda::split_pack_threads(e.n_out, e.k) : 0) + (e.wft ? pda::split_pack_threads(e.k, e.n_out) : 0)) / 256;
+            if (a.count > 0 && blocks + nb >= ((int64_t)1 << 31)) break;
+            a.first[a.count] = (int)blocks;
+            a.e[a.count++] = e;
+            blocks += nb;
+        }
+        for (int i = a.count; i < pda::SP_MAX_ENTRIES; ++i) { a.first[i] = (int)blocks; a.e[i] = pda_split_pack_entry_t{}; }
+        a.first[pda::SP_MAX_ENTRIES] = (int)blocks;
+        hipLaunchKernelGGL(pda::split_pack_grouped_kernel, dim3((unsigned)blocks), dim3(256), 0, (hipStream_t)stream, a);
+    }
+    return pda::check_launch("pda_linear_split_pack_grouped");
+}
+
 PDA_API int pda_linear_split(const float* x, const void* wf, const float* bias, float* y, int64_t tokens, int k, int n_out,
                              int relu, pda_stream_t stream) {
     PDA_REQUIRE(tokens >= 0 && k > 0 && n_out > 0, "pda_linear_split: bad size");
diff --git a/pdanet_amd/csrc/head_loss.hip b/pdanet_amd/csrc/head_loss.hip
--- a/pdanet_amd/csrc/head_loss.hip
+++ b/pdanet_amd/csrc/head_loss.hip
@@ -28,11 +28,9 @@
     return n - 0.5f * beta;
 }
 
-__global__ __launch_bounds__(HL_THREADS) void head_cls_loss_kernel(const float* __restrict__ preds, int row_stride, int col0, int C,
-                                                                   const int64_t* __restrict__ labels, const float* __restrict__ soft,
-                                                                   int64_t n, float scale, float* __restrict__ out,
-                                                                   float* __restrict__ grad) {
-    __shared__ double red[17];
+__device__ __forceinline__ void head_cls_loss_term(const float* __restrict__ preds, int row_stride, int col0, int C,
+                                                   const int64_t* __restrict__ labels, const float* __restrict__ soft, int64_t n,
+                                                   float scale, float* __restrict__ out, float* __restrict__ grad, double* red) {
     double cnt = 0;
     for (int64_t r = threadIdx.x; r < n; r += HL_THREADS) cnt += labels[r] > 0 ? 1.0 : 0.0;
     const double npos = hl_block_sum(cnt, red);
@@ -61,6 +59,14 @@
     if (threadIdx.x == 0) { out[0] = scale * (float)total; out[1] = (float)npos; }
 }
 
+__global__ __launch_bounds__(HL_THREADS) void head_cls_loss_kernel(const float* __restrict__ preds, int row_stride, int col0, int C,
+                                                                   const int64_t* __restrict__ labels, const float* __restrict__ soft,
+                                                                   int64_t n, float scale, float* __restrict__ out,
+                                                                   float* __restrict__ grad) {
+    __shared__ double red[17];
+    head_cls_loss_term(preds, row_stride, col0, C, labels, soft, n, scale, out, grad, red);
+}
+
 __global__ __launch_bounds__(256) void head_centerness_kernel(const float* __restrict__ centers, const float* __restrict__ gt,
                                                               const int64_t* __restrict__ labels, float* __restrict__ out, int64_t n) {
     const int64_t p = (int64_t)blockIdx.x * 256 + threadIdx.x;
@@ -80,11 +86,10 @@
     out[p] = labels[p] > 0 ? powf(fmaxf(prod, 1e-6f), 1.f / 3.f) : 0.f;
 }
 
-__global__ __launch_bounds__(HL_THREADS) void head_box_loss_kernel(const float* __restrict__ preds, const float* __restrict__ labels,
-                                                                   const int64_t* __restrict__ cls_labels, const float* __restrict__ code_w,
-                                                                   float beta, int nb, float dir_w, float box_w, int64_t n,
-                                                                   float* __restrict__ out, float* __restrict__ grad) {
-    __shared__ double red[17];
+__device__ __forceinline__ void head_box_loss_term(const float* __restrict__ preds, const float* __restrict__ labels,
+                                                   const int64_t* __restrict__ cls_labels, const float* __restrict__ code_w, float beta,
+                                                   int nb, float dir_w, float box_w, int64_t n, float* __restrict__ out,
+                                                   float* __restrict__ grad, double* red) {
     const int W = 6 + 2 * nb;
     double cnt = 0, sres = 0;
     for (int64_t r = threadIdx.x; r < n; r += HL_THREADS) {
@@ -131,6 +136,14 @@
         const double res = res_mean * sumw;
         out[0] = (float)((xyz + res + cls) * box_w); out[1] = (float)xyz; out[2] = (float)cls; out[3] = (float)res;
     }
+}
+
+__global__ __launch_bounds__(HL_THREADS) void head_box_loss_kernel(const float* __restrict__ preds, const float* __restrict__ labels,
+                                                                   const int64_t* __restrict__ cls_labels, const float* __restrict__ code_w,
+                                                                   float beta, int nb, float dir_w, float box_w, int64_t n,
+                                                                   float* __restrict__ out, float* __restrict__ grad) {
+    __shared__ double red[17];
+    head_box_loss_term(preds, labels, cls_labels, code_w, beta, nb, dir_w, box_w, n, out, grad, red);
 }
 
 constexpr int HL_MAX_SEG = 2048;
@@ -210,12 +223,11 @@
     }
 }
 
-__global__ __launch_bounds__(HL_THREADS) void head_corner_loss_kernel(const float* __restrict__ box_preds, const float* __restrict__ centers,
-                                                                      const float* __restrict__ cls_preds, int C, const float* __restrict__ gt,
-                                                                      const int64_t* __restrict__ cls_labels, const float* __restrict__ mean_size,
-                                                                      int nb, float weight, int64_t n, float* __restrict__ out,
-                                                                      float* __restrict__ grad_box, float* __restrict__ grad_ctr) {
-    __shared__ double red[17];
+__device__ __forceinline__ void head_corner_loss_term(const float* __restrict__ box_preds, const float* __restrict__ centers,
+                                                      const float* __restrict__ cls_preds, int C, const float* __restrict__ gt,
+                                                      const int64_t* __restrict__ cls_labels, const float* __restrict__ mean_size, int nb,
+                                                      float weight, int64_t n, float* __restrict__ out, float* __restrict__ grad_box,
+                                                      float* __restrict__ grad_ctr, double* red) {
     const int W = 6 + 2 * nb;
     const float PI = 3.14159265358979323846f;
     const float inter = 2.f * PI / (float)nb;
@@ -281,6 +293,38 @@
     if (threadIdx.x == 0) out[0] = (float)(total / npos) * weight;
 }
 
+__global__ __launch_bounds__(HL_THREADS) void head_corner_loss_kernel(const float* __restrict__ box_preds, const float* __restrict__ centers,
+                                                                      const float* __restrict__ cls_preds, int C, const float* __restrict__ gt,
+                                                                      const int64_t* __restrict__ cls_labels, const float* __restrict__ mean_size,
+                                                                      int nb, float weight, int64_t n, float* __restrict__ out,
+                                                                      float* __restrict__ grad_box, float* __restrict__ grad_ctr) {
+    __shared__ double red[17];
+    head_corner_loss_term(box_preds, centers, cls_preds, C, gt, cls_labels, mean_size, nb, weight, n, out, grad_box, grad_ctr, red);
+}
+
+constexpr int HL_MAX_TERMS = 16;
+
+struct HeadLossArgs {
+    pda_head_loss_entry_t e[HL_MAX_TERMS];
+};
+
+__global__ __launch_bounds__(HL_THREADS) void head_loss_grouped_kernel(const HeadLossArgs a) {
+    __shared__ double red[17];
+    const pda_head_loss_entry_t& e = a.e[blockIdx.x];
+    switch (e.kind) {
+    case PDA_HEAD_LOSS_CLS:
+        head_cls_loss_term(e.preds, e.row_stride, e.col0, e.num_class, e.labels, e.aux, e.n, e.weight, e.out, e.grad, red);
+        break;
+    case PDA_HEAD_LOSS_BOX:
+        head_box_loss_term(e.preds, e.aux, e.labels, e.table, e.beta, e.bins, e.dir_weight, e.weight, e.n, e.out, e.grad, red);
+        break;
+    default:
+        head_corner_loss_term(e.preds, e.aux, e.cls_preds, e.num_class, e.gt, e.labels, e.table, e.bins, e.weight, e.n, e.out, e.grad,
+                              e.grad2, red);
+        break;
+    }
+}
+
 }
 
 PDA_API int pda_head_cls_loss(const float* preds, int row_stride, int col0, int num_class, const int64_t* labels, const float* soft,
@@ -332,3 +376,37 @@
                        num_class, gt, cls_labels, mean_size, bins, weight, n, out1, grad_box, grad_centers);
     return pda::check_launch("pda_head_corner_loss");
 }
+
+PDA_API int pda_head_loss_grouped(const pda_head_loss_entry_t* entries, int count, pda_stream_t stream) {
+    PDA_REQUIRE(count >= 1, "pda_head_loss_grouped: bad size: count=%d", count);
+    PDA_REQUIRE(entries, "pda_head_loss_grouped: null pointer");
+    for (int i = 0; i < count; ++i) {
+        const pda_head_loss_entry_t& e = entries[i];
+        switch (e.kind) {
+        case PDA_HEAD_LOSS_CLS:
+            PDA_REQUIRE(e.n >= 0 && e.num_class >= 1 && e.col0 >= 0 && e.col0 + e.num_class <= e.row_stride,
+                        "pda_head_loss_grouped: entry %d (cls): bad shape", i);
+            PDA_REQUIRE(e.preds && e.labels && e.out && e.grad, "pda_head_loss_grouped: entry %d (cls): null pointer", i);
+            break;
+        case PDA_HEAD_LOSS_BOX:
+            PDA_REQUIRE(e.n >= 1 && e.bins >= 1 && e.bins <= 64, "pda_head_loss_grouped: entry %d (box): n=%lld bins=%d", i, (long long)e.n, e.bins);
+            PDA_REQUIRE(e.preds && e.aux && e.labels && e.out && e.grad, "pda_head_loss_grouped: entry %d (box): null pointer", i);
+            break;
+        case PDA_HEAD_LOSS_CORNER:
+            PDA_REQUIRE(e.n >= 1 && e.bins >= 1 && e.bins <= 64 && e.num_class >= 1, "pda_head_loss_grouped: entry %d (corner): n=%lld bins=%d", i,
+                        (long long)e.n, e.bins);
+            PDA_REQUIRE(e.preds && e.aux && e.cls_preds && e.gt && e.labels && e.out && e.grad && e.grad2,
+                        "pda_head_loss_grouped: entry %d (corner): null pointer", i);
+            break;
+        default:
+            PDA_REQUIRE(false, "pda_head_loss_grouped: bad size: entry %d: kind=%d", i, e.kind);
+        }
+    }
+    for (int i0 = 0; i0 < count; i0 += pda::HL_MAX_TERMS) {
+        pda::HeadLossArgs a;
+        const int m = count - i0 < pda::HL_MAX_TERMS ? count - i0 : pda::HL_MAX_TERMS;
+        for (int i = 0; i < pda::HL_MAX_TERMS; ++i) a.e[i] = i < m ? entries[i0 + i] : pda_head_loss_entry_t{};
+        hipLaunchKernelGGL(pda::head_loss_grouped_kernel, dim3(m), dim3(pda::HL_THREADS), 0, (hipStream_t)stream, a);
+    }
+    return pda::check_launch("pda_head_loss_grouped");
+}
diff --git a/pdanet_amd/csrc/head_targets.hip b/pdanet_amd/csrc/head_targets.hip
--- a/pdanet_amd/csrc/head_targets.hip
+++ b/pdanet_amd/csrc/head_targets.hip
@@ -54,15 +54,13 @@
     double lim_x, lim_y, lim_xe, lim_ye;
 };
 
-__global__ __launch_bounds__(256) void head_assign_targets_kernel(const float* __restrict__ pts, int pstride, int poff,
-                                                                  const float* __restrict__ gt_boxes, float ex, float ey, float ez,
-                                                                  int64_t* __restrict__ labels, int64_t* __restrict__ box_idx,
-                                                                  float* __restrict__ gt_of_points, float* __restrict__ box_labels,
-                                                                  const float* __restrict__ mean_size, int bins, int n, int t, int mode,
-                                                                  int single_class) {
-    __shared__ HtBoxRec rec[256];
-    const int bs = blockIdx.y;
-    const int pt = blockIdx.x * 256 + threadIdx.x;
+__device__ __forceinline__ void head_assign_targets_block(const float* __restrict__ pts, int pstride, int poff,
+                                                          const float* __restrict__ gt_boxes, float ex, float ey, float ez,
+                                                          int64_t* __restrict__ labels, int64_t* __restrict__ box_idx,
+                                                          float* __restrict__ gt_of_points, float* __restrict__ box_labels,
+                                                          const float* __restrict__ mean_size, int bins, int n, int t, int mode,
+                                                          int single_class, int bs, int blk, HtBoxRec* rec) {
+    const int pt = blk * 256 + threadIdx.x;
     const bool live = pt < n;
     float x = 0.f, y = 0.f, z = 0.f;
     if (live) {
@@ -159,6 +157,41 @@
     }
 }
 
+__global__ __launch_bounds__(256) void head_assign_targets_kernel(const float* __restrict__ pts, int pstride, int poff,
+                                                                  const float* __restrict__ gt_boxes, float ex, float ey, float ez,
+                                                                  int64_t* __restrict__ labels, int64_t* __restrict__ box_idx,
+                                                                  float* __restrict__ gt_of_points, float* __restrict__ box_labels,
+                                                                  const float* __restrict__ mean_size, int bins, int n, int t, int mode,
+                                                                  int single_class) {
+    __shared__ HtBoxRec rec[256];
+    head_assign_targets_block(pts, pstride, poff, gt_boxes, ex, ey, ez, labels, box_idx, gt_of_points, box_labels, mean_size, bins, n, t,
+                              mode, single_class, blockIdx.y, blockIdx.x, rec);
+}
+
+constexpr int HT_MAX_PROBLEMS = 16;
+
+struct HeadTargetsArgs {
+    pda_head_targets_problem_t p[HT_MAX_PROBLEMS];
+    int first[HT_MAX_PROBLEMS + 1];
+    int count;
+    int t;
+    const float* gt_boxes;
+};
+
+__global__ __launch_bounds__(256) void head_assign_targets_grouped_kernel(const HeadTargetsArgs a) {
+    __shared__ HtBoxRec rec[256];
+    const int b = (int)blockIdx.x;
+    int lo = 0, hi = a.count;
+    while (hi - lo > 1) {
+        const int mid = (lo + hi) >> 1;
+        if (a.first[mid] <= b) lo = mid; else hi = mid;
+    }
+    const pda_head_targets_problem_t& p = a.p[lo];
+    head_assign_targets_block(p.points, p.point_stride, p.point_offset, a.gt_boxes, p.extra_width[0], p.extra_width[1], p.extra_width[2],
+                              p.labels, p.box_idx, p.gt_of_points, p.box_labels, p.mean_size, p.bins, p.n, a.t, p.mode, p.single_class,
+                              blockIdx.y, b - a.first[lo], rec);
+}
+
 }
 
 PDA_API int pda_assign_point_targets(const float* gt_boxes, const int32_t* in_box, const int32_t* in_ext, int64_t* labels,
@@ -201,3 +234,36 @@
                        mean_size, bins, n, t, mode, single_class);
     return pda::check_launch("pda_head_assign_targets");
 }
+
+PDA_API int pda_head_assign_targets_grouped(const pda_head_targets_problem_t* problems, int count, const float* gt_boxes, int b, int t,
+                                            pda_stream_t stream) {
+    PDA_REQUIRE(count >= 1 && b >= 0 && b <= 65535 && t >= 1, "pda_head_assign_targets_grouped: bad size: count=%d b=%d boxes=%d", count, b, t);
+    PDA_REQUIRE(problems && gt_boxes && ((uintptr_t)gt_boxes & 15) == 0, "pda_head_assign_targets_grouped: null or misaligned gt_boxes");
+    for (int i = 0; i < count; ++i) {
+        const pda_head_targets_problem_t& p = problems[i];
+        PDA_REQUIRE(p.n >= 0 && p.mode >= 0 && p.mode <= 2 && p.point_stride >= 3 && p.point_offset >= 0 && p.point_offset + 3 <= p.point_stride,
+                    "pda_head_assign_targets_grouped: bad size: problem %d: n=%d mode=%d stride=%d", i, p.n, p.mode, p.point_stride);
+        if (p.n == 0 || b == 0) continue;
+        PDA_REQUIRE(p.points && p.labels && p.box_idx && p.gt_of_points, "pda_head_assign_targets_grouped: problem %d: null pointer", i);
+        PDA_REQUIRE((((uintptr_t)p.gt_of_points | (uintptr_t)p.box_labels) & 15) == 0,
+                    "pda_head_assign_targets_grouped: problem %d: gt_of_points / box_labels must be 16-byte aligned", i);
+        PDA_REQUIRE(!p.box_labels || (p.bins >= 1 && p.bins <= 64), "pda_head_assign_targets_grouped: problem %d: bins=%d", i, p.bins);
+    }
+    if (b == 0) return PDA_OK;
+    for (int i0 = 0; i0 < count; i0 += pda::HT_MAX_PROBLEMS) {
+        pda::HeadTargetsArgs a;
+        a.count = 0; a.t = t; a.gt_boxes = gt_boxes;
+        int blocks = 0;
+        for (int i = i0; i < count && i < i0 + pda::HT_MAX_PROBLEMS; ++i) {
+            if (problems[i].n == 0) continue;
+            a.first[a.count] = blocks;
+            a.p[a.count++] = problems[i];
+            blocks += pda::divup(problems[i].n, 256);
+        }
+        for (int i = a.count; i < pda::HT_MAX_PROBLEMS; ++i) { a.first[i] = blocks; a.p[i] = pda_head_targets_problem_t{}; }
+        a.first[pda::HT_MAX_PROBLEMS] = blocks;
+        if (blocks == 0) continue;
+        hipLaunchKernelGGL(pda::head_assign_targets_grouped_kernel, dim3(blocks, b), dim3(256), 0, (hipStream_t)stream, a);
+    }
+    return pda::check_launch("pda_head_assign_targets_grouped");
+}
diff --git a/pdanet_amd/iassd_head.py b/pdanet_amd/iassd_head.py
--- a/pdanet_amd/iassd_head.py
+++ b/pdanet_amd/iassd_head.py
@@ -13,6 +13,7 @@
 
 
 FUSED_HEAD_TARGETS = True
+HEAD_TARGETS_GROUPED = os.environ.get("PDA_HEAD_TARGETS_GROUPED", "1") != "0"
 
 FUSED_HEAD_LOSS = os.environ.get("PDA_FUSED_HEAD_LOSS", "1") != "0"
 
@@ -132,37 +133,71 @@
                 return None
             return box_utils.enlarge_box3d(gt_boxes.view(-1, gt_boxes.shape[-1]), extra_width=width).view(B, -1, gt_boxes.shape[-1])
 
-        out = {}
-        t = self.assign_stack_targets_IASSD(input_dict['centers'].detach(), gt_boxes, enlarge(target_cfg["GT_EXTRA_WIDTH"]),
-                                            set_ignore_flag=True, ret_box_labels=True, extra_width=target_cfg["GT_EXTRA_WIDTH"])
-        out['center_cls_labels'], out['center_box_labels'] = t['point_cls_labels'], t['point_box_labels']
-        out['center_gt_box_of_points'] = t['gt_box_of_points']
+        calls = []
+
+        def want(points, ext, **flags):
+            calls.append((points, ext, flags))
+            return len(calls) - 1
+
+        i_center = want(input_dict['centers'].detach(), enlarge(target_cfg["GT_EXTRA_WIDTH"]),
+                        set_ignore_flag=True, ret_box_labels=True, extra_width=target_cfg["GT_EXTRA_WIDTH"])
+        i_first, i_sa, coords = None, [], []
         if _get(target_cfg, 'INS_AWARE_ASSIGN', False):
             preds = input_dict['sa_ins_preds']
             ext = enlarge([0.5, 0.5, 0.5])
-            first = self.assign_stack_targets_IASSD(input_dict['encoder_coords'][0].reshape(-1, 4).detach(), gt_boxes, ext,
-                                                    set_ignore_flag=True, extra_width=[0.5, 0.5, 0.5])
-            out['get_origin_class_label'] = [first['point_cls_labels']]
-            labels, boxes, coords, idxs = [], [], [], []
+            i_first = want(input_dict['encoder_coords'][0].reshape(-1, 4).detach(), ext,
+                           set_ignore_flag=True, extra_width=[0.5, 0.5, 0.5])
             for i in range(1, len(preds)):
                 sa_xyz = input_dict['encoder_coords'][i]
-                t = self.assign_stack_targets_IASSD(sa_xyz.reshape(-1, sa_xyz.shape[-1]).detach(), gt_boxes, ext,
-                                                    set_ignore_flag=(i == 1), use_ex_gt_assign=(i >= 2), extra_width=[0.5, 0.5, 0.5])
-                coords.append(sa_xyz); labels.append(t['point_cls_labels'])
-                boxes.append(t['gt_box_of_points']); idxs.append(t['box_idxs_labels'])
-            out.update(sa_ins_labels=labels, sa_xyz_coords=coords, sa_gt_box_of_points=boxes, sa_box_idxs_labels=idxs)
-        extra = _get(target_cfg, 'ASSIGN_METHOD')
+                i_sa.append(want(sa_xyz.reshape(-1, sa_xyz.shape[-1]).detach(), ext,
+                                 set_ignore_flag=(i == 1), use_ex_gt_assign=(i >= 2), extra_width=[0.5, 0.5, 0.5]))
+                coords.append(sa_xyz)
+        extra, i_extra = _get(target_cfg, 'ASSIGN_METHOD'), None
         if extra is not None:
             if extra["NAME"] != 'extend_gt':
                 raise NotImplementedError(extra["NAME"])
             pts = input_dict['centers_origin' if _get(extra, 'ASSIGN_TYPE', 'centers') == 'centers_origin' else 'centers'].detach()
-            t = self.assign_stack_targets_IASSD(pts, gt_boxes, enlarge(extra["EXTRA_WIDTH"]), set_ignore_flag=True,
-                                                ret_box_labels=True, use_ex_gt_assign=True, extra_width=extra["EXTRA_WIDTH"],
-                                                fg_pc_ignore=extra["FG_PC_IGNORE"])
+            i_extra = want(pts, enlarge(extra["EXTRA_WIDTH"]), set_ignore_flag=True,
+                           ret_box_labels=True, use_ex_gt_assign=True, extra_width=extra["EXTRA_WIDTH"],
+                           fg_pc_ignore=extra["FG_PC_IGNORE"])
+        res = self._assign_all(calls, gt_boxes)
+
+        out = {}
+        t = res[i_center]
+        out['center_cls_labels'], out['center_box_labels'] = t['point_cls_labels'], t['point_box_labels']
+        out['center_gt_box_of_points'] = t['gt_box_of_points']
+        if i_first is not None:
+            out['get_origin_class_label'] = [res[i_first]['point_cls_labels']]
+            out.update(sa_ins_labels=[res[i]['point_cls_labels'] for i in i_sa], sa_xyz_coords=coords,
+                       sa_gt_box_of_points=[res[i]['gt_box_of_points'] for i in i_sa],
+                       sa_box_idxs_labels=[res[i]['box_idxs_labels'] for i in i_sa])
+        if i_extra is not None:
+            t = res[i_extra]
             out['center_origin_cls_labels'] = t['point_cls_labels']
             out['center_origin_box_idxs_of_pts'] = t['box_idxs_labels']
             out['gt_box_of_center_origin'] = t['gt_box_of_points']
         return out
+
+    def _assign_all(self, calls, gt_boxes):
+        def fused(points, flags):
+            return (FUSED_HEAD_TARGETS and points.is_cuda and flags.get('extra_width') is not None
+                    and (flags.get('use_ex_gt_assign', False) or flags.get('set_ignore_flag', True)))
+        if not (HEAD_TARGETS_GROUPED and len(calls) > 1 and gt_boxes.is_cuda and all(fused(p, f) for p, _, f in calls)):
+            return [self.assign_stack_targets_IASSD(p, gt_boxes, ext, **f) for p, ext, f in calls]
+        coder, B = self.box_coder, gt_boxes.shape[0]
+        problems = []
+        for p, _, f in calls:
+            assert p.dim() == 2 and p.shape[1] == 4 and p.shape[0] % B == 0, "scenes must contribute equally many points"
+            ret_box = f.get('ret_box_labels', False)
+            use_ex = f.get('use_ex_gt_assign', False)
+            problems.append(dict(points=p.contiguous(), extra_width=f['extra_width'],
+                                 mode=(2 if f.get('fg_pc_ignore', False) else 1) if use_ex else 0,
+                                 single_class=self.num_class == 1 or f.get('binary_label', False),
+                                 mean_size=coder._mean(gt_boxes).contiguous() if (ret_box and coder.use_mean_size) else None,
+                                 bins=coder.bin_size, ret_box_labels=ret_box))
+        assert gt_boxes.dim() == 3 and gt_boxes.shape[2] == 8
+        return [{'point_cls_labels': labels, 'point_box_labels': box_labels, 'box_idxs_labels': idx, 'gt_box_of_points': gt_of_pts}
+                for labels, idx, gt_of_pts, box_labels in roiaware_pool3d_utils.head_assign_targets_multi(problems, gt_boxes.contiguous())]
 
     def generate_predicted_boxes(self, points, point_cls_preds, point_box_preds):
         _, pred_classes = point_cls_preds.max(dim=-1)
@@ -197,20 +232,22 @@
         tb_dict = {} if tb_dict is None else tb_dict
         cfg, tcfg = self.model_cfg["LOSS_CONFIG"], self.model_cfg["TARGET_CONFIG"]
         am = _get(tcfg, 'ASSIGN_METHOD')
-        if am is not None and _get(am, 'ASSIGN_TYPE') == 'centers_origin':
-            kind = _get(cfg, 'LOSS_VOTE_TYPE', 'none')
-            if kind == 'ver2':
-                vote = self.get_contextual_vote_loss_ver2(tb_dict)
-            elif kind == 'none':
-                vote = self.get_contextual_vote_loss(tb_dict)
+        with roiaware_pool3d_utils.head_loss_group():
+            if am is not None and _get(am, 'ASSIGN_TYPE') == 'centers_origin':
+                kind = _get(cfg, 'LOSS_VOTE_TYPE', 'none')
+                if kind == 'ver2':
+                    vote = self.get_contextual_vote_loss_ver2(tb_dict)
+                elif kind == 'none':
+                    vote = self.get_contextual_vote_loss(tb_dict)
+                else:
+                    raise NotImplementedError("LOSS_VOTE_TYPE %s" % kind)
             else:
-                raise NotImplementedError("LOSS_VOTE_TYPE %s" % kind)
-        else:
-            raise NotImplementedError("vote loss on 'centers' assignment (get_vote_loss_loss)")
-        sa = self.get_sa_ins_layer_loss(tb_dict) if _get(cfg, 'LOSS_INS') is not None else 0
-        cls = self.get_center_cls_layer_loss(tb_dict)
-        box = self.get_center_box_binori_layer_loss(tb_dict)
-        corner = self.get_corner_layer_loss(tb_dict) if _get(cfg, 'CORNER_LOSS_REGULARIZATION', False) else 0
+                raise NotImplementedError("vote loss on 'centers' assignment (get_vote_loss_loss)")
+            sa_terms = self._sa_ins_layer_terms(tb_dict) if _get(cfg, 'LOSS_INS') is not None else None
+            cls = self.get_center_cls_layer_loss(tb_dict)
+            box = self.get_center_box_binori_layer_loss(tb_dict)
+            corner = self.get_corner_layer_loss(tb_dict) if _get(cfg, 'CORNER_LOSS_REGULARIZATION', False) else 0
+        sa = self._sa_ins_layer_total(sa_terms, tb_dict) if sa_terms is not None else 0
         return vote + cls + box + corner + sa, tb_dict
 
     def _weights(self):
@@ -335,12 +372,15 @@
         return masks
 
     def get_sa_ins_layer_loss(self, tb_dict):
+        return self._sa_ins_layer_total(self._sa_ins_layer_terms(tb_dict), tb_dict)
+
+    def _sa_ins_layer_terms(self, tb_dict):
         r = self.forward_ret_dict
         labels_l, preds_l = r['sa_ins_labels'], r['sa_ins_preds']
         masks = self.sa_gaussian_masks()
         methods = self.model_cfg["LOSS_CONFIG"]["SAMPLE_METHOD_LIST"]
         ws = _get(self._weights(), 'ins_aware_weight', [1] * len(labels_l))
-        total, ignore = 0, 0
+        terms, ignore = [], 0
         for i in range(len(labels_l)):
             if len(preds_l[i]) == 0:
                 ignore += 1
@@ -349,7 +389,7 @@
             if FUSED_HEAD_LOSS and preds_l[i].is_cuda:
                 soft = masks[i] if 'ctr' in methods[i + 1][0] else None
                 li, n = roiaware_pool3d_utils.head_cls_loss(preds_l[i], 1, self.num_class, labels, soft, ws[i])
-                total = total + li
+                terms.append(li)
                 tb_dict['sa%d_loss_ins' % i], tb_dict['sa%d_pos_num' % i] = li.detach(), n
                 continue
             preds = preds_l[i][..., 1:].reshape(-1, self.num_class)
@@ -358,9 +398,17 @@
             if 'ctr' in methods[i + 1][0]:
                 targets = targets * masks[i].unsqueeze(-1)
             li = self.ins_loss_func(preds, targets, weights=w).mean(dim=-1).sum() * ws[i]
+            terms.append(li)
+            tb_dict['sa%d_loss_ins' % i], tb_dict['sa%d_pos_num' % i] = li.detach(), n
+        return terms, len(labels_l) - ignore
+
+    @staticmethod
+    def _sa_ins_layer_total(terms_and_count, tb_dict):
+        terms, count = terms_and_count
+        total = 0
+        for li in terms:
             total = total + li
-            tb_dict['sa%d_loss_ins' % i], tb_dict['sa%d_pos_num' % i] = li.detach(), n
-        total = total / (len(labels_l) - ignore)
+        total = total / count
         tb_dict['sa_loss_ins'] = tb_dict['sa_loss_ins_all'] = total.detach()
         return total
 
diff --git a/pdanet_amd/param_cache.py b/pdanet_amd/param_cache.py
--- a/pdanet_amd/param_cache.py
+++ b/pdanet_amd/param_cache.py
@@ -71,3 +71,23 @@
                 return ent[3]
         owner = owning_parameter(t)
         return None if owner is None else self._fill(key, st, owner, key - owner.data_ptr(), make)
+
+    def stale_at(self):
+        if not self.under_capture and torch.cuda.is_available() and torch.cuda.is_current_stream_capturing():
+            return []
+        epoch = _lib.WEIGHT_EPOCH[0] if self.weights_only else _lib.PARAM_EPOCH[0]
+        out = []
+        for key, ent in list(self._entries.items()):
+            st = ent[0]
+            if len(st) < 2 or not isinstance(st[1], tuple) or st[1][0] != key:
+                continue
+            held = ent[1]()
+            if held is None or held.data_ptr() + ent[2] != key:
+                del self._entries[key]
+            elif st[0] != epoch or st[1][1] != held._version:
+                out.append((key, held, st[2:], ent[3]))
+        return out
+
+    def put_at(self, key, owner, extra, value):
+        st = (_lib.WEIGHT_EPOCH[0] if self.weights_only else _lib.PARAM_EPOCH[0], (key, owner._version)) + tuple(extra)
+        self._entries[key] = (st, weakref.ref(owner, lambda r: self._collected(key, r)), key - owner.data_ptr(), value)
diff --git a/pdanet_amd/pointnet2_batch_cuda.py b/pdanet_amd/pointnet2_batch_cuda.py
--- a/pdanet_amd/pointnet2_batch_cuda.py
+++ b/pdanet_amd/pointnet2_batch_cuda.py
@@ -832,6 +832,27 @@
     return wf, wft
 
 
+def linear_split_pack_grouped(weights, device):
+    sizes = [(_split_packed_bytes(int(n), int(k)) if fwd else 0, _split_packed_bytes(int(k), int(n)) if tr else 0)
+             for _, n, k, fwd, tr in weights]
+    arena = torch.empty((sum(a + b for a, b in sizes),), dtype=torch.uint8, device=device)
+    entries, out, off = [], [], 0
+    for (w, n, k, fwd, tr), (a, b) in zip(weights, sizes):
+        if not (fwd or tr):
+            raise ValueError("linear_split_pack_grouped: an entry wants neither form")
+        if isinstance(w, torch.Tensor):
+            _numel_ok(w, n * k, "w")
+            w = _chk(w, "w", F32)
+        wf = arena[off:off + a] if fwd else None
+        wft = arena[off + a:off + a + b] if tr else None
+        off += a + b
+        entries.append(_lib.SplitPackEntry(w, None if wf is None else wf.data_ptr(), None if wft is None else wft.data_ptr(), int(n), int(k)))
+        out.append((wf, wft))
+    if entries:
+        _call("pda_linear_split_pack_grouped", arena, (_lib.SplitPackEntry * len(entries))(*entries), len(entries))
+    return out
+
+
 def linear_split(x, wf, bias, y, tokens, k, n_out, relu=False):
     _numel_ok(x, tokens * k, "x"); _numel_ok(y, tokens * n_out, "y")
     _numel_ok(wf, _split_packed_bytes(int(n_out), int(k)), "wf")
diff --git a/pdanet_amd/pointnet2_utils.py b/pdanet_amd/pointnet2_utils.py
--- a/pdanet_amd/pointnet2_utils.py
+++ b/pdanet_amd/pointnet2_utils.py
@@ -595,10 +595,29 @@
 
 _PLANES = param_cache.Store(under_capture=False, weights_only=True)
 
+SPLIT_PACK_GROUPED = os.environ.get("PDA_SPLIT_PACK_GROUPED", "1") != "0"
+_REPACKED_AT = {}
+
+
+def _repack_stale_planes(device):
+    stale = [(key, owner, extra, pair) for key, owner, extra, pair in _PLANES.stale_at()
+             if owner.device == device and owner.dtype == torch.float32 and len(extra) == 2
+             and (pair[0] is not None or pair[1] is not None)]
+    if not stale:
+        return
+    packed = pointnet2.linear_split_pack_grouped([(key, extra[0], extra[1], pair[0] is not None, pair[1] is not None)
+                                                  for key, owner, extra, pair in stale], device)
+    for (key, owner, extra, _), planes in zip(stale, packed):
+        _PLANES.put_at(key, owner, extra, list(planes))
+
 
 def _split_planes(w, transposed=False):
     n_out, k = w.shape
     wd = w.detach()
+    if SPLIT_PACK_GROUPED and w.is_cuda and _REPACKED_AT.get(w.device.index) != _lib.WEIGHT_EPOCH[0] \
+            and not torch.cuda.is_current_stream_capturing():
+        _REPACKED_AT[w.device.index] = _lib.WEIGHT_EPOCH[0]
+        _repack_stale_planes(w.device)
 
     def pack(t):
         src = wd if wd.is_contiguous() else wd.contiguous()
diff --git a/pdanet_amd/roiaware_pool3d_utils.py b/pdanet_amd/roiaware_pool3d_utils.py
--- a/pdanet_amd/roiaware_pool3d_utils.py
+++ b/pdanet_amd/roiaware_pool3d_utils.py
@@ -1,5 +1,10 @@
+import ctypes
+import os
+import threading
+
 import torch
 
+from . import _lib
 from .pointnet2_batch_cuda import F32, I32, _call, _chk, _numel_ok
 
 
@@ -98,6 +103,30 @@
     return labels, idx, gt_of, box_labels
 
 
+def head_assign_targets_multi(problems, gt_boxes):
+    B, T = gt_boxes.shape[0], gt_boxes.shape[1]
+    dev = gt_boxes.device
+    gt = _chk(gt_boxes, "gt_boxes", F32)
+    _numel_ok(gt_boxes, B * T * 8, "gt_boxes")
+    entries, results = [], []
+    for p in problems:
+        points, mean_size = p["points"], p.get("mean_size")
+        P = points.shape[0]
+        labels = torch.empty((P,), dtype=torch.int64, device=dev)
+        idx = torch.empty((P,), dtype=torch.int64, device=dev)
+        gt_of = torch.empty((P, 8), dtype=torch.float32, device=dev)
+        box_labels = torch.empty((P, 8), dtype=torch.float32, device=dev) if p.get("ret_box_labels") else None
+        entries.append(_lib.HeadTargetsProblem(
+            _chk(points, "points", F32), labels.data_ptr(), idx.data_ptr(), gt_of.data_ptr(),
+            None if box_labels is None else box_labels.data_ptr(), None if mean_size is None else _chk(mean_size, "mean_size", F32),
+            (ctypes.c_float * 3)(*[float(w) for w in p["extra_width"]]), int(points.shape[1]), 1, P // B, int(p.get("bins", 0)),
+            int(p["mode"]), int(bool(p["single_class"]))))
+        results.append((labels, idx, gt_of, box_labels))
+    if entries:
+        _call("pda_head_assign_targets_grouped", gt_boxes, (_lib.HeadTargetsProblem * len(entries))(*entries), len(entries), gt, B, T)
+    return results
+
+
 def sa_gaussian_mask(coords, gt_of_points, labels):
     P = gt_of_points.shape[0]
     _numel_ok(coords, P * coords.shape[-1], "coords"); _numel_ok(labels, P, "labels")
@@ -132,6 +161,47 @@
         return (None,) + tuple(g * g0 for g in ctx.saved_tensors)
 
 
+HEAD_LOSS_GROUPED = os.environ.get("PDA_HEAD_LOSS_GROUPED", "1") != "0"
+_TLS = threading.local()
+LOSS_GROUP_STATS = {"grouped_calls": 0, "entries": 0}
+_CLS, _BOX, _CORNER = 0, 1, 2
+
+
+class head_loss_group:
+    def __init__(self):
+        self.entries, self.keep = [], []
+
+    def __enter__(self):
+        if HEAD_LOSS_GROUPED and _open_loss_group() is None:
+            _TLS.group = self
+        return self
+
+    def __exit__(self, exc_type, exc, tb):
+        if _open_loss_group() is self:
+            _TLS.group = None
+            if exc_type is None:
+                self.flush()
+            self.entries, self.keep = [], []
+        return False
+
+    def add(self, tensors, **fields):
+        self.entries.append(_lib.HeadLossEntry(**fields))
+        self.keep.extend(t for t in tensors if t is not None)
+
+    def flush(self):
+        if not self.entries:
+            return
+        arr = (_lib.HeadLossEntry * len(self.entries))(*self.entries)
+        _call("pda_head_loss_grouped", self.keep[0], arr, len(self.entries))
+        LOSS_GROUP_STATS["grouped_calls"] += 1
+        LOSS_GROUP_STATS["entries"] += len(self.entries)
+        self.entries, self.keep = [], []
+
+
+def _open_loss_group():
+    return getattr(_TLS, "group", None)
+
+
 def head_cls_loss(preds, col0, num_class, labels, soft, scale):
     p2 = preds.reshape(-1, preds.shape[-1])
     p2 = p2 if p2.is_contiguous() else p2.contiguous()
@@ -140,8 +210,14 @@
     def run():
         out = torch.empty((2,), dtype=torch.float32, device=p2.device)
         grad = torch.empty_like(p2)
-        _call("pda_head_cls_loss", p2, _chk(p2.detach(), "preds", F32), cols, int(col0), int(num_class), _chk(labels, "labels", I64),
-              None if soft is None else _chk(soft, "soft", F32), n, float(scale), _chk(out, "out", F32), _chk(grad, "grad", F32))
+        group = _open_loss_group()
+        if group is not None:
+            group.add((p2, labels, soft, out, grad), kind=_CLS, preds=_chk(p2.detach(), "preds", F32), row_stride=cols, col0=int(col0),
+                      num_class=int(num_class), labels=_chk(labels, "labels", I64), aux=None if soft is None else _chk(soft, "soft", F32),
+                      n=n, weight=float(scale), out=_chk(out, "out", F32), grad=_chk(grad, "grad", F32))
+        else:
+            _call("pda_head_cls_loss", p2, _chk(p2.detach(), "preds", F32), cols, int(col0), int(num_class), _chk(labels, "labels", I64),
+                  None if soft is None else _chk(soft, "soft", F32), n, float(scale), _chk(out, "out", F32), _chk(grad, "grad", F32))
         return (out[0], out[1]), (grad.view(preds.shape),)
     return _ScaledGrad.apply(run, preds)
 
@@ -153,9 +229,16 @@
     def run():
         out = torch.empty((4,), dtype=torch.float32, device=p2.device)
         grad = torch.empty_like(p2)
-        _call("pda_head_box_loss", p2, _chk(p2.detach(), "preds", F32), _chk(labels, "labels", F32), _chk(cls_labels, "cls_labels", I64),
-              None if code_weights is None else _chk(code_weights, "code_weights", F32), float(beta), int(bins), float(dir_weight),
-              float(box_weight), n, _chk(out, "out", F32), _chk(grad, "grad", F32))
+        cw = None if code_weights is None else _chk(code_weights, "code_weights", F32)
+        group = _open_loss_group()
+        if group is not None:
+            group.add((p2, labels, cls_labels, code_weights, out, grad), kind=_BOX, preds=_chk(p2.detach(), "preds", F32),
+                      aux=_chk(labels, "labels", F32), labels=_chk(cls_labels, "cls_labels", I64), table=cw, beta=float(beta),
+                      bins=int(bins), dir_weight=float(dir_weight), weight=float(box_weight), n=n, out=_chk(out, "out", F32),
+                      grad=_chk(grad, "grad", F32))
+        else:
+            _call("pda_head_box_loss", p2, _chk(p2.detach(), "preds", F32), _chk(labels, "labels", F32), _chk(cls_labels, "cls_labels", I64),
+                  cw, float(beta), int(bins), float(dir_weight), float(box_weight), n, _chk(out, "out", F32), _chk(grad, "grad", F32))
         return (out[0], out[1], out[2], out[3]), (grad,)
     return _ScaledGrad.apply(run, preds)
 
@@ -182,10 +265,17 @@
     def run():
         out = torch.empty((1,), dtype=torch.float32, device=b2.device)
         gb, gc = torch.empty_like(b2), torch.empty_like(c2)
-        _call("pda_head_corner_loss", b2, _chk(b2.detach(), "box_preds", F32), _chk(c2.detach(), "centers", F32), _chk(k2, "cls_preds", F32),
-              int(k2.shape[1]), _chk(gt, "gt", F32), _chk(cls_labels, "cls_labels", I64),
-              None if mean_size is None else _chk(mean_size, "mean_size", F32), int(bins), float(weight), n, _chk(out, "out", F32),
-              _chk(gb, "grad_box", F32), _chk(gc, "grad_centers", F32))
+        ms = None if mean_size is None else _chk(mean_size, "mean_size", F32)
+        group = _open_loss_group()
+        if group is not None:
+            group.add((b2, c2, k2, gt, cls_labels, mean_size, out, gb, gc), kind=_CORNER, preds=_chk(b2.detach(), "box_preds", F32),
+                      aux=_chk(c2.detach(), "centers", F32), cls_preds=_chk(k2, "cls_preds", F32), num_class=int(k2.shape[1]),
+                      gt=_chk(gt, "gt", F32), labels=_chk(cls_labels, "cls_labels", I64), table=ms, bins=int(bins), weight=float(weight),
+                      n=n, out=_chk(out, "out", F32), grad=_chk(gb, "grad_box", F32), grad2=_chk(gc, "grad_centers", F32))
+        else:
+            _call("pda_head_corner_loss", b2, _chk(b2.detach(), "box_preds", F32), _chk(c2.detach(), "centers", F32),
+                  _chk(k2, "cls_preds", F32), int(k2.shape[1]), _chk(gt, "gt", F32), _chk(cls_labels, "cls_labels", I64), ms, int(bins),
+                  float(weight), n, _chk(out, "out", F32), _chk(gb, "grad_box", F32), _chk(gc, "grad_centers", F32))
         return (out[0],), (gb, gc)
     return _ScaledGrad.apply(run, box_preds, centers)[0]
 
```

Result: faster. 128.0 scenes/s (median of 4 runs) (+2.5%).
